# arhik/GaussianSplat

Measured on AMD Instinct MI355X. Metric: fwd+bwd Msplats/sec at 1M Gaussians, 1920x1080, SH deg 3, higher is better.
Workload: dtype f32; 1 GPU; C3: 1000000 gaussians, 1920x1080, SH3, ONE camera view per step, fwd+bwd; the steps cycle over the cameras [0, 4] (view k: eye rotated about +y by 45k degrees; one view slot per camera); synthetic scene of SURVEY 8d with the quaternions NORMALISED (8d leaves N(0,1)^4 raw: the reference never normalises q and |q| scales every footprint by |q|^4; un-normalised q is parity-tested, tests/test_gpu_size; views_per_rank=1, nranks=1, settle_steps=24, rank_mode=1, binning_rounds=1, schedule=3, view_slots=True, order=depth_desc, tile=16, instances=30150056, coarse_instances=2175944, walked_fwd=8350144, alpha_cull=True, list_cap=0, tile_parts=1, lists_capped=False

## Files before the change

### gaussiansplat_amd/backend.py

```python
from __future__ import annotations

import ctypes as C
import os

import numpy as np

_HERE = os.path.dirname(os.path.abspath(__file__))
LIB_PATH = os.environ.get("GSPLAT_HIP_LIB") or os.path.join(_HERE, "lib", "libgsplat_hip.so")

GS_MEM_HOST, GS_MEM_DEVICE = 0, 1
ORDER_INDEX, ORDER_DEPTH_DESC, ORDER_DEPTH_ASC = 0, 1, 2

(ARR_TS, ARR_TPS, ARR_MU, ARR_COV3D, ARR_COV2D, ARR_INVCOV, ARR_BBS, ARR_RGB, ARR_SIG, ARR_DEPTH_KEY,
 ARR_TILE_RECT, ARR_SORT_IDXS, ARR_TILE_RANGES, ARR_SORTED_IDS, ARR_SORTED_KEYS, ARR_GRAD2D) = range(16)

STAGES = ("preprocess", "depth_sort", "count_scan", "emit", "tile_sort", "ranges", "composite_fwd",
          "composite_bwd", "preprocess_bwd")

SYMBOLS = ("gs_default_config", "gs_abi_version", "gs_create", "gs_destroy", "gs_last_error", "gs_set_stream",
           "gs_synchronize", "gs_set_model", "gs_set_model_2d", "gs_set_image_size", "gs_set_camera", "gs_preprocess", "gs_bin", "gs_bind_outputs", "gs_forward", "gs_backward_sgd",
           "gs_backward", "gs_backward_ex", "gs_reset_grads", "gs_loss_l1_dssim", "gs_sgd_step", "gs_comm_unique_id",
           "gs_comm_init", "gs_allreduce_grads", "gs_comm_destroy", "gs_color_grads_pack", "gs_sh_grads_from_views", "gs_grads_alloc", "gs_grads_read", "gs_num_gaussians", "gs_num_instances", "gs_get_array",
           "gs_get_stage_times", "gs_get_stage_stats", "gs_get_work_counters", "gs_get_work_counters_ex", "gs_debug_time_composite",
           "gs_debug_tile_clock", "gs_debug_clock_mhz", "gs_rank_probe_result", "gs_num_rounds", "gs_set_view_slot", "gs_num_coarse_instances",
           "gs_get_list_stats", "gs_get_tile_parts", "gs_get_bin_path", "gs_debug_set_window", "gs_debug_tile_clock_rows")

GS_ABI_VERSION = 3
GS_DEBUG_WIDE_CURSORS = 1
GS_DEBUG_ALWAYS_ORDER = 2
GS_DEBUG_SUPER16 = 8
GS_DEBUG_SUPER8 = 16
GS_DEBUG_TINY_CAPS = 4
GS_MAX_VIEW_SLOTS = 4096


class GsConfig(C.Structure):
    _fields_ = [("struct_size", C.c_int32), ("abi_version", C.c_int32), ("tile_size", C.c_int32), ("order", C.c_int32), ("t_min", C.c_float),
                ("deterministic", C.c_int32), ("export_debug", C.c_int32), ("profile_stages", C.c_int32),
                ("bin_path", C.c_int32), ("rank_mode", C.c_int32), ("alpha_cull", C.c_int32), ("schedule", C.c_int32),
                ("slab_mode", C.c_int32), ("slab_max_ratio", C.c_float), ("slab_fractions", C.c_float * 3), ("debug_flags", C.c_int32),
                ("depth_sort", C.c_int32), ("list_cap", C.c_int32), ("tile_parts", C.c_int32), ("reserved", C.c_int32 * 3)]


class GsGrads(C.Structure):
    _fields_ = [("d_means", C.c_void_p), ("d_scales", C.c_void_p), ("d_quats", C.c_void_p),
                ("d_opacities", C.c_void_p), ("d_shs", C.c_void_p)]


class GsError(RuntimeError):
    def __init__(self, code: int, msg: str):
        super().__init__(f"libgsplat_hip error {code}: {msg}")
        self.code = code


_lib = None


def load():
    global _lib
    if _lib is not None:
        return _lib
    try:
        import torch
    except ImportError:
        pass
    if not os.path.exists(LIB_PATH):
        raise FileNotFoundError(f"{LIB_PATH} not found: build it with `python -m gaussiansplat_amd.build` "
                                "(there is no CPU fallback)")
    L = C.CDLL(LIB_PATH)
    vp, fp = C.c_void_p, C.POINTER(C.c_float)
    L.gs_default_config.argtypes = [C.POINTER(GsConfig)]; L.gs_default_config.restype = None
    L.gs_abi_version.restype = C.c_int
    L.gs_create.argtypes = [C.POINTER(vp), C.c_int, C.POINTER(GsConfig)]
    L.gs_destroy.argtypes = [vp]
    L.gs_last_error.argtypes = [vp]; L.gs_last_error.restype = C.c_char_p
    L.gs_set_stream.argtypes = [vp, vp]
    L.gs_synchronize.argtypes = [vp]
    L.gs_set_model.argtypes = [vp, C.c_int64, C.c_int, vp, vp, vp, vp, vp, C.c_int]
    L.gs_set_camera.argtypes = [vp, fp, fp, C.c_float, C.c_float, C.c_float, C.c_float, fp, fp, C.c_int32, C.c_int32]
    L.gs_preprocess.argtypes = [vp]
    L.gs_bin.argtypes = [vp, C.c_int32, C.c_int32]
    L.gs_bind_outputs.argtypes = [vp, vp, vp]
    L.gs_backward_sgd.argtypes = [vp, vp, C.c_int, C.c_float]
    L.gs_forward.argtypes = [vp, vp, vp, C.c_int]
    L.gs_backward.argtypes = [vp, vp, C.c_int, C.POINTER(GsGrads)]
    L.gs_backward_ex.argtypes = [vp, vp, C.c_int, C.POINTER(GsGrads), C.c_int]
    L.gs_reset_grads.argtypes = [vp, C.POINTER(GsGrads)]
    L.gs_loss_l1_dssim.argtypes = [vp, vp, vp, C.c_int32, C.c_int32, C.c_int32, C.c_float, vp, C.POINTER(C.c_double), C.c_int]
    L.gs_sgd_step.argtypes = [vp, C.c_float, C.POINTER(GsGrads)]
    L.gs_comm_unique_id.argtypes = [vp]
    L.gs_comm_init.argtypes = [vp, C.c_int, C.c_int, vp]
    L.gs_allreduce_grads.argtypes = [vp, C.POINTER(GsGrads)]
    L.gs_comm_destroy.argtypes = [vp]
    L.gs_grads_alloc.argtypes = [vp, C.POINTER(GsGrads)]
    L.gs_grads_read.argtypes = [vp, C.POINTER(GsGrads), vp, vp, vp, vp, vp]
    L.gs_num_gaussians.argtypes = [vp]; L.gs_num_gaussians.restype = C.c_int64
    L.gs_num_instances.argtypes = [vp]; L.gs_num_instances.restype = C.c_int64
    L.gs_get_array.argtypes = [vp, C.c_int, vp, C.c_int64]
    L.gs_get_stage_times.argtypes = [vp, fp]
    L.gs_get_stage_stats.argtypes = [vp, C.POINTER(C.c_double), C.POINTER(C.c_int64), C.c_int]
    L.gs_get_work_counters.argtypes = [vp, C.POINTER(C.c_int64), C.POINTER(C.c_int64)]
    L.gs_set_model_2d.argtypes = [vp, C.c_int64, vp, vp, vp, vp, vp, C.c_int]
    L.gs_set_image_size.argtypes = [vp, C.c_int32, C.c_int32]
    L.gs_color_grads_pack.argtypes = [vp, vp]
    L.gs_sh_grads_from_views.argtypes = [vp, C.c_int32, vp, vp, vp, C.c_int]
    L.gs_get_work_counters_ex.argtypes = [vp, C.POINTER(C.c_int64)]
    L.gs_debug_time_composite.argtypes = [vp, C.c_int, C.c_int, C.c_int, C.POINTER(C.c_float)]
    L.gs_debug_tile_clock.argtypes = [vp, C.c_int, C.c_int, vp]
    L.gs_debug_clock_mhz.argtypes = [vp, C.POINTER(C.c_float)]
    L.gs_rank_probe_result.argtypes = [vp]
    L.gs_num_rounds.argtypes = [vp]
    L.gs_set_view_slot.argtypes = [vp, C.c_int32]
    L.gs_num_coarse_instances.argtypes = [vp]; L.gs_num_coarse_instances.restype = C.c_int64
    L.gs_get_list_stats.argtypes = [vp, C.POINTER(C.c_int64)]
    L.gs_get_tile_parts.argtypes = [vp]
    L.gs_get_bin_path.argtypes = [vp]
    L.gs_debug_set_window.argtypes = [vp, C.c_int32, C.c_int32]
    L.gs_debug_tile_clock_rows.argtypes = [vp]
    if L.gs_abi_version() != GS_ABI_VERSION:
        raise RuntimeError(f"{LIB_PATH} has ABI version {L.gs_abi_version()}, this binding is written for {GS_ABI_VERSION}: "
                           "rebuild with `python -m gaussiansplat_amd.build --force`")
    _lib = L
    return L


def default_config() -> GsConfig:
    cfg = GsConfig()
    load().gs_default_config(C.byref(cfg))
    return cfg


class Context:

    def __init__(self, device: int = 0, order: int = ORDER_DEPTH_DESC, t_min: float = 1e-5, export_debug: bool = False,
                 profile_stages: bool = False, deterministic: bool = False, bin_path: int = 0, rank_mode: int = 1,
                 alpha_cull: bool = True, schedule: int = 0, slab_mode: int = 1, slab_fractions=(), slab_max_ratio: float = 0.0,
                 debug_flags: int = 0, depth_sort: int = 0, list_cap: int = 0, tile_parts: "int | None" = None,
                 cfg: "GsConfig | None" = None):
        self.L = load()
        if cfg is not None:
            twin = GsConfig()
            C.memmove(C.byref(twin), C.byref(cfg), C.sizeof(GsConfig))
            self.cfg = twin
            self.h = C.c_void_p()
            rc = self.L.gs_create(C.byref(self.h), device, C.byref(twin))
            if rc != 0:
                raise GsError(rc, (self.L.gs_last_error(None) or b"").decode())
            self._keep = []
            return
        cfg = default_config()
        assert cfg.struct_size == C.sizeof(GsConfig) and cfg.abi_version == GS_ABI_VERSION
        cfg.schedule = int(schedule)
        cfg.slab_mode = int(slab_mode)
        cfg.slab_max_ratio = float(slab_max_ratio)
        for i, f in enumerate(tuple(slab_fractions)[:3]):
            cfg.slab_fractions[i] = float(f)
        cfg.debug_flags = int(debug_flags)
        cfg.depth_sort = int(depth_sort)
        cfg.list_cap = int(list_cap)
        cfg.tile_parts = int(os.environ.get("GSPLAT_TILE_PARTS", "0")) if tile_parts is None else int(tile_parts)
        cfg.order, cfg.t_min = int(order), float(t_min)
        cfg.export_debug, cfg.profile_stages, cfg.deterministic = int(export_debug), int(profile_stages), int(deterministic)
        cfg.bin_path, cfg.rank_mode, cfg.alpha_cull = int(bin_path), int(rank_mode), int(alpha_cull)
        self.cfg = cfg
        self.h = C.c_void_p()
        rc = self.L.gs_create(C.byref(self.h), device, C.byref(cfg))
        if rc != 0:
            raise GsError(rc, (self.L.gs_last_error(None) or b"").decode())
        self._keep = []

    def _chk(self, rc: int):
        if rc != 0:
            raise GsError(rc, (self.L.gs_last_error(self.h) or b"").decode())

    def close(self):
        if getattr(self, "h", None) and self.h.value:
            self.L.gs_destroy(self.h)
            self.h = C.c_void_p()

    def __del__(self):
        try:
            self.close()
        except Exception:
            pass

    def set_stream(self, hip_stream: int | None):
        self._chk(self.L.gs_set_stream(self.h, C.c_void_p(hip_stream or 0)))

    def synchronize(self):
        self._chk(self.L.gs_synchronize(self.h))

    def set_model_host(self, means, scales, quats, opacities, shs, sh_degree: int):
        arrs = [np.ascontiguousarray(a, np.float32) for a in (means, scales, quats, opacities, shs)]
        n = arrs[0].shape[0]
        self._chk(self.L.gs_set_model(self.h, n, sh_degree, *(C.c_void_p(a.ctypes.data) for a in arrs), GS_MEM_HOST))

    def set_model_device(self, n: int, sh_degree: int, ptrs):
        self._chk(self.L.gs_set_model(self.h, n, sh_degree, *(C.c_void_p(int(p)) for p in ptrs), GS_MEM_DEVICE))

    def set_model_2d_host(self, means, scales, rots, opacities, colors):
        arrs = [np.ascontiguousarray(a, np.float32) for a in (means, scales, rots, opacities, colors)]
        n = arrs[0].shape[0]
        self._chk(self.L.gs_set_model_2d(self.h, n, *(C.c_void_p(a.ctypes.data) for a in arrs), GS_MEM_HOST))

    def set_model_2d_device(self, n: int, ptrs):
        self._chk(self.L.gs_set_model_2d(self.h, n, *(C.c_void_p(int(p)) for p in ptrs), GS_MEM_DEVICE))

    def set_image_size(self, W: int, H: int):
        self._chk(self.L.gs_set_image_size(self.h, int(W), int(H)))
        self.W, self.H = int(W), int(H)

    def set_camera(self, T, P, fx, fy, near, far, eye, lookAt, W, H):
        fp = C.POINTER(C.c_float)
        a = [np.ascontiguousarray(v, np.float32).reshape(-1) for v in (T, P, eye, lookAt)]
        self._chk(self.L.gs_set_camera(self.h, a[0].ctypes.data_as(fp), a[1].ctypes.data_as(fp), fx, fy, near, far,
                                       a[2].ctypes.data_as(fp), a[3].ctypes.data_as(fp), int(W), int(H)))
        self.W, self.H = int(W), int(H)

    def camera_record(self, T, P, fx, fy, near, far, eye, lookAt, W, H):
        f16, f3 = C.c_float * 16, C.c_float * 3
        a = [np.ascontiguousarray(v, np.float32).reshape(-1) for v in (T, P, eye, lookAt)]
        return (f16(*a[0]), f16(*a[1]), float(fx), float(fy), float(near), float(far), f3(*a[2]), f3(*a[3]), int(W), int(H))

    def set_camera_record(self, rec):
        self._chk(self.L.gs_set_camera(self.h, *rec))
        self.W, self.H = rec[8], rec[9]

    def set_view_slot(self, slot: int):
        self._chk(self.L.gs_set_view_slot(self.h, int(slot)))

    def preprocess(self):
        self._chk(self.L.gs_preprocess(self.h))

    def bin(self, gx: int = 0, gy: int = 0):
        self._chk(self.L.gs_bin(self.h, gx, gy))

    def forward_host(self):
        img = np.empty((3, self.H, self.W), np.float32)
        tr = np.empty((self.H, self.W), np.float32)
        self._chk(self.L.gs_forward(self.h, C.c_void_p(img.ctypes.data), C.c_void_p(tr.ctypes.data), GS_MEM_HOST))
        return img, tr

    def bind_outputs(self, image_ptr: int = 0, trans_ptr: int = 0):
        self._chk(self.L.gs_bind_outputs(self.h, C.c_void_p(image_ptr), C.c_void_p(trans_ptr)))

    def forward_device(self, image_ptr: int = 0, trans_ptr: int = 0):
        self._chk(self.L.gs_forward(self.h, C.c_void_p(image_ptr), C.c_void_p(trans_ptr), GS_MEM_DEVICE))

    def backward(self, dC_ptr_or_array, grads: GsGrads, overwrite: bool = False, phase: str = "all"):
        flags = (1 if overwrite else 0) | {"all": 0, "composite": 2, "params": 4, "params_sh": 4 | 8, "params_geom": 4 | 16}[phase]
        if isinstance(dC_ptr_or_array, np.ndarray):
            a = np.ascontiguousarray(dC_ptr_or_array, np.float32)
            self._chk(self.L.gs_backward_ex(self.h, C.c_void_p(a.ctypes.data), GS_MEM_HOST, C.byref(grads), flags))
        else:
            self._chk(self.L.gs_backward_ex(self.h, C.c_void_p(int(dC_ptr_or_array)), GS_MEM_DEVICE, C.byref(grads), flags))

    def color_grads_pack(self, drgb_ptr: int):
        self._chk(self.L.gs_color_grads_pack(self.h, C.c_void_p(int(drgb_ptr))))

    def sh_grads_from_views(self, cam_records: np.ndarray, drgb_ptr: int, d_shs_ptr: int, overwrite: bool = True):
        cr = np.ascontiguousarray(cam_records, np.float32)
        assert cr.ndim == 2 and cr.shape[1] == 38
        self._chk(self.L.gs_sh_grads_from_views(self.h, cr.shape[0], C.c_void_p(cr.ctypes.data), C.c_void_p(int(drgb_ptr)),
                                                C.c_void_p(int(d_shs_ptr)), 1 if overwrite else 0))

    def backward_sgd(self, dC_ptr: int, lr: float):
        self._chk(self.L.gs_backward_sgd(self.h, C.c_void_p(dC_ptr), GS_MEM_DEVICE, C.c_float(lr)))

    def grads_alloc(self) -> GsGrads:
        g = GsGrads()
        self._chk(self.L.gs_grads_alloc(self.h, C.byref(g)))
        return g

    def grads_read(self, grads: GsGrads, sh_degree: int) -> dict:
        n, k3 = self.num_gaussians, 3 * (sh_degree + 1) ** 2
        out = dict(means=np.empty((n, 3), np.float32), scales=np.empty((n, 3), np.float32), quats=np.empty((n, 4), np.float32),
                   opacities=np.empty((n,), np.float32), shs=np.empty((n, k3), np.float32))
        self._chk(self.L.gs_grads_read(self.h, C.byref(grads), *(C.c_void_p(out[k].ctypes.data) for k in
                                                                   ("means", "scales", "quats", "opacities", "shs"))))
        return out

    def grads_read_2d(self, grads: GsGrads) -> dict:
        n = self.num_gaussians
        out = dict(means=np.empty((n, 2), np.float32), scales=np.empty((n, 2), np.float32), rots=np.empty((n,), np.float32),
                   opacities=np.empty((n,), np.float32), colors=np.empty((n, 3), np.float32))
        self._chk(self.L.gs_grads_read(self.h, C.byref(grads), *(C.c_void_p(out[k].ctypes.data) for k in
                                                                   ("means", "scales", "rots", "opacities", "colors"))))
        return out

    def loss_host(self, img: np.ndarray, gt: np.ndarray, lam: float = 0.1):
        img = np.ascontiguousarray(img, np.float32); gt = np.ascontiguousarray(gt, np.float32)
        dC = np.empty_like(img)
        out = C.c_double()
        Cn, H, W = img.shape
        self._chk(self.L.gs_loss_l1_dssim(self.h, C.c_void_p(img.ctypes.data), C.c_void_p(gt.ctypes.data), W, H, Cn, lam,
                                          C.c_void_p(dC.ctypes.data), C.byref(out), GS_MEM_HOST))
        return float(out.value), dC

    def loss_device(self, img_ptr: int, gt_ptr: int, dC_ptr: int, W: int, H: int, Cn: int, lam: float = 0.1, want_loss: bool = True):
        out = C.c_double()
        self._chk(self.L.gs_loss_l1_dssim(self.h, C.c_void_p(img_ptr), C.c_void_p(gt_ptr), W, H, Cn, lam, C.c_void_p(dC_ptr),
                                          C.byref(out) if want_loss else None, GS_MEM_DEVICE))
        return float(out.value) if want_loss else None

    @staticmethod
    def comm_unique_id() -> bytes:
        buf = C.create_string_buffer(128)
        rc = load().gs_comm_unique_id(buf)
        if rc != 0:
            raise GsError(rc, (load().gs_last_error(None) or b"").decode())
        return buf.raw

    def comm_init(self, rank: int, nranks: int, unique_id: bytes):
        self._chk(self.L.gs_comm_init(self.h, rank, nranks, C.c_char_p(unique_id)))

    def allreduce_grads(self, grads: GsGrads):
        self._chk(self.L.gs_allreduce_grads(self.h, C.byref(grads)))

    def sgd_step(self, lr: float, grads: GsGrads):
        self._chk(self.L.gs_sgd_step(self.h, lr, C.byref(grads)))

    def reset_grads(self, grads: GsGrads):
        self._chk(self.L.gs_reset_grads(self.h, C.byref(grads)))

    @property
    def num_gaussians(self) -> int:
        return int(self.L.gs_num_gaussians(self.h))

    @property
    def num_instances(self) -> int:
        return int(self.L.gs_num_instances(self.h))

    @property
    def num_coarse_instances(self) -> int:
        return int(self.L.gs_num_coarse_instances(self.h))

    @property
    def num_rounds(self) -> int:
        return int(self.L.gs_num_rounds(self.h))

    def get_array(self, which: int, gx: int | None = None, gy: int | None = None) -> np.ndarray:
        n, ni = self.num_gaussians, self.num_instances
        spec = {ARR_TS: ((n, 4), np.float32), ARR_TPS: ((n, 4), np.float32), ARR_MU: ((n, 2), np.float32),
                ARR_COV3D: ((n, 9), np.float32), ARR_COV2D: ((n, 4), np.float32), ARR_INVCOV: ((n, 4), np.float32),
                ARR_BBS: ((n, 4), np.float32), ARR_RGB: ((n, 3), np.float32), ARR_SIG: ((n,), np.float32),
                ARR_DEPTH_KEY: ((n,), np.uint32), ARR_TILE_RECT: ((n, 4), np.uint16), ARR_SORT_IDXS: ((n,), np.uint32),
                ARR_SORTED_IDS: ((ni,), np.uint32), ARR_SORTED_KEYS: ((ni,), np.uint64), ARR_GRAD2D: ((n, 10), np.float32)}
        if which == ARR_TILE_RANGES:
            ntiles = ((self.W + 15) // 16) * ((self.H + 15) // 16)
            shape, dt = (ntiles, 2), np.uint32
        else:
            shape, dt = spec[which]
        out = np.empty(shape, dt)
        self._chk(self.L.gs_get_array(self.h, which, C.c_void_p(out.ctypes.data), out.nbytes))
        return out

    def stage_stats(self, reset: bool = False) -> dict:
        sm = (C.c_double * len(STAGES))()
        ct = (C.c_int64 * len(STAGES))()
        self._chk(self.L.gs_get_stage_stats(self.h, sm, ct, int(reset)))
        return {k: (float(sm[i]), int(ct[i])) for i, k in enumerate(STAGES)}

    def work_counters(self):
        a, b = C.c_int64(), C.c_int64()
        self._chk(self.L.gs_get_work_counters(self.h, C.byref(a), C.byref(b)))
        return int(a.value), int(b.value)

    def work_counters_ex(self) -> dict:
        o = (C.c_int64 * 4)()
        self._chk(self.L.gs_get_work_counters_ex(self.h, o))
        return dict(walked_fwd=int(o[0]), walked_bwd=int(o[1]), evaluated_fwd=int(o[2]), evaluated_bwd=int(o[3]))

    def list_stats(self) -> dict:
        o = (C.c_int64 * 3)()
        self._chk(self.L.gs_get_list_stats(self.h, o))
        return dict(listed=int(o[0]), extended_segments=int(o[1]), capped=bool(o[2]))

    def tile_parts_of_frame(self) -> int:
        rc = self.L.gs_get_tile_parts(self.h)
        if rc < 0:
            self._chk(rc)
        return int(rc)

    def bin_path_of_frame(self) -> int:
        rc = self.L.gs_get_bin_path(self.h)
        if rc < 0:
            self._chk(rc)
        return int(rc)

    def time_composite(self, which: int, variant: int, reps: int = 10) -> float:
        ms = C.c_float()
        self._chk(self.L.gs_debug_time_composite(self.h, which, variant, reps, C.byref(ms)))
        return float(ms.value)

    def tile_clock(self, which: int, variant: int = 0) -> np.ndarray:
        ntiles = ((self.W + 15) // 16) * ((self.H + 15) // 16)
        rows = ntiles
        if variant < 0:
            rows = int(self.L.gs_debug_tile_clock_rows(self.h))
            if rows <= 0:
                raise GsError(-1, "tile_clock: records by workgroup need a frame with a launch order")
        out = np.zeros((rows, 15), np.uint64)
        self._chk(self.L.gs_debug_tile_clock(self.h, which, variant, C.c_void_p(out.ctypes.data)))
        return out

    def set_debug_window(self, start: int = 0, length: int = 0):
        self._chk(self.L.gs_debug_set_window(self.h, start, length))

    def clock_mhz(self) -> float:
        mhz = C.c_float()
        self._chk(self.L.gs_debug_clock_mhz(self.h, C.byref(mhz)))
        return float(mhz.value)

    @property
    def rank_probe_result(self) -> int:
        return int(self.L.gs_rank_probe_result(self.h))

    def stage_times(self) -> dict:
        ms = (C.c_float * len(STAGES))()
        self._chk(self.L.gs_get_stage_times(self.h, ms))
        return {k: float(ms[i]) for i, k in enumerate(STAGES)}
```

### gaussiansplat_amd/csrc/gs_api_composite.hip

```cpp
#include "gs_ctx.h"

const uint32_t *forward_order(gs_ctx *c) {
    const int64_t ntiles = (int64_t)c->gx * c->gy;
    if (!lpt_schedule(c) || ntiles <= 0 || ntiles > GS_LPT_MAX_TILES) return nullptr;
    const int k = order_index(c);
    if (k == GS_MAX_VIEW_SLOTS && c->cfg.schedule != 4) return nullptr;
    if (c->slots[k].tiles != (((int64_t)c->gx << 32) | (int64_t)c->gy)) return nullptr;
    if (c->order_pending) {
        if (hipStreamWaitEvent(c->stream, c->ev_order, 0) != hipSuccess) return nullptr;
        c->order_pending = false;
    }
    c->frame_order_split = c->pinned_split ? c->pinned_split + 2 * k + c->slots[k].sel : nullptr;
    return c->slots[k].order[c->slots[k].sel].as<uint32_t>();
}

int build_frame_order(gs_ctx *c, const uint32_t *used) {
    const int64_t ntiles = (int64_t)c->gx * c->gy;
    c->frame_order = used;
    if (!lpt_schedule(c) || ntiles <= 0 || ntiles > GS_LPT_MAX_TILES) return GS_OK;
    const int k = order_index(c);
    const int dst = used ? 1 - c->slots[k].sel : c->slots[k].sel;
    DevBuf &ob = c->slots[k].order[dst];
    HIPCHK(c, ob.ensure(sizeof(uint32_t) * ((size_t)lpt_order_entries(c) + GS_SEG_SLOTS + 16)));
    const uint32_t *walked = lpt_front(c) > 0 ? c->last_walked : nullptr;
    uint32_t *rearm = nullptr, *nsplit = c->pinned_split ? c->pinned_split + 2 * k + dst : nullptr;
    if (nsplit) *nsplit = 0xFFFFFFFFu;
    if (lpt_front(c) > 0) {
        if (!c->snap_walked.p) {
            HIPCHK(c, c->snap_walked.ensure(sizeof(uint32_t) * 2 * GS_SEG_SLOTS));
            HIPCHK(c, hipMemsetAsync(c->snap_walked.p, 0, sizeof(uint32_t) * 2 * GS_SEG_SLOTS, c->stream));
        }
        rearm = c->snap_walked.as<uint32_t>() + (size_t)(c->snap_parity ^ 1) * GS_SEG_SLOTS;
    }
    if (used && use_side_stream(c)) {
        if (c->order_pending) HIPCHK(c, hipStreamWaitEvent(c->stream, c->ev_order, 0));
        HIPCHK(c, hipEventRecord(c->ev_main, c->stream));
        HIPCHK(c, hipStreamWaitEvent(c->side, c->ev_main, 0));
        HIPCHK(c, gs_launch_tile_lpt_order(c->tile_work.as<uint32_t>(), 0, c->gx, c->gy, ob.as<uint32_t>(), c->side, nullptr, 0, lpt_front(c), lpt_split_div(c), walked, rearm, nsplit));
        HIPCHK(c, hipEventRecord(c->ev_order, c->side));
        c->order_pending = true;
        c->slots[k].sel = dst;
    } else {
        HIPCHK(c, gs_launch_tile_lpt_order(c->tile_work.as<uint32_t>(), 0, c->gx, c->gy, ob.as<uint32_t>(), c->stream, nullptr, 0, lpt_front(c), lpt_split_div(c), walked, rearm, nsplit));
        c->frame_order = ob.as<uint32_t>();
        c->frame_order_split = nsplit;
    }
    c->slots[k].tiles = ((int64_t)c->gx << 32) | (int64_t)c->gy;
    return GS_OK;
}

extern "C" {

int gs_bind_outputs(gs_ctx *c, float *image, float *transmittance) {
    if (!c) return GS_ERR_INVALID;
    if ((image == nullptr) != (transmittance == nullptr)) return fail(c, GS_ERR_INVALID, "gs_bind_outputs: bind both buffers or neither");
    c->bound_image = image; c->bound_trans = transmittance;
    c->did_fwd = c->did_bwd = false;
    return GS_OK;
}

int gs_set_view_slot(gs_ctx *c, int32_t slot) {
    if (!c) return GS_ERR_INVALID;
    if (slot >= GS_MAX_VIEW_SLOTS) return fail(c, GS_ERR_INVALID, "gs_set_view_slot: slot must be below GS_MAX_VIEW_SLOTS (or negative: none)");
    c->view_slot = slot < 0 ? -1 : (int)slot;
    return GS_OK;
}

static int composite_parts(const gs_ctx *c) {
    const int want = c->cfg.tile_parts;
    if (want == 1 || !(c->cfg.t_min > 0.0f) || c->n_rounds > 1 || c->frame_capped) return 1;
    if (want == 2 || want == 4) return want;
    const long long ntiles = (long long)c->gx * c->gy, slots = c->wave_slots;
    return 4 * ntiles <= slots ? 4 : 2 * ntiles <= slots ? 2 : 1;
}

static int enqueue_forward_round(gs_ctx *c, int r, const uint32_t *order) {
    const int R = c->n_rounds;
    GsCompositeArgs a{};
    a.W = c->cam.W; a.H = c->cam.H; a.gx = c->gx; a.gy = c->gy; a.t_min = c->cfg.t_min;
    a.ranges = r == 0 ? c->ranges.as<uint32_t>() : c->ranges_r[r].as<uint32_t>();
    a.ids = c->ids.as<uint32_t>() + c->round_ids_off[r]; a.payload = c->payload.as<GsPayload>();
    a.image = c->img(); a.trans = c->tr();
    a.walked = nullptr;
    a.cull = c->cfg.alpha_cull != 0;
    a.resume = r > 0; a.final_round = r == R - 1;
    a.tile_work = c->tile_work.as<uint32_t>(); a.tile_walked = const_cast<uint32_t *>(c->last_walked);
    a.tile_order = order; a.order_len = order ? lpt_order_entries(c) : 0;
    a.parts = c->frame_parts;
    a.split_ok = order && lpt_front(c) > 0 && c->frame_parts == 1 && !c->frame_capped && R == 1;
    c->snap_order = nullptr;
    if (c->frame_seg_n && R == 1) {
        const size_t nt = (size_t)c->gx * c->gy;
        HIPCHK(c, c->snap.ensure(sizeof(float) * nt * (size_t)(c->frame_seg_n - 1) * 4 * 256));
        HIPCHK(c, c->tile_walked_b.ensure(sizeof(uint32_t) * (nt ? nt : 1)));
        HIPCHK(c, c->tile_work_b.ensure(sizeof(uint32_t) * (nt ? nt : 1)));
        a.snap = c->snap.as<float>(); a.seg_hist = c->seg_hist; a.seg_n = c->frame_seg_n;
        a.bw_walked = c->tile_walked_b.as<uint32_t>(); a.bw_work = c->tile_work_b.as<uint32_t>();
    }
    const bool may_split = !c->frame_order_split || *c->frame_order_split != 0u;
    if (a.split_ok && c->snap_walked.p && may_split) {
        HIPCHK(c, c->snap.ensure(sizeof(float) * (size_t)GS_SEG_SLOTS * GS_SEG_SNAP_FLOATS));
        const size_t nt = (size_t)c->gx * c->gy;
        HIPCHK(c, c->tile_walked_b.ensure(sizeof(uint32_t) * (nt ? nt : 1)));
        HIPCHK(c, c->tile_work_b.ensure(sizeof(uint32_t) * (nt ? nt : 1)));
        a.snap = c->snap.as<float>(); a.seg_len = order_seg_len(c, order); a.front = lpt_front(c);
        a.snap_walked = c->snap_walked.as<uint32_t>() + (size_t)c->snap_parity * GS_SEG_SLOTS;
        a.bw_walked = c->tile_walked_b.as<uint32_t>(); a.bw_work = c->tile_work_b.as<uint32_t>();
        c->snap_order = order;
    }
    if (c->frame_capped && R == 1) {
        a.tile_ext = c->tile_ext.as<uint2>(); a.cranges = c->cranges.as<uint32_t>(); a.cids = c->cids.as<uint32_t>(); a.clr = c->clr.as<uint16_t>();
        a.ids_w = c->ids.as<uint32_t>(); a.sgx = c->sgx; a.sbs = c->sbs; a.ext_count = c->ext_count();
    }
    if (R > 1) { a.tile_pos = c->tile_pos.as<uint32_t>(); a.tile_done = c->tile_done.as<uint8_t>(); a.tile_dead = c->tile_dead.as<unsigned long long>(); }
    StageTimer t(c, GS_STAGE_COMPOSITE_FWD);
    HIPCHK(c, gs_launch_composite_fwd(a, c->stream));
    return GS_OK;
}

int gs_forward(gs_ctx *c, float *image, float *transmittance, int mem) {
    if (!c) return GS_ERR_INVALID;
    if (!c->did_bin) return fail(c, GS_ERR_INVALID, "gs_forward: gs_bin first");
    if (mem != GS_MEM_HOST && mem != GS_MEM_DEVICE) return fail(c, GS_ERR_INVALID, "gs_forward: bad mem");
    if (bind_device(c)) return GS_ERR_HIP;
    const size_t px = (size_t)c->cam.W * c->cam.H;
    const size_t ntiles = (size_t)c->gx * c->gy;
    if (!c->bound_image) {
        HIPCHK(c, c->image.ensure(sizeof(float) * 3 * px));
        HIPCHK(c, c->trans.ensure(sizeof(float) * px));
    }
    HIPCHK(c, c->counters.ensure(GS_COUNTER_BYTES));
    HIPCHK(c, c->tile_work.ensure(sizeof(uint32_t) * (ntiles ? ntiles : 1)));
    c->counters_grid = ((int64_t)c->gx << 32) | (int64_t)c->gy;
    c->frame_seg_n = 0; c->seg_hist = nullptr;
    int flip_slot = -1;
    {
        const int k = order_index(c);
        if (k < GS_MAX_VIEW_SLOTS || c->cfg.schedule == 4) {
            gs_ctx::ViewSlot &vs = c->slots[k];
            DevBuf &wb = vs.walkbuf[vs.wsel ^ 1];
            HIPCHK(c, wb.ensure(sizeof(uint32_t) * (ntiles ? ntiles : 1)));
            const bool hist = vs.walked_grid == c->counters_grid && vs.walked().p;
            if (hist && c->cfg.tile_parts == 0 && c->cfg.t_min > 0.0f && c->n_rounds == 1 && !c->frame_capped && !lpt_schedule(c) && c->kind == 0 &&
                2 * (int64_t)ntiles <= c->wave_slots && ntiles > 0) {
                c->frame_seg_n = 2;
                c->seg_hist = vs.walked().as<uint32_t>();
            }
            c->last_walked = wb.as<uint32_t>();
            flip_slot = k;
        } else {
            HIPCHK(c, c->tile_walked.ensure(sizeof(uint32_t) * (ntiles ? ntiles : 1)));
            c->last_walked = c->tile_walked.as<uint32_t>();
        }
    }
    const int R = c->n_rounds;
    if (R > 1) {
        HIPCHK(c, c->tile_pos.ensure(sizeof(uint32_t) * (ntiles ? ntiles : 1)));
        HIPCHK(c, c->tile_done.ensure(ntiles ? ntiles : 1));
        HIPCHK(c, c->tile_dead.ensure(sizeof(unsigned long long) * 4 * (ntiles ? ntiles : 1)));
        HIPCHK(c, hipMemsetAsync(c->tile_pos.p, 0, sizeof(uint32_t) * ntiles, c->stream));
    }
    c->frame_parts = composite_parts(c);
    c->snap_parity ^= 1;
    const uint32_t *order = forward_order(c);
    if (c->order_pending) { HIPCHK(c, hipStreamWaitEvent(c->stream, c->ev_order, 0)); c->order_pending = false; }
    for (int r = 0; r < R; ++r) {
        if (r > 0) { if (int rc = bin_round(c, r)) return rc; }
        if (int rc = enqueue_forward_round(c, r, order)) return rc;
        if (r == 0) {
            bool redo = false;
            if (int rc = settle_totals(c, &redo, true)) return rc;
            if (redo) {
                if (int rc = enqueue_forward_round(c, 0, order)) return rc;
            }
        }
    }
    if (flip_slot >= 0) { c->slots[flip_slot].wsel ^= 1; c->slots[flip_slot].walked_grid = c->counters_grid; }
    if (int rc = build_frame_order(c, order)) return rc;
    const hipMemcpyKind kind = mem == GS_MEM_HOST ? hipMemcpyDeviceToHost : hipMemcpyDeviceToDevice;
    if (image && image != c->img()) HIPCHK(c, hipMemcpyAsync(image, c->img(), sizeof(float) * 3 * px, kind, c->stream));
    if (transmittance && transmittance != c->tr()) HIPCHK(c, hipMemcpyAsync(transmittance, c->tr(), sizeof(float) * px, kind, c->stream));
    if (mem == GS_MEM_HOST && (image || transmittance)) HIPCHK(c, hipStreamSynchronize(c->stream));
    c->did_fwd = true; c->did_bwd = false; c->did_bwd_composite = false;
    c->prev_counters_valid = true; c->prev_n_inst = c->n_inst;
    return GS_OK;
}

int gs_backward(gs_ctx *c, const float *dC, int mem, const gs_grads *grads) { return gs_backward_ex(c, dC, mem, grads, 0); }

static int backward_impl(gs_ctx *c, const float *dC, int mem, const gs_grads *grads, int flags, float sgd_scale);
int gs_backward_ex(gs_ctx *c, const float *dC, int mem, const gs_grads *grads, int flags) { return backward_impl(c, dC, mem, grads, flags, 0.0f); }

int gs_backward_sgd(gs_ctx *c, const float *dC, int mem, float lr) {
    if (!c) return GS_ERR_INVALID;
    if (c->kind != 0) return fail(c, GS_ERR_UNSUPPORTED, "gs_backward_sgd: 3-D renderer only");
    if (!(lr != 0.0f)) return fail(c, GS_ERR_INVALID, "gs_backward_sgd: lr must be non-zero");
    gs_grads g{const_cast<float *>(c->means), const_cast<float *>(c->scales), const_cast<float *>(c->quats),
               const_cast<float *>(c->opac), const_cast<float *>(c->shs)};
    const int rc = backward_impl(c, dC, mem, &g, 0, -lr);
    if (rc == GS_OK) c->did_pre = c->did_bin = c->did_fwd = c->did_bwd = false;
    return rc;
}

static int backward_impl(gs_ctx *c, const float *dC, int mem, const gs_grads *grads, int flags, float sgd_scale) {
    if (!c) return GS_ERR_INVALID;
    if (!c->did_fwd) return fail(c, GS_ERR_INVALID, "gs_backward: gs_forward first");
    const bool params_only = (flags & GS_BWD_PARAMS_ONLY) != 0, composite_only = (flags & GS_BWD_COMPOSITE_ONLY) != 0;
    if (params_only && composite_only) return fail(c, GS_ERR_INVALID, "gs_backward: COMPOSITE_ONLY and PARAMS_ONLY exclude each other");
    const int chain = (flags & (GS_BWD_PARAMS_SH | GS_BWD_PARAMS_GEOM)) >> 3;
    if (chain && !params_only) return fail(c, GS_ERR_INVALID, "gs_backward: GS_BWD_PARAMS_SH / _GEOM need GS_BWD_PARAMS_ONLY");
    if (chain && c->kind != 0) return fail(c, GS_ERR_UNSUPPORTED, "gs_backward: GS_BWD_PARAMS_SH / _GEOM: 3-D renderer only");
    if (params_only && !c->did_bwd_composite) return fail(c, GS_ERR_INVALID, "gs_backward: GS_BWD_PARAMS_ONLY needs a GS_BWD_COMPOSITE_ONLY call on this frame");
    if ((!dC && !params_only) || (!grads && !composite_only)) return fail(c, GS_ERR_INVALID, "gs_backward: NULL argument");
    if (mem != GS_MEM_HOST && mem != GS_MEM_DEVICE) return fail(c, GS_ERR_INVALID, "gs_backward: bad mem");
    if (bind_device(c)) return GS_ERR_HIP;
    const size_t px = (size_t)c->cam.W * c->cam.H, n1 = c->n ? (size_t)c->n : 1;
    const float *dC_dev = dC;
    if (mem == GS_MEM_HOST && !params_only) {
        HIPCHK(c, c->stage_in.ensure(sizeof(float) * 3 * px));
        HIPCHK(c, hipMemcpyAsync(c->stage_in.p, dC, sizeof(float) * 3 * px, hipMemcpyHostToDevice, c->stream));
        dC_dev = c->stage_in.as<float>();
    }
    const bool det = c->cfg.deterministic != 0;
    HIPCHK(c, c->g2d.ensure((det ? sizeof(long long) : sizeof(float)) * GS_G2D_STRIDE * n1));
    GsCompositeArgs a{};
    a.W = c->cam.W; a.H = c->cam.H; a.gx = c->gx; a.gy = c->gy; a.t_min = c->cfg.t_min;
    a.ranges = c->ranges.as<uint32_t>(); a.ids = c->ids.as<uint32_t>(); a.payload = c->payload.as<GsPayload>();
    a.image = c->img(); a.trans = c->tr();
    a.nseg = 0;
    for (int r = 0; r < c->n_rounds; ++r) {
        if (r > 0 && c->round_gen[r] == 0) continue;
        a.seg_ranges[a.nseg] = r == 0 ? c->ranges.as<uint32_t>() : c->ranges_r[r].as<uint32_t>();
        a.seg_ids[a.nseg] = c->ids.as<uint32_t>() + c->round_ids_off[r];
        ++a.nseg;
    }
    a.dC = dC_dev; a.g2d = det ? nullptr : c->g2d.as<float>(); a.g2d_fixed = det ? c->g2d.as<long long>() : nullptr;
    {
        const size_t nt = (size_t)c->gx * c->gy;
        HIPCHK(c, c->tile_walked_b.ensure(sizeof(uint32_t) * (nt ? nt : 1)));
        HIPCHK(c, c->tile_work_b.ensure(sizeof(uint32_t) * (nt ? nt : 1)));
    }
    a.walked = nullptr; a.tile_walked = c->tile_walked_b.as<uint32_t>(); a.tile_work = c->tile_work_b.as<uint32_t>();
    if (c->frame_capped && c->n_rounds == 1) a.tile_ext = c->tile_ext.as<uint2>();
    a.cull = c->cfg.alpha_cull != 0;
    a.parts = c->frame_parts;
    if (c->frame_seg_n && c->n_rounds == 1 && !c->frame_capped) {
        const long long nt = (long long)c->gx * c->gy;
        a.snap = c->snap.as<float>(); a.seg_hist = c->seg_hist; a.seg_n = c->frame_seg_n;
        a.parts = 4 * a.seg_n * nt <= c->wave_slots ? 4 : 2 * a.seg_n * nt <= c->wave_slots ? 2 : 1;
    }
    if (!params_only) {
        c->last_dC = dC_dev;
        if (!c->g2d_clean) HIPCHK(c, hipMemsetAsync(c->g2d.p, 0, (det ? sizeof(long long) : sizeof(float)) * GS_G2D_STRIDE * n1, c->stream));
        c->g2d_clean = false;
        if (lpt_schedule(c)) { a.tile_order = c->frame_order; a.order_len = c->frame_order ? lpt_order_entries(c) : 0; }
        a.split_ok = a.tile_order && lpt_front(c) > 0 && c->frame_parts == 1 && !c->frame_capped && c->n_rounds == 1;
        if (a.split_ok && c->snap_order && c->snap_order == a.tile_order) {
            a.snap = c->snap.as<float>(); a.seg_len = order_seg_len(c, a.tile_order); a.front = lpt_front(c);
            a.snap_walked = c->snap_walked.as<uint32_t>() + (size_t)c->snap_parity * GS_SEG_SLOTS;
        }
        {
            StageTimer t(c, GS_STAGE_COMPOSITE_BWD);
            HIPCHK(c, gs_launch_composite_bwd(a, c->stream));
        }
        c->did_bwd_composite = true;
    }
    if (composite_only) {
        if (mem == GS_MEM_HOST) HIPCHK(c, hipStreamSynchronize(c->stream));
        c->did_bwd = true;
        return GS_OK;
    }
    if (c->kind == 1) {
        GsPreprocess2DBwdArgs b2{};
        b2.n = c->n; b2.W = c->cam.W; b2.H = c->cam.H;
        b2.scales = c->scales; b2.rots = c->quats; b2.opac = c->opac;
        b2.g2d = det ? nullptr : c->g2d.as<float>(); b2.g2d_fixed = det ? c->g2d.as<long long>() : nullptr;
        b2.overwrite = (flags & GS_BWD_OVERWRITE) ? 1 : 0;
        b2.d_means = grads->d_means; b2.d_scales = grads->d_scales; b2.d_rots = grads->d_quats;
        b2.d_opac = grads->d_opacities; b2.d_colors = grads->d_shs;
        {
            StageTimer t(c, GS_STAGE_PREPROCESS_BWD);
            HIPCHK(c, gs_launch_preprocess2d_bwd(b2, c->stream));
        }
        if (mem == GS_MEM_HOST) HIPCHK(c, hipStreamSynchronize(c->stream));
        c->did_bwd = true;
        return GS_OK;
    }
    GsPreprocessBwdArgs b{};
    b.n = c->n; b.sh_degree = c->sh_degree;
    b.means = c->means; b.scales = c->scales; b.quats = c->quats; b.opac = c->opac; b.shs = c->shs;
    b.g2d = det ? nullptr : c->g2d.as<float>(); b.g2d_fixed = det ? c->g2d.as<long long>() : nullptr;
    HIPCHK(c, c->dpc.ensure(sizeof(float) * 4 * n1));
    b.dpc = c->dpc.as<float>();
    b.overwrite = (flags & GS_BWD_OVERWRITE) ? 1 : 0;
    b.sgd_scale = sgd_scale;
    b.d_means = grads->d_means; b.d_scales = grads->d_scales; b.d_quats = grads->d_quats;
    b.d_opac = grads->d_opacities; b.d_shs = grads->d_shs;
    {
        StageTimer t(c, GS_STAGE_PREPROCESS_BWD);
        HIPCHK(c, gs_launch_preprocess_bwd(b, c->cam, c->stream, chain ? chain : 3));
    }
    if (mem == GS_MEM_HOST) HIPCHK(c, hipStreamSynchronize(c->stream));
    c->did_bwd = true;
    return GS_OK;
}

int gs_color_grads_pack(gs_ctx *c, float *drgb) {
    if (!c || !drgb) return GS_ERR_INVALID;
    if (c->kind != 0) return fail(c, GS_ERR_UNSUPPORTED, "gs_color_grads_pack: 3-D renderer only");
    if (!c->did_bwd) return fail(c, GS_ERR_INVALID, "gs_color_grads_pack: gs_backward first");
    if (bind_device(c)) return GS_ERR_HIP;
    const bool det = c->cfg.deterministic != 0;
    HIPCHK(c, gs_launch_pack_drgb(det ? nullptr : c->g2d.as<float>(), det ? c->g2d.as<long long>() : nullptr, drgb, c->n, c->stream));
    return GS_OK;
}

int gs_sh_grads_from_views(gs_ctx *c, int32_t nviews, const float *cams, const float *drgb, float *d_shs, int flags) {
    if (!c || !cams || !drgb || !d_shs || nviews <= 0) return GS_ERR_INVALID;
    if (c->kind != 0) return fail(c, GS_ERR_UNSUPPORTED, "gs_sh_grads_from_views: 3-D renderer only");
    if (bind_device(c)) return GS_ERR_HIP;
    const size_t bytes = sizeof(float) * GS_VIEW_RECORD_FLOATS * (size_t)nviews;
    HIPCHK(c, c->view_cams.ensure(bytes));
    HIPCHK(c, hipMemcpyAsync(c->view_cams.p, cams, bytes, hipMemcpyHostToDevice, c->stream));
    HIPCHK(c, gs_launch_sh_from_views(c->n, c->sh_degree, c->means, nviews, c->view_cams.as<float>(), drgb, d_shs,
                                      (flags & GS_BWD_OVERWRITE) ? 1 : 0, c->stream));
    return GS_OK;
}

}
```

### gaussiansplat_amd/csrc/gs_api_debug.hip

```cpp
#include "gs_ctx.h"

extern "C" {

int64_t gs_num_gaussians(const gs_ctx *c) { return c ? c->n : 0; }
int64_t gs_num_instances(gs_ctx *c) { if (!c) return 0; (void)settle_totals(c, nullptr, true); return c->n_inst; }
int64_t gs_num_coarse_instances(gs_ctx *c) { if (!c) return 0; (void)settle_totals(c, nullptr, true); return c->two_level ? c->n_coarse : 0; }
int gs_num_rounds(const gs_ctx *c) { return c ? c->n_rounds : 0; }

int gs_get_array(gs_ctx *c, int which, void *dst, int64_t bytes) {
    if (!c || !dst) return GS_ERR_INVALID;
    if (bind_device(c)) return GS_ERR_HIP;
    const size_t n = (size_t)c->n;
    const void *src = nullptr;
    size_t need = 0;
    auto need_dbg = [&](int i, size_t w) -> int {
        if (!c->cfg.export_debug) return fail(c, GS_ERR_INVALID, "gs_get_array: needs gs_config.export_debug = 1");
        src = c->dbg[i].p; need = sizeof(float) * w * n; return GS_OK;
    };
    if (which <= GS_ARR_TILE_RECT && !c->did_pre) return fail(c, GS_ERR_INVALID, "gs_get_array: gs_preprocess first");
    if (which >= GS_ARR_SORT_IDXS && which <= GS_ARR_SORTED_KEYS && !c->did_bin) return fail(c, GS_ERR_INVALID, "gs_get_array: gs_bin first");
    if (which >= GS_ARR_TILE_RANGES && which <= GS_ARR_SORTED_KEYS) { if (int rc = settle_totals(c, nullptr, true)) return rc; }
    if (which >= GS_ARR_TILE_RANGES && which <= GS_ARR_SORTED_KEYS && c->n_rounds > 1)
        return fail(c, GS_ERR_INVALID, "gs_get_array: this frame was binned in depth slabs (lists spread over rounds); use gs_config.slab_mode = 0");
    if ((which == GS_ARR_SORTED_IDS || which == GS_ARR_SORTED_KEYS) && c->frame_capped && c->have_l2) {
        GsBin3Args a = c->last_l2;
        a.cap_src = nullptr; a.tile_nopen = nullptr; a.smax = nullptr; a.tile_ext = nullptr;
        HIPCHK(c, gs_bin3_write_lists(a, c->stream));
        c->frame_capped = false;
    }
    switch (which) {
        case GS_ARR_TS: if (int r = need_dbg(0, 4)) return r; break;
        case GS_ARR_TPS: if (int r = need_dbg(1, 4)) return r; break;
        case GS_ARR_COV3D: if (int r = need_dbg(3, 9)) return r; break;
        case GS_ARR_COV2D: if (int r = need_dbg(4, 4)) return r; break;
        case GS_ARR_BBS: if (int r = need_dbg(6, 4)) return r; break;
        case GS_ARR_INVCOV: src = c->invcov.p; need = sizeof(float) * 4 * n; break;
        case GS_ARR_MU: case GS_ARR_RGB: case GS_ARR_SIG: {
            const size_t w = which == GS_ARR_MU ? 2 : which == GS_ARR_RGB ? 3 : 1;
            if ((size_t)bytes != sizeof(float) * w * n) return fail(c, GS_ERR_INVALID, "gs_get_array: size mismatch");
            std::vector<GsPayload> h(n ? n : 1);
            HIPCHK(c, hipMemcpyAsync(h.data(), c->payload.p, sizeof(GsPayload) * n, hipMemcpyDeviceToHost, c->stream));
            HIPCHK(c, hipStreamSynchronize(c->stream));
            float *o = static_cast<float *>(dst);
            for (size_t g = 0; g < n; ++g) {
                const GsPayload &p = h[g];
                if (which == GS_ARR_MU) { o[2 * g] = p.mx; o[2 * g + 1] = p.my; }
                else if (which == GS_ARR_RGB) { o[3 * g] = p.r; o[3 * g + 1] = p.g; o[3 * g + 2] = p.b; }
                else o[g] = p.sig;
            }
            return GS_OK;
        }
        case GS_ARR_DEPTH_KEY: src = c->depth_key.p; need = sizeof(uint32_t) * n; break;
        case GS_ARR_TILE_RECT: src = c->rect.p; need = sizeof(uint16_t) * 4 * n; break;
        case GS_ARR_SORT_IDXS: {
            if ((size_t)bytes != sizeof(uint32_t) * n) return fail(c, GS_ERR_INVALID, "gs_get_array: size mismatch");
            if (c->perm_pending) {
                uint32_t *perm = nullptr;
                if (int rc = depth_order(c, &perm)) return rc;
                c->perm_ptr = c->perm_all = perm; c->perm_pending = false;
            }
            if (c->perm_ptr) { src = c->perm_ptr; need = sizeof(uint32_t) * n; break; }
            uint32_t *o = static_cast<uint32_t *>(dst);
            for (size_t g = 0; g < n; ++g) o[g] = (uint32_t)g;
            return GS_OK;
        }
        case GS_ARR_TILE_RANGES: src = c->ranges.p; need = sizeof(uint32_t) * 2 * (size_t)c->gx * c->gy; break;
        case GS_ARR_SORTED_IDS: case GS_ARR_SORTED_KEYS: {
            const size_t ni = (size_t)c->n_inst, nt = (size_t)c->gx * c->gy;
            const size_t w = which == GS_ARR_SORTED_IDS ? sizeof(uint32_t) : sizeof(uint64_t);
            if ((size_t)bytes != w * ni) return fail(c, GS_ERR_INVALID, "gs_get_array: size mismatch");
            std::vector<uint32_t> h(ni ? ni : 1), dk(n ? n : 1), rg(2 * (nt ? nt : 1));
            HIPCHK(c, hipMemcpyAsync(h.data(), c->ids.p, sizeof(uint32_t) * ni, hipMemcpyDeviceToHost, c->stream));
            HIPCHK(c, hipMemcpyAsync(dk.data(), c->depth_key.p, sizeof(uint32_t) * n, hipMemcpyDeviceToHost, c->stream));
            HIPCHK(c, hipMemcpyAsync(rg.data(), c->ranges.p, sizeof(uint32_t) * 2 * nt, hipMemcpyDeviceToHost, c->stream));
            HIPCHK(c, hipStreamSynchronize(c->stream));
            if (which == GS_ARR_SORTED_IDS) {
                std::memcpy(dst, h.data(), sizeof(uint32_t) * ni);
            } else {
                uint64_t *o = static_cast<uint64_t *>(dst);
                const bool by_index = c->order() == GS_ORDER_INDEX;
                for (size_t t = 0; t < nt; ++t)
                    for (size_t p = rg[2 * t]; p < rg[2 * t + 1] && p < ni; ++p)
                        o[p] = ((uint64_t)t << 32) | (by_index ? h[p] : dk[h[p]]);
            }
            return GS_OK;
        }
        case GS_ARR_GRAD2D: {
            if (!c->did_bwd) return fail(c, GS_ERR_INVALID, "gs_get_array: gs_backward first");
            if ((size_t)bytes != sizeof(float) * 10 * n) return fail(c, GS_ERR_INVALID, "gs_get_array: size mismatch");
            float *o = static_cast<float *>(dst);
            if (c->cfg.deterministic) {
                std::vector<long long> fx((size_t)GS_G2D_STRIDE * (n ? n : 1));
                if (n) HIPCHK(c, hipMemcpyAsync(fx.data(), c->g2d.p, sizeof(long long) * GS_G2D_STRIDE * n, hipMemcpyDeviceToHost, c->stream));
                HIPCHK(c, hipStreamSynchronize(c->stream));
                for (size_t g = 0; g < n; ++g)
                    for (int i = 0; i < 10; ++i) o[10 * g + i] = (float)((double)fx[GS_G2D_STRIDE * g + i] * gs_fixed_inv(i));
            } else {
                std::vector<float> fl((size_t)GS_G2D_STRIDE * (n ? n : 1));
                if (n) HIPCHK(c, hipMemcpyAsync(fl.data(), c->g2d.p, sizeof(float) * GS_G2D_STRIDE * n, hipMemcpyDeviceToHost, c->stream));
                HIPCHK(c, hipStreamSynchronize(c->stream));
                for (size_t g = 0; g < n; ++g)
                    for (int i = 0; i < 10; ++i) o[10 * g + i] = fl[GS_G2D_STRIDE * g + i];
            }
            std::vector<GsPayload> pay(n ? n : 1);
            std::vector<float> ic(4 * (n ? n : 1));
            if (n) HIPCHK(c, hipMemcpyAsync(pay.data(), c->payload.p, sizeof(GsPayload) * n, hipMemcpyDeviceToHost, c->stream));
            if (n) HIPCHK(c, hipMemcpyAsync(ic.data(), c->invcov.p, sizeof(float) * 4 * n, hipMemcpyDeviceToHost, c->stream));
            HIPCHK(c, hipStreamSynchronize(c->stream));
            for (size_t g = 0; g < n; ++g) {
                float row[10];
                for (int i = 0; i < 10; ++i) row[i] = o[10 * g + i];
                gs_g2d_to_grads(row, pay[g].sig, ic[4 * g], 0.5f * (ic[4 * g + 1] + ic[4 * g + 2]), ic[4 * g + 3]);
                for (int i = 0; i < 10; ++i) o[10 * g + i] = row[i];
            }
            return GS_OK;
        }
        default: return fail(c, GS_ERR_INVALID, "gs_get_array: unknown array");
    }
    if ((size_t)bytes != need) return fail(c, GS_ERR_INVALID, "gs_get_array: size mismatch");
    if (need) HIPCHK(c, hipMemcpyAsync(dst, src, need, hipMemcpyDeviceToHost, c->stream));
    HIPCHK(c, hipStreamSynchronize(c->stream));
    return GS_OK;
}

int gs_get_stage_times(gs_ctx *c, float ms[GS_STAGE_COUNT]) {
    if (!c || !ms) return GS_ERR_INVALID;
    if (!c->cfg.profile_stages) return fail(c, GS_ERR_INVALID, "gs_get_stage_times: needs gs_config.profile_stages = 1");
    if (bind_device(c)) return GS_ERR_HIP;
    HIPCHK(c, hipStreamSynchronize(c->stream));
    for (int s = 0; s < GS_STAGE_COUNT; ++s) {
        ms[s] = 0.0f;
        if (c->ev_valid[s]) HIPCHK(c, hipEventElapsedTime(&ms[s], c->ev[s][0], c->ev[s][1]));
    }
    return GS_OK;
}

int gs_get_stage_stats(gs_ctx *c, double sum_ms[GS_STAGE_COUNT], int64_t count[GS_STAGE_COUNT], int reset) {
    if (!c || !sum_ms || !count) return GS_ERR_INVALID;
    if (!c->cfg.profile_stages) return fail(c, GS_ERR_INVALID, "gs_get_stage_stats: needs gs_config.profile_stages = 1");
    if (bind_device(c)) return GS_ERR_HIP;
    HIPCHK(c, hipStreamSynchronize(c->stream));
    harvest_events(c);
    for (int s = 0; s < GS_STAGE_COUNT; ++s) {
        sum_ms[s] = c->ev_sum[s]; count[s] = c->ev_cnt[s];
        if (reset) { c->ev_sum[s] = 0.0; c->ev_cnt[s] = 0; }
    }
    return GS_OK;
}

static int debug_composite_args(gs_ctx *c, int which, int variant, GsCompositeArgs &a) {
    a.W = c->cam.W; a.H = c->cam.H; a.gx = c->gx; a.gy = c->gy; a.t_min = c->cfg.t_min;
    a.ranges = c->ranges.as<uint32_t>(); a.ids = c->ids.as<uint32_t>(); a.payload = c->payload.as<GsPayload>();
    a.image = c->img(); a.trans = c->tr();
    a.dC = c->last_dC; a.walked = nullptr;
    if (variant >= 10000) {
        variant -= 10000;
        a.walked = reinterpret_cast<unsigned long long *>(static_cast<char *>(c->counters.p) + 160);
    }
    a.final_round = 1;
    a.nseg = 0;
    for (int r = 0; r < c->n_rounds; ++r) {
        if (r > 0 && c->round_gen[r] == 0) continue;
        a.seg_ranges[a.nseg] = r == 0 ? c->ranges.as<uint32_t>() : c->ranges_r[r].as<uint32_t>();
        a.seg_ids[a.nseg] = c->ids.as<uint32_t>() + c->round_ids_off[r];
        ++a.nseg;
    }
    a.g2d = c->cfg.deterministic ? nullptr : c->g2d.as<float>(); a.g2d_fixed = c->cfg.deterministic ? c->g2d.as<long long>() : nullptr;
    c->g2d_clean = false;
    if (c->frame_capped && c->n_rounds == 1) {
        a.tile_ext = c->tile_ext.as<uint2>(); a.cranges = c->cranges.as<uint32_t>(); a.cids = c->cids.as<uint32_t>(); a.clr = c->clr.as<uint16_t>();
        a.ids_w = c->ids.as<uint32_t>(); a.sgx = c->sgx; a.sbs = c->sbs; a.ext_count = c->ext_count();
    }
    a.variant = variant % 100;
    a.cull = (c->cfg.alpha_cull != 0) != (variant >= 1000);
    a.tile_order = lpt_schedule(c) ? c->frame_order : nullptr;
    a.order_len = a.tile_order ? lpt_order_entries(c) : 0;
    a.split_ok = a.tile_order && lpt_front(c) > 0 && c->frame_parts == 1 && !c->frame_capped && c->n_rounds == 1;
    if (which == 1 && a.split_ok && c->snap_order && c->snap_order == a.tile_order) {
        a.snap = c->snap.as<float>(); a.seg_len = order_seg_len(c, a.tile_order); a.front = lpt_front(c);
        a.snap_walked = c->snap_walked.as<uint32_t>() + (size_t)c->snap_parity * GS_SEG_SLOTS;
    }
    a.parts = c->frame_parts;
    if (which == 1 && c->frame_seg_n && c->n_rounds == 1 && !c->frame_capped && !a.tile_order) {
        const long long nt = (long long)c->gx * c->gy;
        a.snap = c->snap.as<float>(); a.seg_hist = c->seg_hist; a.seg_n = c->frame_seg_n;
        a.parts = 4 * a.seg_n * nt <= c->wave_slots ? 4 : 2 * a.seg_n * nt <= c->wave_slots ? 2 : 1;
    }
    if (c->dbg_win_len > 0) {
        if (!a.tile_order || a.parts > 1) return fail(c, GS_ERR_INVALID, "gs_debug_set_window: the frame has no launch order (or several waves per tile)");
        if (c->dbg_win_start + c->dbg_win_len > a.order_len) return fail(c, GS_ERR_INVALID, "gs_debug_set_window: beyond the launch order");
        a.tile_order += c->dbg_win_start; a.order_len = c->dbg_win_len;
    }
    return GS_OK;
}

int gs_debug_set_window(gs_ctx *c, int32_t start, int32_t len) {
    if (!c) return GS_ERR_INVALID;
    if (start < 0 || len < 0 || (start & 7) || (len & 7)) return fail(c, GS_ERR_INVALID, "gs_debug_set_window: start and len must be non-negative multiples of 8");
    c->dbg_win_start = start; c->dbg_win_len = len;
    return GS_OK;
}

int gs_debug_time_composite(gs_ctx *c, int which, int variant, int reps, float *mean_ms) {
    if (!c || !mean_ms || reps == 0) return GS_ERR_INVALID;
    const bool cold = reps < 0;
    if (cold) reps = -reps;
    if (!c->did_fwd) return fail(c, GS_ERR_INVALID, "gs_debug_time_composite: gs_forward first");
    if (which == 1 && !c->did_bwd) return fail(c, GS_ERR_INVALID, "gs_debug_time_composite: gs_backward first");
    if (bind_device(c)) return GS_ERR_HIP;
    GsCompositeArgs a{};
    if (int rc = debug_composite_args(c, which, variant, a)) return rc;
    hipEvent_t e0, e1;
    HIPCHK(c, hipEventCreate(&e0)); HIPCHK(c, hipEventCreate(&e1));
    auto launch = [&]() -> hipError_t { return which == 0 ? gs_launch_composite_fwd(a, c->stream) : gs_launch_composite_bwd(a, c->stream); };
    if (!cold) HIPCHK(c, launch());
    HIPCHK(c, hipEventRecord(e0, c->stream));
    for (int i = 0; i < reps; ++i) HIPCHK(c, launch());
    HIPCHK(c, hipEventRecord(e1, c->stream));
    HIPCHK(c, hipEventSynchronize(e1));
    float ms = 0.0f;
    HIPCHK(c, hipEventElapsedTime(&ms, e0, e1));
    *mean_ms = ms / reps;
    (void)hipEventDestroy(e0); (void)hipEventDestroy(e1);
    return GS_OK;
}

int gs_debug_tile_clock(gs_ctx *c, int which, int variant, uint64_t *out) {
    if (!c || !out) return GS_ERR_INVALID;
    if (!c->did_fwd) return fail(c, GS_ERR_INVALID, "gs_debug_tile_clock: gs_forward first");
    if (which == 1 && !c->did_bwd) return fail(c, GS_ERR_INVALID, "gs_debug_tile_clock: gs_backward first");
    if (bind_device(c)) return GS_ERR_HIP;
    const size_t ntiles = (size_t)c->gx * c->gy;
    GsCompositeArgs a{};
    const bool by_block = variant < 0;
    if (by_block) variant = -variant;
    if (int rc = debug_composite_args(c, which, variant, a)) return rc;
    if (by_block) {
        if ((!a.tile_order && a.parts <= 1 && !a.seg_hist) || (a.variant / 10) % 10 == 1)
            return fail(c, GS_ERR_INVALID, "gs_debug_tile_clock: records by workgroup need the frame's launch order (or a small grid's tile parts)");
        a.clock_by_block = 1;
    } else { a.split_ok = 0; a.snap = nullptr; }
    const size_t rows = !a.clock_by_block ? ntiles : a.tile_order ? (size_t)(lpt_order_entries(c) + gs_seg_units(lpt_front(c))) : (size_t)gs_debug_tile_clock_rows(c);
    if (a.clock_by_block && (size_t)gs_composite_grid_blocks(a, which) > rows) return fail(c, GS_ERR_INVALID, "gs_debug_tile_clock: launch larger than its record");
    HIPCHK(c, c->tile_clock.ensure(sizeof(uint64_t) * GS_TILE_CLOCK_WORDS * (rows ? rows : 1)));
    HIPCHK(c, hipMemsetAsync(c->tile_clock.p, 0, sizeof(uint64_t) * GS_TILE_CLOCK_WORDS * rows, c->stream));
    a.tile_clock = c->tile_clock.as<unsigned long long>();
    for (int rep = 0; rep < 2; ++rep) {
        HIPCHK(c, which == 0 ? gs_launch_composite_fwd(a, c->stream) : gs_launch_composite_bwd(a, c->stream));
    }
    HIPCHK(c, hipMemcpyAsync(out, c->tile_clock.p, sizeof(uint64_t) * GS_TILE_CLOCK_WORDS * rows, hipMemcpyDeviceToHost, c->stream));
    HIPCHK(c, hipStreamSynchronize(c->stream));
    return GS_OK;
}

int gs_debug_tile_clock_rows(gs_ctx *c) {
    if (!c) return GS_ERR_INVALID;
    if (lpt_schedule(c)) return lpt_order_entries(c) + gs_seg_units(lpt_front(c));
    const int len = ((c->gx * c->gy + 7) / 8) * 8;
    const int units = std::max(c->frame_parts, 1) * (c->frame_seg_n ? 4 * c->frame_seg_n : 1);
    return units > 1 ? len * units : 0;
}

int gs_debug_clock_mhz(gs_ctx *c, float *mhz) {
    if (!c || !mhz) return GS_ERR_INVALID;
    if (bind_device(c)) return GS_ERR_HIP;
    HIPCHK(c, c->counters.ensure(GS_COUNTER_BYTES));
    unsigned long long *d = reinterpret_cast<unsigned long long *>(static_cast<char *>(c->counters.p) + 160), h[2] = {0, 1};
    HIPCHK(c, gs_launch_clock_probe(d, c->stream));
    HIPCHK(c, hipMemcpyAsync(h, d, sizeof(h), hipMemcpyDeviceToHost, c->stream));
    HIPCHK(c, hipStreamSynchronize(c->stream));
    *mhz = h[1] ? (float)((double)h[0] / (double)h[1] * 100.0) : 0.0f;
    return GS_OK;
}

int gs_rank_probe_result(const gs_ctx *c) { return c ? c->rank_probe : -1; }

static int sum_work_counters(gs_ctx *c) {
    unsigned long long *w = c->counters.as<unsigned long long>();
    const int nt = c->gx * c->gy;
    HIPCHK(c, gs_launch_sum_tiles(c->last_walked, c->tile_work.as<uint32_t>(), nt, w, c->stream));
    if (c->did_bwd_composite && c->tile_walked_b.p && c->tile_work_b.p)
        HIPCHK(c, gs_launch_sum_tiles(c->tile_walked_b.as<uint32_t>(), c->tile_work_b.as<uint32_t>(), nt, w + 2, c->stream));
    else HIPCHK(c, hipMemsetAsync(w + 2, 0, 16, c->stream));
    return GS_OK;
}

int gs_get_work_counters(gs_ctx *c, int64_t *walked_fwd, int64_t *walked_bwd) {
    if (!c) return GS_ERR_INVALID;
    if (!c->did_fwd) return fail(c, GS_ERR_INVALID, "gs_get_work_counters: gs_forward first");
    if (bind_device(c)) return GS_ERR_HIP;
    unsigned long long h[4] = {0, 0, 0, 0};
    if (int rc = sum_work_counters(c)) return rc;
    HIPCHK(c, hipMemcpyAsync(h, c->counters.p, 32, hipMemcpyDeviceToHost, c->stream));
    HIPCHK(c, hipStreamSynchronize(c->stream));
    if (walked_fwd) *walked_fwd = (int64_t)h[0];
    if (walked_bwd) *walked_bwd = (int64_t)h[2];
    return GS_OK;
}

int gs_get_list_stats(gs_ctx *c, int64_t out[3]) {
    if (!c || !out) return GS_ERR_INVALID;
    if (!c->did_fwd) return fail(c, GS_ERR_INVALID, "gs_get_list_stats: gs_forward first");
    if (bind_device(c)) return GS_ERR_HIP;
    if (int rc = settle_totals(c, nullptr, true)) return rc;
    out[0] = c->n_inst; out[1] = 0; out[2] = 0;
    if (!c->frame_capped || c->n_rounds != 1) return GS_OK;
    unsigned long long *d = reinterpret_cast<unsigned long long *>(static_cast<char *>(c->counters.p) + 160), h = 0;
    uint32_t e = 0;
    HIPCHK(c, gs_launch_sum_listed(c->tile_ext.as<uint2>(), c->gx * c->gy, d, c->stream));
    HIPCHK(c, hipMemcpyAsync(&h, d, sizeof(h), hipMemcpyDeviceToHost, c->stream));
    HIPCHK(c, hipMemcpyAsync(&e, c->ext_count(), sizeof(e), hipMemcpyDeviceToHost, c->stream));
    HIPCHK(c, hipStreamSynchronize(c->stream));
    out[0] = (int64_t)h; out[1] = (int64_t)e; out[2] = 1;
    return GS_OK;
}

int gs_get_tile_parts(gs_ctx *c) {
    if (!c) return GS_ERR_INVALID;
    if (!c->did_fwd) return fail(c, GS_ERR_INVALID, "gs_get_tile_parts: gs_forward first");
    return c->frame_parts;
}

int gs_get_bin_path(gs_ctx *c) {
    if (!c) return GS_ERR_INVALID;
    if (!c->did_bin) return fail(c, GS_ERR_INVALID, "gs_get_bin_path: gs_bin first");
    return c->small_bin ? 3 : c->two_level ? 0 : c->fast_bin ? 2 : 1;
}

int gs_get_work_counters_ex(gs_ctx *c, int64_t out[4]) {
    if (!c || !out) return GS_ERR_INVALID;
    if (!c->did_fwd) return fail(c, GS_ERR_INVALID, "gs_get_work_counters_ex: gs_forward first");
    if (bind_device(c)) return GS_ERR_HIP;
    unsigned long long h[4] = {0, 0, 0, 0};
    if (int rc = sum_work_counters(c)) return rc;
    HIPCHK(c, hipMemcpyAsync(h, c->counters.p, 32, hipMemcpyDeviceToHost, c->stream));
    HIPCHK(c, hipStreamSynchronize(c->stream));
    out[0] = (int64_t)h[0]; out[1] = (int64_t)h[2]; out[2] = (int64_t)h[1]; out[3] = (int64_t)h[3];
    return GS_OK;
}

}
```

### gaussiansplat_amd/csrc/gs_common.h

```cpp
#pragma once
#include <hip/hip_runtime.h>
#include <stdint.h>

#define GS_TILE 16
#define GS_WAVE 64

#define GS_PAYLOAD_QUADS 4
#define GS_BIG 1.0e30f
struct __attribute__((aligned(16))) GsPayload {
    float mx, my;
    float l2s;
    float xlo;
    float ka, kb, kc;
    float xhi;
    float r, g, b;
    float ylo;
    float yhi;
    float sig;
    uint32_t bbx;
    uint32_t bby;
};
static_assert(sizeof(GsPayload) == 16 * GS_PAYLOAD_QUADS, "payload row size");
__host__ __device__ inline void gs_payload_box_edges(GsPayload &p) {
    const int xmin = (int)(short)(p.bbx & 0xFFFFu), xmax = (int)(short)(p.bbx >> 16);
    const int ymin = (int)(short)(p.bby & 0xFFFFu), ymax = (int)(short)(p.bby >> 16);
    const bool empty = xmax < xmin || ymax < ymin;
    p.xlo = empty ? GS_BIG : ((float)xmin - p.mx) - 0.25f; p.xhi = empty ? GS_BIG : ((float)xmax - p.mx) + 0.25f;
    p.ylo = empty ? GS_BIG : ((float)ymin - p.my) - 0.25f; p.yhi = empty ? GS_BIG : ((float)ymax - p.my) + 0.25f;
}
#define GS_NEG_HALF_LOG2E (-0.72134752044448170368f)
#define GS_L2S_CAP (-2.6e-7f)

struct GsCamera {
    float T[16], P[16];
    float fx, fy, near_, far_;
    float eye[3], lookAt[3];
    int32_t W, H;
};

struct GsDebugArrays {
    float *ts, *tps, *mu, *cov3d, *cov2d, *invcov, *bbs;
};

struct GsPreprocessArgs {
    int64_t n;
    int sh_degree;
    int order;
    int gx, gy;
    const float *means, *scales, *quats, *opac, *shs;
    GsPayload *payload;
    float *invcov;
    uint32_t *depth_key;
    uint16_t *rect;
    GsDebugArrays dbg;
    uint32_t *key_range;
};
#define GS_KEY_RANGE_SLOTS 64
#define GS_KEY_RANGE_STRIDE 64
hipError_t gs_launch_preprocess(const GsPreprocessArgs &a, const GsCamera &cam, hipStream_t stream);

struct GsPreprocess2DArgs {
    int64_t n;
    int W, H, gx, gy;
    const float *means, *scales, *rots, *opac, *colors;
    GsPayload *payload;
    float *invcov;
    uint32_t *depth_key;
    uint16_t *rect;
    GsDebugArrays dbg;
};
struct GsPreprocess2DBwdArgs {
    int64_t n;
    int W, H;
    const float *scales, *rots, *opac;
    const float *g2d;
    const long long *g2d_fixed;
    float *d_means, *d_scales, *d_rots, *d_opac, *d_colors;
    int overwrite;
};
hipError_t gs_launch_preprocess2d(const GsPreprocess2DArgs &a, hipStream_t stream);
hipError_t gs_launch_preprocess2d_bwd(const GsPreprocess2DBwdArgs &a, hipStream_t stream);

struct GsSortScratch {
    uint32_t *block_hist;
    uint32_t *digit_total;
};
size_t gs_sort_table_entries(int64_t n_max);
hipError_t gs_radix_sort_u64(uint64_t *a, uint64_t *b, int64_t n, int bit_lo, int bit_hi,
                             uint32_t *block_hist, uint32_t *digit_total, int *result_in_b,
                             hipStream_t stream, bool ballot_ranks = false, uint32_t *final_low32 = nullptr,
                             const uint32_t *keys32 = nullptr);

size_t gs_depth_range_words();
size_t gs_depth_range_parity_words();
int64_t gs_depth_buckets_max_n();
hipError_t gs_depth_range_reset(uint32_t *acc, hipStream_t s, int nparity = 2);
hipError_t gs_depth_sort_buckets(const uint32_t *keys32, uint64_t *pairs_a, uint64_t *pairs_b, int64_t n, uint32_t *block_hist,
                                 uint32_t *digit_total, uint32_t *perm, const uint32_t *range_acc, uint32_t *reset_acc,
                                 uint32_t *host_stat, hipStream_t stream, bool ballot_ranks);

hipError_t gs_probe_lds_atomic_order(hipStream_t s, int *mismatches);
hipError_t gs_launch_depth_pairs(const uint32_t *depth_key, uint64_t *pairs, int64_t n, hipStream_t s);
hipError_t gs_launch_unpack_perm(const uint64_t *pairs, uint32_t *perm, int64_t n, hipStream_t s);
hipError_t gs_launch_count_scan(const uint16_t *rect, const uint32_t *perm, uint32_t *offsets,
                                uint32_t *block_sums, int64_t n, hipStream_t s);
hipError_t gs_launch_live_prefix(const uint8_t *done, int gx, int gy, uint32_t *live2d, uint32_t *rowp_scratch, hipStream_t s);
hipError_t gs_launch_count_scan_live(const uint16_t *rect, const uint32_t *perm, const uint32_t *live2d, int gx, uint16_t *rect_out,
                                     uint32_t *offsets, uint32_t *block_sums, int64_t n, hipStream_t s);
hipError_t gs_launch_emit(const uint16_t *rect, const uint32_t *perm, const uint32_t *offsets,
                          uint64_t *inst, int64_t n, int gx, hipStream_t s);
hipError_t gs_launch_ranges(const uint64_t *inst, int64_t n_inst, uint32_t *ranges, int64_t n_tiles,
                            hipStream_t s);
hipError_t gs_launch_split_ids(const uint64_t *inst, uint32_t *ids, int64_t n_inst, hipStream_t s);
hipError_t gs_launch_radix_scan(uint32_t *block_hist, int nblocks, uint32_t *digit_total, hipStream_t s);

size_t gs_tile_ranges_scratch_ints(int gx, int gy);
bool gs_tile_ranges_supported(int gx, int gy);
hipError_t gs_launch_tile_ranges(const uint16_t *rect, const uint32_t *perm, int64_t n, int *scratch, int gx, int gy, uint32_t *ranges,
                                 const uint8_t *done, hipStream_t s);
struct GsBin2Args {
    int64_t n, n_inst;
    int gx;
    int lo_bits, hi_bits, gid_bits;
    const uint32_t *offsets, *perm;
    const uint16_t *rect;
    uint32_t *cs;
    uint32_t *block_hist, *digit_total;
    uint32_t *buf_a;
    uint32_t *ids_out;
    bool ballot_ranks;
    const uint8_t *done;
    uint32_t *live_total;
};
hipError_t gs_bin2_build_lists(const GsBin2Args &b, hipStream_t s);

struct GsBin3L1 {
    const uint16_t *rect;
    const uint32_t *perm;
    const uint8_t *sdone;
    int64_t n, n_slab;
    int sgx, ns;
    int sbs;
    uint32_t *rect_sorted;
    uint32_t *table;
    uint32_t *row_total;
    uint32_t *partials;
    uint32_t *totals;
    uint32_t *cranges;
    uint32_t *cids;
    uint16_t *clr;
    uint32_t *tilecnt;
    int ntiles;
    uint32_t *zero_words;
    uint32_t cap_coarse, cap_fine;
    uint32_t *host_totals, *host_walked;
    const uint32_t *walked_src;
    const uint32_t *tile_walked;
    int n_tile_walked;
};
struct GsBin3Args {
    const uint32_t *cranges;
    const uint32_t *cids;
    const uint16_t *clr;
    uint32_t *ranges;
    uint32_t *tilecnt;
    const uint8_t *done;
    uint32_t *segcnt;
    uint32_t *ids_out;
    int gx, gy, sgx, ns;
    int sbs;
    int max_work;
    int wide;
    const uint32_t *totals;
    uint32_t cap_coarse, cap_fine;
    const uint32_t *cap_src;
    uint32_t *tile_nopen;
    uint32_t *smax;
    uint2 *tile_ext;
    uint32_t *ext_count;
};
#define GS_CONT_NONE 0xFFFFFFFFu
__host__ __device__ inline uint32_t gs_list_cap(uint32_t w) { const uint32_t c = w + (w >> 2) + 128u; return c < w ? 0xFFFFFFFFu : c; }
int gs_bin3_seg();
int gs_bin3_sb_shift(int gx, int gy, int force);
bool gs_bin3_supported(int ns);
int64_t gs_bin3_max_work(int64_t coarse_instances, int ns);
size_t gs_bin3_table_words(int64_t n_slab, int ns);
size_t gs_bin3_partial_words(int64_t n, int ns);
hipError_t gs_bin3_l1_count(const GsBin3L1 &b, hipStream_t s);
hipError_t gs_bin3_l1_scatter(const GsBin3L1 &b, hipStream_t s);
hipError_t gs_bin3_build_lists(const GsBin3Args &a, hipStream_t s);
hipError_t gs_bin3_write_lists(const GsBin3Args &a, hipStream_t s);
hipError_t gs_launch_super_done(const uint8_t *done, int gx, int gy, int sgx, int sgy, int sbs, uint8_t *sdone, hipStream_t s);

#define GS_BIN_SMALL_MAX_N 16384
#define GS_BIN_SMALL_MAX_TILES 1024
#define GS_BIN_SMALL_MAX_PAIRS (4ll << 20)
struct GsBinSmallArgs {
    const uint32_t *depth_key;
    const uint2 *rect;
    int n, gx, gy, ntiles;
    uint32_t *ranges;
    uint32_t *ids;
    uint32_t *totals;
    uint32_t *host_totals, *host_walked;
    const uint32_t *walked_src, *tile_walked;
    int n_tile_walked;
    uint4 *zero; size_t zero_words16;
};
bool gs_bin_small_supported(int64_t n, int gx, int gy);
hipError_t gs_bin_small(const GsBinSmallArgs &a, hipStream_t s);

#define GS_TILE_CLOCK_WORDS 15
#define GS_MAX_ROUNDS 4
#define GS_G2D_STRIDE 16
struct GsCompositeArgs {
    int W, H, gx, gy;
    float t_min;
    const uint32_t *ranges;
    const uint32_t *ids;
    const GsPayload *payload;
    float *image;
    float *trans;
    const float *dC;
    float *g2d;
    long long *g2d_fixed;
    unsigned long long *walked;
    uint32_t *tile_walked;
    int cull;
    int variant;
    const uint32_t *tile_order;
    int order_len;
    uint32_t *tile_work;
    unsigned long long *zero_words;
    unsigned long long *tile_clock;
    int nseg;
    const uint32_t *seg_ranges[GS_MAX_ROUNDS];
    const uint32_t *seg_ids[GS_MAX_ROUNDS];
    uint32_t *tile_pos;
    uint8_t *tile_done;
    unsigned long long *tile_dead;
    int resume;
    int final_round;
    uint2 *tile_ext;
    const uint32_t *cranges, *cids;
    const uint16_t *clr;
    uint32_t *ids_w;
    int sgx, sbs;
    uint32_t *ext_count;
    int parts;
    int split_ok;
    float *snap;
    const uint32_t *seg_len;
    uint32_t *snap_walked;
    int front;
    uint32_t *bw_walked, *bw_work;
    const uint32_t *seg_hist;
    int seg_n;
    int clock_by_block;
};
hipError_t gs_launch_sum_listed(const uint2 *ext, int n, unsigned long long *out, hipStream_t s);
#define GS_LPT_MAX_TILES 35000
int gs_lpt_order_len(int gx, int gy);
hipError_t gs_launch_clock_probe(unsigned long long *out, hipStream_t s);
hipError_t gs_launch_sum_tiles(const uint32_t *a, const uint32_t *b, int n, unsigned long long *out, hipStream_t s);
#define GS_LPT_FRONT 2304
#define GS_SEG_MAX 8
#define GS_SEG_MIN_LEN 1024
#define GS_SEG_ALL_MIN_LEN 128
#define GS_SEG_SLOTS (GS_LPT_FRONT / 3)
#define GS_SEG_SNAP_FLOATS ((GS_SEG_MAX - 1) * 4 * 256)
hipError_t gs_launch_tile_lpt_order(const uint32_t *work_or_ranges, int ranges_mode, int gx, int gy, uint32_t *order, hipStream_t s,
                                    unsigned long long *zero14 = nullptr, int buckets = 0, int front = 0, int split_div = 1,
                                    const uint32_t *walked = nullptr, uint32_t *zero_words = nullptr, uint32_t *host_nsplit = nullptr);
#ifndef GS_SEG_ALL_NUM
#define GS_SEG_ALL_NUM 5
#define GS_SEG_ALL_DEN 8
#endif
#ifndef GS_SEG_ALL_SHORT
#define GS_SEG_ALL_SHORT 1
#endif
__host__ __device__ inline uint32_t gs_seg_len_all(uint32_t w, int seg_n) {
    if (GS_SEG_ALL_SHORT && w >= 80u && w <= (seg_n == 2 ? 192u : 64u * (uint32_t)seg_n + 64u)) return 64u;
    const uint32_t per = seg_n == 2 ? (w * GS_SEG_ALL_NUM + GS_SEG_ALL_DEN - 1u) / GS_SEG_ALL_DEN : (w + (uint32_t)seg_n - 1u) / (uint32_t)seg_n, sl = ((per + 63u) & ~63u) < (uint32_t)GS_SEG_ALL_MIN_LEN ? (uint32_t)GS_SEG_ALL_MIN_LEN : ((per + 63u) & ~63u);
    return w > sl ? sl : 0u;
}
int gs_seg_units(int front);
int gs_composite_grid_blocks(const GsCompositeArgs &a, int bwd);
hipError_t gs_launch_composite_fwd(const GsCompositeArgs &a, hipStream_t s);
hipError_t gs_launch_composite_bwd(const GsCompositeArgs &a, hipStream_t s);

struct GsPreprocessBwdArgs {
    int64_t n;
    int sh_degree;
    const float *means, *scales, *quats, *opac, *shs;
    const float *g2d;
    const long long *g2d_fixed;
    float *d_means, *d_scales, *d_quats, *d_opac, *d_shs;
    float *dpc;
    int overwrite;
    float sgd_scale;
};
hipError_t gs_launch_preprocess_bwd(const GsPreprocessBwdArgs &a, const GsCamera &cam, hipStream_t s, int phases = 3);

hipError_t gs_launch_pack_drgb(const float *g2d, const long long *g2d_fixed, float *out, int64_t n, hipStream_t s);
hipError_t gs_launch_sh_from_views(int64_t n, int sh_degree, const float *means, int nviews, const float *cams, const float *drgb,
                                   float *d_shs, int overwrite, hipStream_t s);

template <typename R>
__host__ __device__ inline void gs_g2d_to_grads(R (&g2)[10], R sig, R i0, R mc, R i3) {
#pragma clang fp contract(off)
    const R S0 = g2[3], Sx = g2[4], Sy = g2[5], Sxx = g2[6], Sxy = g2[7], Syy = g2[9];
    g2[3] = sig > R(0) ? -S0 / sig : R(0);
    g2[4] = -(i0 * Sx + mc * Sy);
    g2[5] = -(mc * Sx + i3 * Sy);
    g2[6] = R(0.5) * Sxx; g2[7] = R(0.5) * Sxy; g2[8] = R(0.5) * Sxy; g2[9] = R(0.5) * Syy;
}

#define GS_FIXED_SCALE 1099511627776.0f
#define GS_FIXED_INV (1.0 / 1099511627776.0)
#define GS_FIXED_SCALE2 268435456.0f
#define GS_FIXED_INV2 (1.0 / 268435456.0)
__host__ __device__ inline double gs_fixed_inv(int comp) { return comp >= 6 ? GS_FIXED_INV2 : GS_FIXED_INV; }

#define GS_LOSS_SLOTS 64
#define GS_LOSS_SLOT_STRIDE 8
hipError_t gs_loss_run(int W, int H, int C, const float *img, const float *gt, float *maps, double *acc, float *dC, float lam,
                       const float *win121, hipStream_t s);
hipError_t gs_launch_sgd(float *p, const float *g, float lr, size_t n, hipStream_t s);
```

### gaussiansplat_amd/csrc/gs_composite.hip

```cpp
#include "gs_common.h"

#pragma clang fp contract(off)

#ifndef GS_BWD_MINW
#define GS_BWD_MINW 6
#endif
#ifndef GS_FWD_MINW
#define GS_FWD_MINW 5
#endif
#ifndef GS_LIVE_RECT
#define GS_LIVE_RECT 1
#endif
#ifndef GS_FWD_PACK
#define GS_FWD_PACK 1
#endif
#ifndef GS_FWD_NO_PREFETCH
#define GS_FWD_NO_PREFETCH 0
#endif
#ifndef GS_BWD_PAIR
#define GS_BWD_PAIR 1
#endif
#ifndef GS_FWD_UNROLL
#define GS_FWD_UNROLL 2
#endif
constexpr int kFwdUnroll = GS_FWD_UNROLL;
#define CB 64
#ifndef L2_SEG
#define L2_SEG 2048
#endif
__device__ __forceinline__ int gs_bin3_seg_const() { return L2_SEG; }
#define NEG_HALF_LOG2E (-0.72134752044448170368f)

__device__ __forceinline__ float fast_exp2(float x) { return __builtin_amdgcn_exp2f(x); }
__device__ __forceinline__ float vgpr_const(float x) { float r; asm volatile("v_mov_b32 %0, %1" : "=v"(r) : "s"(x)); return r; }
__device__ __forceinline__ float fast_rcp(float x) { return __builtin_amdgcn_rcpf(x); }

#define GS_ORDER_TILE_MASK 0x0FFFFFFFu
__device__ __forceinline__ int tile_of_block(const GsCompositeArgs &a, int ntiles, int &part, int &nparts, int first_block = 0) {
    const int len = (a.tile_order && a.order_len > 0) ? a.order_len : ((ntiles + 7) / 8) * 8;
    int b = (int)blockIdx.x - first_block;
    part = 0; nparts = a.parts > 1 ? a.parts : 1;
    if (a.parts > 1) { part = b / len; b -= part * len; if (part >= a.parts) return -1; }
    if (a.tile_order) {
        if (b >= (a.order_len > 0 ? a.order_len : ntiles)) return -1;
        uint32_t t = a.tile_order[b];
        if (t == 0xFFFFFFFFu) return -1;
        if (a.parts <= 1 && (t >> 28)) {
            part = (int)((t >> 28) & 3u); nparts = 1 << (t >> 30);
            if (!a.split_ok) { if (part) return -1; nparts = 1; }
        }
        t &= GS_ORDER_TILE_MASK;
        return t < (uint32_t)ntiles ? (int)t : -1;
    }
    return b < ntiles ? b : -1;
}
__device__ __forceinline__ uint32_t strips_of_part(int nparts, int part) {
    return nparts == 4 ? (1u << part) : nparts == 2 ? (3u << (2 * part)) : 0xFu;
}

__device__ __forceinline__ unsigned long long wave_hw_id() {
    const uint32_t hw = (uint32_t)__builtin_amdgcn_s_getreg((4) | (0 << 6) | (31 << 11));
    const uint32_t xcc = (uint32_t)__builtin_amdgcn_s_getreg((20) | (0 << 6) | (3 << 11));
    return (unsigned long long)hw | ((unsigned long long)xcc << 32);
}

#define GS_ALPHA_CULL_LOG2 (-27.0f)
__device__ __forceinline__ bool rect_can_contribute(float A, float B, float C, float hBrA, float hBrC, bool concave, float l2s,
                                                    float rx0, float rx1, float ry0, float ry1) {
    const float cx = __builtin_amdgcn_fmed3f(0.0f, rx0, rx1), cy = __builtin_amdgcn_fmed3f(0.0f, ry0, ry1);
    const float dy1 = __builtin_amdgcn_fmed3f(-(hBrC * cx), ry0, ry1);
    const float dx2 = __builtin_amdgcn_fmed3f(-(hBrA * cy), rx0, rx1);
    const float f1 = fmaf(A * cx, cx, dy1 * fmaf(B, cx, C * dy1));
    const float f2 = fmaf(C * cy, cy, dx2 * fmaf(B, cy, A * dx2));
    const float fm = (cx != 0.0f && cy != 0.0f) ? fmaxf(f1, f2) : (cx != 0.0f ? f1 : f2);
    const bool nopix = rx0 > rx1 || ry0 > ry1;
    return !(nopix || (concave && fm + l2s < GS_ALPHA_CULL_LOG2));
}

template <bool STRIPS>
__device__ __forceinline__ void stage_record(const float4 &n0, const float4 &n1, const float4 &n3, const int qx0, const int qx1, const int qy0, const int qy1,
                                             const int ty0, bool &keep, uint32_t &strips) {
    const uint32_t bbx = __float_as_uint(n3.z), bby = __float_as_uint(n3.w);
    const int xmin = (int)(short)(bbx & 0xFFFFu), xmax = (int)(short)(bbx >> 16);
    const int ymin = (int)(short)(bby & 0xFFFFu), ymax = (int)(short)(bby >> 16);
    const bool empty = xmax < xmin || ymax < ymin;
    const float l2s = n0.z;
    const float A = n1.x, B = n1.y, C = n1.z;
    const bool concave = A < 0.0f && C < 0.0f && 4.0f * A * C - B * B > 0.0f;
    const float rx0 = (float)max(qx0, xmin) - n0.x, rx1 = (float)min(qx1, xmax) - n0.x;
    const float ry0 = (float)max(qy0, ymin) - n0.y, ry1 = (float)min(qy1, ymax) - n0.y;
    const float hBrA = 0.5f * B * fast_rcp(A), hBrC = 0.5f * B * fast_rcp(C);
    keep = !empty && rect_can_contribute(A, B, C, hBrA, hBrC, concave, l2s, rx0, rx1, ry0, ry1);
    strips = 0xFu;
    if (STRIPS) {
        strips = 0;
#pragma unroll
        for (int p = 0; p < 4; ++p) {
            const float sy0 = (float)max(max(ty0 + 4 * p, qy0), ymin) - n0.y, sy1 = (float)min(min(ty0 + 4 * p + 3, qy1), ymax) - n0.y;
            if (keep && rect_can_contribute(A, B, C, hBrA, hBrC, concave, l2s, rx0, rx1, sy0, sy1)) strips |= 1u << p;
        }
    }
}

__device__ __forceinline__ void first_use_here(float4 &a, float4 &b, float4 &c, float4 &d) {
    asm volatile("" : "+v"(a.x), "+v"(a.y), "+v"(a.z), "+v"(a.w), "+v"(b.x), "+v"(b.y), "+v"(b.z), "+v"(b.w),
                      "+v"(c.x), "+v"(c.y), "+v"(c.z), "+v"(c.w), "+v"(d.x), "+v"(d.y), "+v"(d.z), "+v"(d.w));
}

__device__ __forceinline__ int wave_min_i32(int v) {
#pragma unroll
    for (int d = 32; d > 0; d >>= 1) v = min(v, __shfl_xor(v, d));
    return __builtin_amdgcn_readfirstlane(v);
}
__device__ __forceinline__ int wave_max_i32(int v) {
#pragma unroll
    for (int d = 32; d > 0; d >>= 1) v = max(v, __shfl_xor(v, d));
    return __builtin_amdgcn_readfirstlane(v);
}

#ifndef GS_RECT_FROM_MASKS
#define GS_RECT_FROM_MASKS 1
#endif
struct LiveRectAcc {
    uint64_t any = 0; uint32_t rows = 0;
    __device__ __forceinline__ void slot(const int p, const uint64_t m) {
        any |= m;
        uint64_t t = m | (m >> 8); t |= t >> 4; t |= t >> 2; t |= t >> 1;
        t &= 0x0001000100010001ull;
        rows |= (uint32_t)((t | (t >> 15) | (t >> 30) | (t >> 45)) & 0xFull) << (4 * p);
    }
    __device__ __forceinline__ void rect(const int tx0, const int ty0, int &qx0, int &qx1, int &qy0, int &qy1) const {
        const uint32_t cols = (uint32_t)((any | (any >> 16) | (any >> 32) | (any >> 48)) & 0xFFFFull);
        if (cols == 0u) { qx0 = 1 << 20; qx1 = -1; qy0 = 1 << 20; qy1 = -1; return; }
        qx0 = tx0 + (int)__builtin_ctz(cols); qx1 = tx0 + 31 - (int)__builtin_clz(cols);
        qy0 = ty0 + (int)__builtin_ctz(rows); qy1 = ty0 + 31 - (int)__builtin_clz(rows);
    }
};

__device__ __forceinline__ int slot_of(uint64_t m) {
    return (int)__builtin_amdgcn_mbcnt_hi((uint32_t)(m >> 32), __builtin_amdgcn_mbcnt_lo((uint32_t)m, 0u));
}

struct Entry { float4 q0, q1, q2; float yhi; };
__device__ __forceinline__ Entry load_entry(const float4 *sp, const float *syhi, int k) {
    Entry e;
    e.q0 = sp[3 * k]; e.q1 = sp[3 * k + 1]; e.q2 = sp[3 * k + 2]; e.yhi = syhi[k];
    return e;
}

__device__ __forceinline__ uint32_t extend_tile_list(const GsCompositeArgs &a, const int tile, uint32_t &cont, uint32_t s1) {
    const int lane = threadIdx.x;
    const int tx = tile % a.gx, ty = tile / a.gx;
    const int sbs = a.sbs;
    const uint32_t sm = (1u << sbs) - 1u;
    const int S = (ty >> sbs) * a.sgx + (tx >> sbs);
    const uint32_t lx = (uint32_t)tx & sm, ly = (uint32_t)ty & sm;
    const uint32_t c1 = a.cranges[2 * S + 1];
    const uint32_t seg = (uint32_t)gs_bin3_seg_const();
    const uint32_t e_end = min(cont + seg, c1);
    for (uint32_t e0 = cont; e0 < e_end; e0 += GS_WAVE) {
        const uint32_t e = e0 + (uint32_t)lane;
        bool hit = false;
        uint32_t id = 0;
        if (e < e_end) {
            const uint32_t lr = a.clr[e];
            hit = (lr & sm) <= lx && lx <= ((lr >> sbs) & sm) && ((lr >> (2 * sbs)) & sm) <= ly && ly <= ((lr >> (3 * sbs)) & sm);
            id = a.cids[e];
        }
        const uint64_t bal = __ballot(hit);
        if (hit) a.ids_w[s1 + (uint32_t)slot_of(bal)] = id;
        s1 += (uint32_t)__popcll(bal);
    }
    cont = e_end < c1 ? e_end : GS_CONT_NONE;
    if (lane == 0 && a.ext_count) atomicAdd(a.ext_count, 1u);
    __threadfence();
    return s1;
}

template <bool EARLY, bool CULL, bool CLK, bool SLAB, bool SNAP = false>
__device__ __forceinline__ void forward_tile(const GsCompositeArgs &a, const int tile, const int part, const int nparts, float4 *sp, float *syhi, const float nbig,
                                             const int snap_slot = -1, const uint32_t seg_len = 0) {
    const int lane = threadIdx.x;
    const int px = (tile % a.gx) * GS_TILE + (lane & 15) + 1;
    const int py0 = (tile / a.gx) * GS_TILE + (lane >> 4) + 1;
    const float fx = (float)px;
    const uint32_t s0 = a.ranges[2 * tile];
    uint32_t s1 = a.ranges[2 * tile + 1];
    uint32_t cont = GS_CONT_NONE;
    const bool capped = !SLAB && EARLY && a.tile_ext != nullptr;
    if (capped) { const uint2 ex = a.tile_ext[tile]; s1 = s0 + ex.x; cont = ex.y; }
    const int ty0 = py0 - (lane >> 4);
    unsigned long long clk0 = 0;
    if (CLK) clk0 = __builtin_amdgcn_s_memrealtime();

    if (SLAB && a.resume && a.tile_done[tile]) return;
    const uint32_t gp0 = SLAB && a.tile_pos ? a.tile_pos[tile] : 0u;
    const uint32_t plane = (uint32_t)a.W * (uint32_t)a.H;
    float Cr[4], Cg[4], Cb[4], T[4], fy[4];
    bool dead[4];
    uint32_t walked = 0, evaluated = 0;
    constexpr bool PACK = GS_FWD_PACK && EARLY && !SLAB;
    const uint32_t own = (EARLY && !SLAB) ? strips_of_part(nparts, part) : 0xFu;
    bool first_pack = PACK && nparts > 1;
    int K = 4;
    uint32_t next_snap = (SNAP && snap_slot >= 0) ? seg_len : 0xFFFFFFFFu;
#pragma unroll
    for (int p = 0; p < 4; ++p) {
        Cr[p] = Cg[p] = Cb[p] = 0.0f;
        fy[p] = (float)(py0 + 4 * p);
        const bool in = (px <= a.W && py0 + 4 * p <= a.H) && ((own >> p) & 1u);
        T[p] = in ? 1.0f : 0.0f;
        dead[p] = !in;
        if (SLAB && a.resume && in) {
            const uint32_t o = (uint32_t)(px - 1) + (uint32_t)a.W * (uint32_t)(py0 + 4 * p - 1);
            Cr[p] = a.image[o]; Cg[p] = a.image[o + plane]; Cb[p] = a.image[o + 2u * plane];
            dead[p] = ((a.tile_dead[4 * (size_t)tile + p] >> lane) & 1ull) != 0ull;
            T[p] = dead[p] ? 0.0f : a.trans[o];
        }
    }
    int qx0, qx1, qy0, qy1;
    auto live_rect = [&]() {
        int lx0 = 1 << 20, lx1 = -1, ly0 = 1 << 20, ly1 = -1;
#pragma unroll
        for (int p = 0; p < 4; ++p) {
            if (!dead[p]) {
                const int x = (int)((!PACK || K == 4) ? fx : fy[2 + (p & 1)]), y = (int)fy[p];
                lx0 = min(lx0, x); lx1 = max(lx1, x); ly0 = min(ly0, y); ly1 = max(ly1, y);
            }
        }
        qx0 = wave_min_i32(lx0); qx1 = wave_max_i32(lx1); qy0 = wave_min_i32(ly0); qy1 = wave_max_i32(ly1);
        if (!GS_LIVE_RECT) { qx0 = (tile % a.gx) * GS_TILE + 1; qx1 = qx0 + GS_TILE - 1; qy0 = ty0; qy1 = ty0 + GS_TILE - 1; }
    };
    {
        qx0 = (tile % a.gx) * GS_TILE + 1; qx1 = min(qx0 + GS_TILE - 1, a.W);
        qy0 = ty0 + 4 * (int)__builtin_ctz(own); qy1 = min(ty0 + 4 * (31 - (int)__builtin_clz(own)) + 3, a.H);
        if (SLAB && a.resume) live_rect();
    }
    const float4 *pay4 = reinterpret_cast<const float4 *>(a.payload);
    float4 n0 = make_float4(0.f, 0.f, 0.f, 0.f), n1 = n0, n2 = n0, n3 = n0;
    uint32_t pos = s0 + lane;
    uint32_t id2 = 0;
    uint32_t gp = gp0;
    uint32_t base = s0;
    unsigned long long t_loop = 0, t_stage = 0, t_mark = 0;
    unsigned long long clk_exec = 0, clk_ideal = 0, clk_alive = 0, clk_pix = 0;
    uint32_t clk_live = 0, clk_strips = 0;
    uint32_t clk_hist[3][4] = {{0, 0, 0, 0}, {0, 0, 0, 0}, {0, 0, 0, 0}};
    int clk_k[3] = {4, 4, 4};
    uint32_t clk_bbkeep = 0;
    if (CLK) t_mark = __builtin_amdgcn_s_memtime();
    for (;;) {
    bool stopped = false;
    {
        const uint32_t pos2 = pos + min((uint32_t)CB - (gp & (CB - 1)), s1 - base);
        if (pos < s1) { const size_t g = a.ids[pos]; n0 = pay4[4 * g]; n1 = pay4[4 * g + 1]; n2 = pay4[4 * g + 2]; n3 = pay4[4 * g + 3]; }
        if (pos2 < s1) id2 = a.ids[pos2];
    }
    for (; base < s1;) {
        const uint32_t phase = gp & (CB - 1);
        const int cnt = (int)min((uint32_t)CB - phase, s1 - base);
        if (EARLY && phase == 0) {
            bool live = false, froze = false;
#pragma unroll
            for (int p = 0; p < 4; ++p) {
                if (!dead[p] && T[p] < a.t_min) {
                    const float x = (!PACK || K == 4) ? fx : fy[2 + (p & 1)];
                    if (a.trans) a.trans[(uint32_t)((int)x - 1) + (uint32_t)a.W * (uint32_t)((int)fy[p] - 1)] = T[p];
                    if (SNAP && snap_slot >= 0) {
                        const int nsn = a.seg_hist ? a.seg_n - 1 : GS_SEG_MAX - 1;
                        float *st = a.snap + (size_t)snap_slot * (size_t)(nsn * 4 * 256) + 768 + ((int)fy[p] - ty0) * GS_TILE + ((int)x - (px - (lane & 15)));
                        for (int kk = (int)(next_snap / seg_len) - 1; kk < nsn; ++kk) st[kk * (4 * 256)] = __int_as_float(0x7FC00000);
                    }
                    dead[p] = true; T[p] = 0.0f; froze = true;
                }
                live = live || !dead[p];
            }
            if (__ballot(live) == 0ull) { stopped = true; break; }
            const bool anyfroze = __ballot(froze) != 0ull;
            if (anyfroze) live_rect();
            if (PACK && K > 1 && (anyfroze || first_pack)) {
                first_pack = false;
                uint64_t lm[4];
                uint32_t nlive = 0;
#pragma unroll
                for (int p = 0; p < 4; ++p) { lm[p] = __ballot(!dead[p]); nlive += (uint32_t)__popcll(lm[p]); }
                const int Kn = (int)((nlive + 63u) >> 6);
                if (Kn <= 2 && Kn < K) {
#pragma unroll
                    for (int p = 0; p < 4; ++p) {
                        const float x = K == 4 ? fx : fy[2 + (p & 1)];
                        const bool mine = K == 4 ? (px <= a.W && py0 + 4 * p <= a.H && ((own >> p) & 1u)) : (p < 2 && x > 0.5f);
                        if (mine && dead[p] && a.image) {
                            const uint32_t o = (uint32_t)((int)x - 1) + (uint32_t)a.W * (uint32_t)((int)fy[p] - 1);
                            a.image[o] = Cr[p]; a.image[o + plane] = Cg[p]; a.image[o + 2u * plane] = Cb[p];
                        }

                    }
                    float *buf = reinterpret_cast<float *>(sp);
                    __syncthreads();
                    uint32_t rb = 0;
#pragma unroll
                    for (int p = 0; p < 4; ++p) {
                        if (!dead[p]) {
                            const uint32_t r = rb + (uint32_t)slot_of(lm[p]);
                            buf[r] = K == 4 ? fx : fy[2 + (p & 1)]; buf[128 + r] = fy[p];
                            buf[256 + r] = Cr[p]; buf[384 + r] = Cg[p]; buf[512 + r] = Cb[p]; buf[640 + r] = T[p];
                        }
                        rb += (uint32_t)__popcll(lm[p]);
                    }
                    __syncthreads();
#pragma unroll
                    for (int q = 0; q < 2; ++q) {
                        const uint32_t idx = (uint32_t)(q * 64 + lane);
                        const bool has = idx < nlive;
                        fy[2 + q] = has ? buf[idx] : 0.0f;
                        fy[q] = has ? buf[128 + idx] : 0.0f;
                        Cr[q] = has ? buf[256 + idx] : 0.0f; Cg[q] = has ? buf[384 + idx] : 0.0f; Cb[q] = has ? buf[512 + idx] : 0.0f;
                        T[q] = has ? buf[640 + idx] : 0.0f;
                        dead[q] = !has; dead[2 + q] = true;
                        T[2 + q] = 0.0f;
                    }
                    K = Kn;
                }
            }
        }
        if (SNAP && EARLY && !SLAB && gp == next_snap) {
            const int ksnap = (int)(next_snap / seg_len) - 1;
            const int nsn = a.seg_hist ? a.seg_n - 1 : GS_SEG_MAX - 1;
            if (ksnap < nsn) {
                float *sn = a.snap + (size_t)snap_slot * (size_t)(nsn * 4 * 256) + ksnap * (4 * 256);
#pragma unroll
                for (int p = 0; p < 4; ++p) {
                    if (!dead[p]) {
                        const float x = (!PACK || K == 4) ? fx : fy[2 + (p & 1)];
                        const int idx = ((int)fy[p] - ty0) * GS_TILE + ((int)x - (px - (lane & 15)));
                        sn[idx] = Cr[p]; sn[256 + idx] = Cg[p]; sn[512 + idx] = Cb[p]; sn[768 + idx] = T[p];
                    }
                }
            }
            next_snap += seg_len;
        }
        if (CLK && (phase == 0 || base == s0)) {
            clk_live = 0; clk_strips = 0;
            uint32_t rows = 0, colcnt[16];
            for (int cidx = 0; cidx < 16; ++cidx) colcnt[cidx] = 0;
#pragma unroll
            for (int p = 0; p < 4; ++p) {
                const uint64_t m = __ballot(!dead[p]); clk_live += (uint32_t)__popcll(m); clk_strips += m ? 1u : 0u;
                for (int r4 = 0; r4 < 4; ++r4) rows += ((m >> (16 * r4)) & 0xFFFFull) ? 1u : 0u;
                for (int cidx = 0; cidx < 16; ++cidx) colcnt[cidx] += (uint32_t)__popcll(m & (0x0001000100010001ull << cidx));
            }
            uint32_t cmax = 0;
            for (int cidx = 0; cidx < 16; ++cidx) cmax = max(cmax, colcnt[cidx]);
            clk_k[0] = (int)((clk_live + 63u) >> 6); clk_k[1] = (int)((rows + 3u) >> 2); clk_k[2] = (int)((cmax + 3u) >> 2);
        }
#if GS_FWD_NO_PREFETCH
        if (base > s0 && pos < s1) {
            const size_t g = a.ids[pos]; n0 = pay4[4 * g]; n1 = pay4[4 * g + 1]; n2 = pay4[4 * g + 2]; n3 = pay4[4 * g + 3];
        }
#endif
        uint32_t strips;
        bool keep;
        stage_record<false>(n0, n1, n3, qx0, qx1, qy0, qy1, ty0, keep, strips);
        int slot = lane, nk = cnt;
        if (!CULL) keep = true;
        if (CULL) {
            keep = keep && lane < cnt;
            const uint64_t m = __ballot(keep);
            slot = slot_of(m); nk = __popcll(m);
        }
        if (CLK && CULL) {
            bool k2; uint32_t st2;
            stage_record<false>(n0, n1, n3, px - (lane & 15), px - (lane & 15) + GS_TILE - 1, ty0, ty0 + GS_TILE - 1, ty0, k2, st2);
            clk_bbkeep += (uint32_t)__popcll(__ballot(k2 && lane < cnt));
        }
        __syncthreads();
        if (keep) {
            sp[3 * slot] = n0; sp[3 * slot + 1] = n1; sp[3 * slot + 2] = n2;
            syhi[slot] = n3.x;
        }
        __syncthreads();
        base += (uint32_t)cnt; gp += (uint32_t)cnt;
        pos = base + lane;
#if !GS_FWD_NO_PREFETCH
        {
            if (pos < s1) { const size_t g = id2; n0 = pay4[4 * g]; n1 = pay4[4 * g + 1]; n2 = pay4[4 * g + 2]; n3 = pay4[4 * g + 3]; }
            const uint32_t pos2 = pos + min((uint32_t)CB, s1 - base);
            if (base < s1 && pos2 < s1) id2 = a.ids[pos2];
        }
#endif
        if (CLK) { const unsigned long long t = __builtin_amdgcn_s_memtime(); t_stage += t - t_mark; t_mark = t; }
#define GS_FWD_PIXEL(e, A0, B0, p) do {                                               \
            const float dY = fy[p] - (e).q0.y;                                              \
            const float ey = dY - __builtin_amdgcn_fmed3f(dY, (e).q2.w, (e).yhi);           \
            const float pw = fmaf(dY, fmaf((e).q1.z, dY, (B0)), (A0));                      \
            const float w = fast_exp2(fmaf(nbig, fabsf(ey), pw)) * T[p];                    \
            Cr[p] = fmaf((e).q2.x, w, Cr[p]);                                               \
            Cg[p] = fmaf((e).q2.y, w, Cg[p]);                                               \
            Cb[p] = fmaf((e).q2.z, w, Cb[p]);                                               \
            T[p] = T[p] - w;                                                                \
        } while (0)
#define GS_FWD_COLUMN(e, XCOL, A0, B0)                                                        \
            const float dX##A0 = (XCOL) - (e).q0.x;                                           \
            const float ex##A0 = dX##A0 - __builtin_amdgcn_fmed3f(dX##A0, (e).q0.w, (e).q1.w);    \
            const float A0 = fmaf(nbig, fabsf(ex##A0), fmaf((e).q1.x * dX##A0, dX##A0, (e).q0.z));  \
            const float B0 = (e).q1.y * dX##A0
        if (!PACK || K == 4) {
#pragma clang loop unroll_count(kFwdUnroll)
            for (int k = 0; k < nk; ++k) {
                const Entry e = load_entry(sp, syhi, k);
                GS_FWD_COLUMN(e, fx, A0, B0);
                GS_FWD_PIXEL(e, A0, B0, 0); GS_FWD_PIXEL(e, A0, B0, 1); GS_FWD_PIXEL(e, A0, B0, 2); GS_FWD_PIXEL(e, A0, B0, 3);
            }
        } else if (K == 2) {
#pragma clang loop unroll_count(kFwdUnroll)
            for (int k = 0; k < nk; ++k) {
                const Entry e = load_entry(sp, syhi, k);
                GS_FWD_COLUMN(e, fy[2], A0, B0);
                GS_FWD_COLUMN(e, fy[3], A1, B1);
                GS_FWD_PIXEL(e, A0, B0, 0); GS_FWD_PIXEL(e, A1, B1, 1);
            }
        } else {
#pragma clang loop unroll_count(4)
            for (int k = 0; k < nk; ++k) {
                const Entry e = load_entry(sp, syhi, k);
                GS_FWD_COLUMN(e, fy[2], A0, B0);
                GS_FWD_PIXEL(e, A0, B0, 0);
            }
        }
#undef GS_FWD_PIXEL
#undef GS_FWD_COLUMN
        walked += (uint32_t)cnt; evaluated += (uint32_t)nk;
        first_use_here(n0, n1, n2, n3);
        if (CLK) {
            const unsigned long long t = __builtin_amdgcn_s_memtime(); t_loop += t - t_mark; t_mark = t;
            clk_exec += (unsigned long long)K * (uint32_t)nk; clk_ideal += (unsigned long long)nk * ((clk_live + 63u) >> 6);
            clk_alive += (unsigned long long)nk * clk_strips; clk_pix += (unsigned long long)nk * clk_live;
            for (int w = 0; w < 3; ++w) if (clk_k[w] >= 1 && clk_k[w] <= 4) clk_hist[w][clk_k[w] - 1] += (uint32_t)nk;
        }
    }
    if (!capped || stopped || cont == GS_CONT_NONE) break;
    s1 = extend_tile_list(a, tile, cont, s1);
    pos = base + lane;
    }
    if (capped && lane == 0) a.tile_ext[tile] = make_uint2(s1 - s0, cont);
    bool anylive = false;
#pragma unroll
    for (int p = 0; p < 4; ++p) anylive = anylive || !dead[p];
    const bool all_dead = __ballot(anylive) == 0ull;
    if (SLAB && a.tile_dead && !a.final_round) {
#pragma unroll
        for (int p = 0; p < 4; ++p) {
            const unsigned long long m = __ballot(dead[p]);
            if (lane == 0) a.tile_dead[4 * (size_t)tile + p] = m;
        }
    }
    if (SNAP && snap_slot >= 0 && lane == 0) {
        if (a.snap_walked) atomicMax(a.snap_walked + snap_slot, gp0 + walked);
        if (part == 0) { if (a.bw_walked) a.bw_walked[tile] = 0u; if (a.bw_work) a.bw_work[tile] = 0u; }
    }
    if (lane == 0 && part == 0) {
        if (a.tile_work) a.tile_work[tile] = SLAB && a.resume ? a.tile_work[tile] + evaluated : evaluated;
        if (a.tile_walked) a.tile_walked[tile] = SLAB && a.resume ? a.tile_walked[tile] + walked : walked;
        if (SLAB && a.tile_done) a.tile_done[tile] = all_dead ? 1 : 0;
        if (SLAB && a.tile_pos) a.tile_pos[tile] = gp0 + (s1 - s0);
    }
    if (PACK && K < 4) {
#pragma unroll
        for (int q = 0; q < 2; ++q) {
            if (fy[2 + q] > 0.5f) {
                const uint32_t o = (uint32_t)((int)fy[2 + q] - 1) + (uint32_t)a.W * (uint32_t)((int)fy[q] - 1);
                if (a.image) { a.image[o] = Cr[q]; a.image[o + plane] = Cg[q]; a.image[o + 2u * plane] = Cb[q]; }
                if (a.trans && !dead[q]) a.trans[o] = T[q];
            }
        }
    } else if (px <= a.W) {
#pragma unroll
        for (int p = 0; p < 4; ++p) {
            const int py = py0 + 4 * p;
            if (py <= a.H && ((own >> p) & 1u)) {
                const uint32_t o = (uint32_t)(px - 1) + (uint32_t)a.W * (uint32_t)(py - 1);
                if (a.image) { a.image[o] = Cr[p]; a.image[o + plane] = Cg[p]; a.image[o + 2u * plane] = Cb[p]; }
                if (a.trans && !(EARLY && dead[p])) a.trans[o] = T[p];
            }
        }
    }
    if (CLK && a.tile_clock && lane == 0) {
        unsigned long long *c = a.tile_clock + GS_TILE_CLOCK_WORDS * (size_t)(a.clock_by_block ? (int)blockIdx.x : tile);
        c[0] = clk0; c[1] = __builtin_amdgcn_s_memrealtime(); c[2] = wave_hw_id();
        c[3] = ((unsigned long long)walked << 32) | evaluated;
        c[4] = t_loop; c[5] = t_stage;
        c[6] = (clk_exec << 32) | (clk_ideal & 0xFFFFFFFFull); c[7] = (clk_alive << 32) | (clk_pix & 0xFFFFFFFFull);
        c[14] = clk_bbkeep;
        for (int w = 0; w < 3; ++w) {
            c[8 + 2 * w] = ((unsigned long long)clk_hist[w][0] << 32) | clk_hist[w][1];
            c[9 + 2 * w] = ((unsigned long long)clk_hist[w][2] << 32) | clk_hist[w][3];
        }
    }
}

template <bool EARLY, int MINW, bool CULL, bool CLK = false, bool SLAB = false, bool SNAP = false>
__global__ __launch_bounds__(64, MINW) void composite_fwd_kernel(GsCompositeArgs a) {
    __shared__ float4 sp[CB * 3];
    __shared__ float syhi[CB];
    const int ntiles = a.gx * a.gy;
    const float nbig = vgpr_const(-GS_BIG);
    int part, nparts;
    const int tile = tile_of_block(a, ntiles, part, nparts);
    if (tile < 0) return;
    int snap_slot = -1;
    uint32_t sl = 0;
    if (SNAP && EARLY && !SLAB && a.snap && a.seg_hist) {
        sl = gs_seg_len_all(a.seg_hist[tile], a.seg_n);
        if (sl) snap_slot = tile;
    } else if (SNAP && EARLY && !SLAB && a.snap && nparts > 1 && a.parts <= 1) {
        const int b = (int)blockIdx.x, slot = (b < a.front ? ((b >> 3) / 3) : ((b - a.front) >> 3)) * 8 + (b & 7);
        sl = a.seg_len[slot];
        if (sl) snap_slot = slot;
    }
    forward_tile<EARLY, CULL, CLK, SLAB, SNAP>(a, tile, part, nparts, sp, syhi, nbig, snap_slot, sl);
}

#define RS 68
#define RED_FLOATS (9 * RS)

template <bool DET>
__device__ __forceinline__ void add_to_row(const GsCompositeArgs &a, uint32_t gid, int ocomp, float v) {
    if (DET) {
        const float sc = fminf(fmaxf(v * (ocomp >= 6 ? GS_FIXED_SCALE2 : GS_FIXED_SCALE), -9.0e18f), 9.0e18f);
        char *rowp = reinterpret_cast<char *>(a.g2d_fixed) + (size_t)gid * (8 * GS_G2D_STRIDE);
        atomicAdd(reinterpret_cast<unsigned long long *>(rowp + 8u * (uint32_t)ocomp), (unsigned long long)__float2ll_rn(sc));
    } else {
        char *rowp = reinterpret_cast<char *>(a.g2d) + (size_t)gid * (4 * GS_G2D_STRIDE);
        atomicAdd(reinterpret_cast<float *>(rowp + 4u * (uint32_t)ocomp), v);
    }
}

__device__ __forceinline__ float dpp_xor1(float v) { return __int_as_float(__builtin_amdgcn_update_dpp(0, __float_as_int(v), 0xB1, 0xF, 0xF, true)); }
__device__ __forceinline__ float dpp_xor2(float v) { return __int_as_float(__builtin_amdgcn_update_dpp(0, __float_as_int(v), 0x4E, 0xF, 0xF, true)); }


__device__ __forceinline__ void backward_entry(const Entry &e, const float fx, const float (&fy)[4], const float nbig,
                                               const float (&dCr)[4], const float (&dCg)[4], const float (&dCb)[4],
                                               float (&T)[4], float (&S)[4], float (&v)[9], bool &any, const uint32_t live) {
    const float dX = fx - e.q0.x;
    const float ex = dX - __builtin_amdgcn_fmed3f(dX, e.q0.w, e.q1.w);
    const float A0 = fmaf(nbig, fabsf(ex), fmaf(e.q1.x * dX, dX, e.q0.z));
    const float B0 = e.q1.y * dX;
    float ar = 0.0f, ag = 0.0f, ab = 0.0f, q0s = 0.0f, q1s = 0.0f, q2s = 0.0f, asum = 0.0f;
#pragma unroll
    for (int p = 0; p < 4; ++p) {
        if (!((live >> p) & 1u)) continue;
        const float dY = fy[p] - e.q0.y;
        const float ey = dY - __builtin_amdgcn_fmed3f(dY, e.q2.w, e.yhi);
        const float xp = fmaf(nbig, fabsf(ey), fmaf(dY, fmaf(e.q1.z, dY, B0), A0));
        const float al = fast_exp2(xp);
        asum += al;
        const float w = al * T[p];
        const float cdot = fmaf(e.q2.x, dCr[p], fmaf(e.q2.y, dCg[p], e.q2.z * dCb[p]));
        S[p] = fmaf(-cdot, w, S[p]);
        const float inv = fast_rcp(1.0f - al);
        const float dalpha = fmaf(T[p], cdot, -(S[p] * inv));
        const float dd = -(al * dalpha);
        const float ddy = dd * dY;
        ar = fmaf(w, dCr[p], ar); ag = fmaf(w, dCg[p], ag); ab = fmaf(w, dCb[p], ab);
        q0s += dd; q1s += ddy; q2s = fmaf(ddy, dY, q2s);
        T[p] = T[p] - w;
    }
    any = asum != 0.0f;
    const float qx = dX * q0s;
    v[0] = ar; v[1] = ag; v[2] = ab; v[3] = q0s;
    v[4] = qx; v[5] = q1s;
    v[6] = dX * qx; v[7] = dX * q1s; v[8] = q2s;
}

template <bool EARLY, bool DET, bool CULL, bool CLK, bool PAIR = false>
__device__ __forceinline__ void backward_tile(const GsCompositeArgs &a, const int tile, const int part, const int nparts, float4 *sp, float *syhi, uint32_t *sid,
                                              uint32_t *sstrip, float *red, const float nbig, const float *snap_in = nullptr, const uint32_t seg_start = 0,
                                              const uint32_t seg_end = 0xFFFFFFFFu, const bool seg_tile = false) {
    const int lane = threadIdx.x;
    const int px = (tile % a.gx) * GS_TILE + (lane & 15) + 1;
    const int py0 = (tile / a.gx) * GS_TILE + (lane >> 4) + 1;
    const float fx = (float)px;
    const size_t plane = (size_t)a.W * a.H;
    const int ty0 = py0 - (lane >> 4);
    unsigned long long clk0 = 0;
    if (CLK) clk0 = __builtin_amdgcn_s_memrealtime();
    const int rl = lane < 36 ? lane : lane - 36;
    const float *rrow = red + (rl >> 2) * RS + (rl & 3) * 16;
    float *wrow = red + lane;
    const int ocomp_t = (lane < 36 && (lane & 3) == 0) ? ((lane >> 2) < 8 ? (lane >> 2) : 9) : -1;

    float dCr[4], dCg[4], dCb[4], T[4], S[4], fy[4];
    bool dead[4];
    uint32_t walked = 0, evaluated = 0;
    const uint32_t own = EARLY ? strips_of_part(nparts, part) : 0xFu;
#pragma unroll
    for (int p = 0; p < 4; ++p) {
        const int py = py0 + 4 * p;
        const bool in = (px <= a.W && py <= a.H) && ((own >> p) & 1u);
        const size_t o = in ? (size_t)(px - 1) + (size_t)a.W * (py - 1) : 0;
        fy[p] = (float)py;
        dCr[p] = in ? a.dC[o] : 0.0f;
        dCg[p] = in ? a.dC[o + plane] : 0.0f;
        dCb[p] = in ? a.dC[o + 2 * plane] : 0.0f;
        T[p] = in ? 1.0f : 0.0f;
        S[p] = in ? (a.image[o] * dCr[p] + a.image[o + plane] * dCg[p] + a.image[o + 2 * plane] * dCb[p]) : 0.0f;
        dead[p] = !in;
        if (snap_in && in) {
            const int idx = (lane >> 4) * GS_TILE + 64 * p + (lane & 15);
            const float tin = snap_in[768 + idx];
            if (tin != tin) { T[p] = 0.0f; S[p] = 0.0f; dead[p] = true; }
            else {
                T[p] = tin;
                S[p] = (a.image[o] - snap_in[idx]) * dCr[p] + (a.image[o + plane] - snap_in[256 + idx]) * dCg[p] + (a.image[o + 2 * plane] - snap_in[512 + idx]) * dCb[p];
            }
        }
    }
    int qx0, qx1, qy0, qy1;
    auto live_rect = [&]() {
        if (GS_RECT_FROM_MASKS && GS_LIVE_RECT) {
            LiveRectAcc acc;
#pragma unroll
            for (int p = 0; p < 4; ++p) acc.slot(p, __ballot(!dead[p]));
            acc.rect(px - (lane & 15), ty0, qx0, qx1, qy0, qy1);
            return;
        }
        int lx0 = 1 << 20, lx1 = -1, ly0 = 1 << 20, ly1 = -1;
#pragma unroll
        for (int p = 0; p < 4; ++p) {
            if (!dead[p]) { const int x = (int)fx, y = (int)fy[p]; lx0 = min(lx0, x); lx1 = max(lx1, x); ly0 = min(ly0, y); ly1 = max(ly1, y); }
        }
        qx0 = wave_min_i32(lx0); qx1 = wave_max_i32(lx1); qy0 = wave_min_i32(ly0); qy1 = wave_max_i32(ly1);
        if (!GS_LIVE_RECT) { qx0 = (tile % a.gx) * GS_TILE + 1; qx1 = qx0 + GS_TILE - 1; qy0 = ty0; qy1 = ty0 + GS_TILE - 1; }
    };
    qx0 = (tile % a.gx) * GS_TILE + 1; qx1 = min(qx0 + GS_TILE - 1, a.W);
    qy0 = ty0 + 4 * (int)__builtin_ctz(own); qy1 = min(ty0 + 4 * (31 - (int)__builtin_clz(own)) + 3, a.H);
    if (snap_in) live_rect();
    const float4 *pay4 = reinterpret_cast<const float4 *>(a.payload);
    float4 n0 = make_float4(0.f, 0.f, 0.f, 0.f), n1 = n0, n2 = n0, n3 = n0;
    uint32_t nid = 0;
    float4 r0 = make_float4(0.f, 0.f, 0.f, 0.f), r1 = r0, r2 = r0, r3 = r0;
    uint32_t pend_gid = 0;
    auto finish = [&]() {
        float s = ((r0.x + r0.y) + (r0.z + r0.w)) + ((r1.x + r1.y) + (r1.z + r1.w));
        s += ((r2.x + r2.y) + (r2.z + r2.w)) + ((r3.x + r3.y) + (r3.z + r3.w));
        s += dpp_xor1(s);
        s += dpp_xor2(s);
        if (ocomp_t >= 0) add_to_row<DET>(a, pend_gid, ocomp_t, s);
    };
    uint32_t gp = seg_start;
    uint32_t alive = own;
    bool stop = false;
    unsigned long long t_loop = 0, t_stage = 0, t_mark = 0;
    unsigned long long clk_exec = 0, clk_ideal = 0, clk_alive = 0, clk_pix = 0;
    uint32_t clk_live = 0, clk_strips = 0;
    if (CLK) t_mark = __builtin_amdgcn_s_memtime();
    for (int sg = 0; sg < a.nseg && !stop; ++sg) {
    const uint32_t *ids = a.seg_ids[sg];
    const uint32_t r0s = a.seg_ranges[sg][2 * tile];
    const uint32_t r1s = a.tile_ext ? r0s + a.tile_ext[tile].x : a.seg_ranges[sg][2 * tile + 1];
    const uint32_t s0 = min(r1s, r0s + seg_start), s1 = seg_end < r1s - r0s ? r0s + seg_end : r1s;
    uint32_t pos = s0 + lane;
    uint32_t id2 = 0;
    {
        const uint32_t pos2 = pos + min((uint32_t)CB - (gp & (CB - 1)), s1 - s0);
        if (pos < s1) { nid = ids[pos]; n0 = pay4[4 * (size_t)nid]; n1 = pay4[4 * (size_t)nid + 1]; n2 = pay4[4 * (size_t)nid + 2]; n3 = pay4[4 * (size_t)nid + 3]; }
        if (pos2 < s1) id2 = ids[pos2];
    }
    for (uint32_t base = s0; base < s1;) {
        const uint32_t phase = gp & (CB - 1);
        const int cnt = (int)min((uint32_t)CB - phase, s1 - base);
        if (EARLY && phase == 0) {
            bool live = false, froze = false;
            alive = 0;
#pragma unroll
            for (int p = 0; p < 4; ++p) {
                if (!dead[p] && T[p] < a.t_min) { dead[p] = true; T[p] = 0.0f; S[p] = 0.0f; froze = true; }
                live = live || !dead[p];
                if (__ballot(!dead[p]) != 0ull) alive |= 1u << p;
            }
            if (alive == 0u) { stop = true; break; }
            if (__ballot(froze) != 0ull) live_rect();
        }
        if (CLK && (phase == 0 || gp == 0)) {
            clk_live = 0; clk_strips = 0;
#pragma unroll
            for (int p = 0; p < 4; ++p) { const uint64_t m = __ballot(!dead[p]); clk_live += (uint32_t)__popcll(m); clk_strips += m ? 1u : 0u; }
        }
        uint32_t strips;
        bool keep;
        stage_record<CULL>(n0, n1, n3, qx0, qx1, qy0, qy1, ty0, keep, strips);
        if (CULL && EARLY) strips &= alive;
        int slot = lane, nk = cnt;
        if (!CULL) keep = true;
        uint64_t mq[4] = {~0ull, ~0ull, ~0ull, ~0ull};
        if (CULL) {
            keep = keep && lane < cnt;
            const uint64_t m = __ballot(keep);
            slot = slot_of(m); nk = __popcll(m);
        }
        __syncthreads();
        if (keep) {
            sp[3 * slot] = n0; sp[3 * slot + 1] = n1; sp[3 * slot + 2] = n2;
            syhi[slot] = n3.x;
            sid[slot] = nid;
            if (CULL) sstrip[slot] = strips;
        }
        __syncthreads();
        if (CULL) {
            const uint32_t mine = lane < nk ? sstrip[lane] : 0u;
#pragma unroll
            for (int p = 0; p < 4; ++p) mq[p] = __ballot((mine >> p) & 1u);
        }
        auto live_of = [&](int k) -> uint32_t {
            return (uint32_t)((mq[0] >> k) & 1ull) | ((uint32_t)((mq[1] >> k) & 1ull) << 1) | ((uint32_t)((mq[2] >> k) & 1ull) << 2)
                   | ((uint32_t)((mq[3] >> k) & 1ull) << 3);
        };
        base += (uint32_t)cnt; gp += (uint32_t)cnt;
        pos = base + lane;
        if (pos < s1) { nid = id2; n0 = pay4[4 * (size_t)nid]; n1 = pay4[4 * (size_t)nid + 1]; n2 = pay4[4 * (size_t)nid + 2]; n3 = pay4[4 * (size_t)nid + 3]; }
        {
            const uint32_t pos2 = pos + min((uint32_t)CB, s1 - base);
            if (base < s1 && pos2 < s1) id2 = ids[pos2];
        }
        if (CLK) { const unsigned long long t = __builtin_amdgcn_s_memtime(); t_stage += t - t_mark; t_mark = t; }
        int k = 0;
        if (PAIR) {
            float *wrow2 = wrow + RED_FLOATS;
            const float4 *rr = reinterpret_cast<const float4 *>(rrow), *rr2 = reinterpret_cast<const float4 *>(rrow + RED_FLOATS);
            for (; k + 1 < nk; k += 2) {
                const Entry ea = load_entry(sp, syhi, k), eb = load_entry(sp, syhi, k + 1);
                const uint32_t gida = (uint32_t)__builtin_amdgcn_readfirstlane((int)sid[k]), gidb = (uint32_t)__builtin_amdgcn_readfirstlane((int)sid[k + 1]);
                float va[9], vb[9];
                bool anya = true, anyb = true;
                backward_entry(ea, fx, fy, nbig, dCr, dCg, dCb, T, S, va, anya, live_of(k));
                backward_entry(eb, fx, fy, nbig, dCr, dCg, dCb, T, S, vb, anyb, live_of(k + 1));
#pragma unroll
                for (int c = 0; c < 9; ++c) { wrow[c * RS] = va[c]; wrow2[c * RS] = vb[c]; }
                const float4 a0 = rr[0], a1 = rr[1], a2 = rr[2], a3 = rr[3], b0 = rr2[0], b1 = rr2[1], b2 = rr2[2], b3 = rr2[3];
                r0 = a0; r1 = a1; r2 = a2; r3 = a3; pend_gid = gida; finish();
                r0 = b0; r1 = b1; r2 = b2; r3 = b3; pend_gid = gidb; finish();
            }
        }
        for (; k < nk; ++k) {
            const Entry e = load_entry(sp, syhi, k);
            const uint32_t gid = (uint32_t)__builtin_amdgcn_readfirstlane((int)sid[k]);
            float v[9];
            bool any = true;
            backward_entry(e, fx, fy, nbig, dCr, dCg, dCb, T, S, v, any, live_of(k));
            if (!CULL && __ballot(any) == 0ull) continue;
#pragma unroll
            for (int c = 0; c < 9; ++c) wrow[c * RS] = v[c];
            const float4 *rr = reinterpret_cast<const float4 *>(rrow);
            r0 = rr[0]; r1 = rr[1]; r2 = rr[2]; r3 = rr[3];
            pend_gid = gid;
            finish();
        }
        walked += (uint32_t)cnt; evaluated += (uint32_t)nk;
        first_use_here(n0, n1, n2, n3);
        if (CLK) {
            const unsigned long long t = __builtin_amdgcn_s_memtime(); t_loop += t - t_mark; t_mark = t;
            const uint64_t below = nk >= 64 ? ~0ull : ((1ull << nk) - 1ull);
            clk_exec += CULL ? (unsigned long long)(__popcll(mq[0] & below) + __popcll(mq[1] & below) + __popcll(mq[2] & below) + __popcll(mq[3] & below)) : 4ull * (uint32_t)nk;
            clk_ideal += (unsigned long long)nk * ((clk_live + 63u) >> 6);
            clk_alive += (unsigned long long)nk * clk_strips; clk_pix += (unsigned long long)nk * clk_live;
        }
    }
    }
    if (lane == 0 && part == 0) {
        if (a.walked) { atomicAdd(a.walked, (unsigned long long)walked); atomicAdd(a.walked + 1, (unsigned long long)evaluated); }
        if (seg_tile) {
            if (a.tile_walked) atomicAdd(a.tile_walked + tile, walked);
            if (a.tile_work) atomicAdd(a.tile_work + tile, evaluated);
        } else {
            if (a.tile_walked) a.tile_walked[tile] = walked;
            if (a.tile_work) a.tile_work[tile] = evaluated;
        }
    }
    if (CLK && a.tile_clock && lane == 0) {
        unsigned long long *c = a.tile_clock + GS_TILE_CLOCK_WORDS * (size_t)(a.clock_by_block ? (int)blockIdx.x : tile);
        c[0] = clk0; c[1] = __builtin_amdgcn_s_memrealtime(); c[2] = wave_hw_id();
        c[3] = ((unsigned long long)walked << 32) | evaluated;
        c[4] = t_loop; c[5] = t_stage;
        c[6] = (clk_exec << 32) | (clk_ideal & 0xFFFFFFFFull); c[7] = (clk_alive << 32) | (clk_pix & 0xFFFFFFFFull);
    }
}

template <bool EARLY, int MINW, bool DET, bool CULL, bool CLK = false, bool PAIR = false>
__global__ __launch_bounds__(64, MINW) void composite_bwd_kernel(GsCompositeArgs a) {
    __shared__ float4 sp[CB * 3];
    __shared__ float syhi[CB];
    __shared__ uint32_t sid[CB];
    __shared__ uint32_t sstrip[CB];
    __shared__ __attribute__((aligned(16))) float red[PAIR ? 2 * RED_FLOATS : RED_FLOATS];
    const int ntiles = a.gx * a.gy;
    const float nbig = vgpr_const(-GS_BIG);
    int part = 0, nparts = 1, tile;
    const float *snap_in = nullptr;
    uint32_t seg_start = 0, seg_end = 0xFFFFFFFFu;
    bool seg_tile = false;
    const int segunits = (EARLY && a.snap && !a.seg_hist) ? 8 * (a.front / 24) * (GS_SEG_MAX - 1) : 0;
    if (EARLY && a.snap && a.seg_hist) {
        const int len = ((ntiles + 7) / 8) * 8, unit = (int)blockIdx.x / len;
        tile = (int)blockIdx.x - unit * len;
        nparts = a.parts > 1 ? a.parts : 1; part = unit % nparts;
        const int k = unit / nparts;
        if (tile >= ntiles || k >= a.seg_n) return;
        const uint32_t sl = gs_seg_len_all(a.seg_hist[tile], a.seg_n);
        if (k > 0) {
            if (sl == 0u) return;
            snap_in = a.snap + (size_t)tile * (size_t)((a.seg_n - 1) * 4 * 256) + (size_t)(k - 1) * (4 * 256);
            seg_start = (uint32_t)k * sl;
        }
        if (sl) { seg_end = k == a.seg_n - 1 ? 0xFFFFFFFFu : seg_start + sl; seg_tile = true; }
    } else if ((int)blockIdx.x < segunits) {
        const int b = (int)blockIdx.x, x = b & 7, q = b >> 3, pos = q / (GS_SEG_MAX - 1), k = q - pos * (GS_SEG_MAX - 1) + 1, slot = 8 * pos + x;
        const uint32_t sl = a.seg_len[slot], t = a.tile_order[a.front + 8 * pos + x];
        if (sl == 0u || t == 0xFFFFFFFFu || (t >> 30) == 0u) return;
        const uint32_t wk = a.snap_walked[slot];
        if ((uint32_t)k * sl >= wk) return;
        tile = (int)(t & GS_ORDER_TILE_MASK);
        if (tile >= ntiles) return;
        snap_in = a.snap + (size_t)slot * GS_SEG_SNAP_FLOATS + (size_t)(k - 1) * (4 * 256);
        seg_start = (uint32_t)k * sl; seg_end = k == GS_SEG_MAX - 1 ? 0xFFFFFFFFu : seg_start + sl; seg_tile = true;
    } else {
        tile = tile_of_block(a, ntiles, part, nparts, segunits);
        if (tile < 0) return;
        if (segunits && nparts > 1) {
            const int b = (int)blockIdx.x - segunits, slot = (b < a.front ? ((b >> 3) / 3) : ((b - a.front) >> 3)) * 8 + (b & 7);
            const uint32_t sl = a.seg_len[slot];
            if (sl) {
                if (part) return;
                nparts = 1; seg_end = sl; seg_tile = true;
            }
        }
    }
    backward_tile<EARLY, DET, CULL, CLK, PAIR>(a, tile, part, nparts, sp, syhi, sid, sstrip, red, nbig, snap_in, seg_start, seg_end, seg_tile);
}

#ifndef GS_LPT_BUCKETS
#define GS_LPT_BUCKETS 32
#endif
#define GS_LPT_NONE 0xFFFFFFFFu
static inline int lpt_groups(int gx, int gy, int gs) { return ((gx + gs - 1) / gs) * ((gy + gs - 1) / gs); }
static inline int lpt_group_side(int gx, int gy) {
    for (int gs = 8; gs > 1; gs >>= 1) if (lpt_groups(gx, gy, gs) >= 128) return gs;
    return 1;
}
int gs_lpt_order_len(int gx, int gy) { const int gs = lpt_group_side(gx, gy); return 8 * gs * gs * ((lpt_groups(gx, gy, gs) + 7) / 8); }

__global__ __launch_bounds__(1024) void tile_lpt_order_kernel(const uint32_t *__restrict__ src, int ranges_mode, int ntiles, int gx, int ng, int gs, int nb,
                                                               uint32_t *__restrict__ order, unsigned long long *__restrict__ zero14, int front, int split_div,
                                                               const uint32_t *__restrict__ walked, uint32_t *__restrict__ zero_words,
                                                               uint32_t *__restrict__ host_nsplit) {
    extern __shared__ uint32_t lds[];
    __shared__ uint32_t wmax, wtot, nsplit;
    __shared__ uint32_t rowtot[8 * 32], rowstart[8 * 32], xcount[8];
    const int tid = threadIdx.x, lane = tid & 63, wv = tid >> 6;
    const int GT = gs * gs;
    const int ordmax = (ng + 7) >> 3;
    const int per = ordmax * GT;
    const int W = (per + 31) >> 5;
    const int rows = 8 * nb;
    const int ngx = (gx + gs - 1) / gs;
    uint32_t *bm = lds;
    uint32_t *gsum = bm + rows * W;
    uint16_t *pre = reinterpret_cast<uint16_t *>(gsum + ng);
    uint16_t *ginfo = pre + rows * W;
    uint8_t *cls = reinterpret_cast<uint8_t *>(ginfo + ng + (ng & 1) + ((rows * W) & 1));
    for (int i = tid; i < rows * W + ng; i += 1024) bm[i] = 0;
    for (int i = tid; i < front; i += 1024) order[i] = GS_LPT_NONE;
    uint32_t *seg_len = order + front + 8 * per;
    if (front > 0) for (int i = tid; i < front / 3; i += 1024) { seg_len[i] = 0; if (zero_words) zero_words[i] = 0; }
    if (tid == 0) { wmax = 1; nsplit = 0; }
    if (zero14 && tid < 14) zero14[tid] = 0ull;
    __syncthreads();
    auto load8 = [&](int t0, uint32_t (&v)[8]) {
#pragma unroll
        for (int k = 0; k < 8; ++k) {
            const int t = t0 + k * 1024 + tid;
            v[k] = 0;
            if (t < ntiles) v[k] = ranges_mode ? src[2 * t + 1] - src[2 * t] : src[t];
        }
    };
    auto group_of = [&](int t, int &local) {
        const int ty = t / gx, tx = t - ty * gx;
        local = (ty & (gs - 1)) * gs + (tx & (gs - 1));
        return (ty / gs) * ngx + tx / gs;
    };
    uint32_t m = 0;
    for (int t0 = 0; t0 < ntiles; t0 += 8 * 1024) {
        uint32_t v[8];
        load8(t0, v);
#pragma unroll
        for (int k = 0; k < 8; ++k) {
            const int t = t0 + k * 1024 + tid;
            m = max(m, v[k]);
            if (t < ntiles && v[k]) { int local; atomicAdd(&gsum[group_of(t, local)], v[k]); }
        }
    }
#pragma unroll
    for (int d = 32; d > 0; d >>= 1) m = max(m, (uint32_t)__shfl_xor((int)m, d));
    if (lane == 0) atomicMax(&wmax, m);
    __syncthreads();
    if (wv == 0) {
        uint32_t sw = 0;
        for (int g = lane; g < ng; g += 64) sw += gsum[g];
#pragma unroll
        for (int d = 32; d > 0; d >>= 1) sw += (uint32_t)__shfl_xor((int)sw, d);
        if (lane == 0) wtot = sw;
    }
    for (int g = tid; g < ng; g += 1024) {
        const uint32_t mine = gsum[g];
        int rank = 0;
        for (int h = 0; h < ng; ++h) { const uint32_t o = gsum[h]; rank += (o > mine || (o == mine && h < g)) ? 1 : 0; }
        const int r = rank >> 3, x = (r & 1) ? 7 - (rank & 7) : (rank & 7);
        ginfo[g] = (uint16_t)(x | (r << 3));
    }
    __syncthreads();
    const float scale = (float)nb / (float)wmax;
    for (int t0 = 0; t0 < ntiles; t0 += 8 * 1024) {
        uint32_t v[8];
        load8(t0, v);
#pragma unroll
        for (int k = 0; k < 8; ++k) {
            const int t = t0 + k * 1024 + tid;
            if (t < ntiles) {
                const int c = min(nb - 1, max(0, nb - 1 - (int)((float)v[k] * scale)));
                cls[t] = (uint8_t)c;
                int local;
                const uint32_t gi = ginfo[group_of(t, local)];
                const int i = (int)(gi >> 3) * GT + local;
                atomicOr(&bm[((int)(gi & 7u) * nb + c) * W + (i >> 5)], 1u << (i & 31));
            }
        }
    }
    __syncthreads();
    for (int r = wv; r < rows; r += 16) {
        uint32_t carry = 0;
        for (int w0 = 0; w0 < W; w0 += 64) {
            const int w = w0 + lane;
            const uint32_t c = w < W ? (uint32_t)__popc(bm[r * W + w]) : 0u;
            uint32_t incl = c;
#pragma unroll
            for (int d = 1; d < 64; d <<= 1) { const uint32_t u = __shfl_up(incl, d); if (lane >= d) incl += u; }
            if (w < W) pre[r * W + w] = (uint16_t)(carry + incl - c);
            carry += (uint32_t)__shfl((int)incl, 63);
        }
        if (lane == 0) rowtot[r] = carry;
    }
    __syncthreads();
    if (tid < 8) {
        uint32_t run = 0;
        for (int c = 0; c < nb; ++c) { rowstart[tid * nb + c] = run; run += rowtot[tid * nb + c]; }
        xcount[tid] = run;
    }
    __syncthreads();
    uint32_t *main_order = order + front;
    for (int i = tid; i < 8 * per; i += 1024)
        if ((uint32_t)(i >> 3) >= xcount[i & 7]) main_order[i] = GS_LPT_NONE;
    const uint32_t thr = front > 0 ? max(wtot / (uint32_t)max(split_div, 1), 256u) : 0xFFFFFFFFu, eligible = (uint32_t)front / 24u;
    for (int t = tid; t < ntiles; t += 1024) {
        int local;
        const uint32_t gi = ginfo[group_of(t, local)];
        const int x = (int)(gi & 7u), r = x * nb + cls[t], i = (int)(gi >> 3) * GT + local;
        const uint32_t pos = rowstart[r] + pre[r * W + (i >> 5)] + (uint32_t)__popc(bm[r * W + (i >> 5)] & ((1u << (i & 31)) - 1u));
        uint32_t entry = (uint32_t)t;
        if (pos < eligible) {
            const uint32_t w = ranges_mode ? src[2 * t + 1] - src[2 * t] : src[t];
            if (w >= thr) {
                const uint32_t pc = w >= 2u * thr ? 2u : 1u, extra = (1u << pc) - 1u;
                for (uint32_t j = 0; j < extra; ++j) order[8u * (3u * pos + j) + (uint32_t)x] = (uint32_t)t | ((j + 1u) << 28) | (pc << 30);
                entry |= pc << 30;
                atomicAdd(&nsplit, 1u);
                if (walked) {
                    const uint32_t wk = walked[t], per_seg = (wk + GS_SEG_MAX - 1) / GS_SEG_MAX;
                    const uint32_t sl = max((per_seg + 63u) & ~63u, (uint32_t)GS_SEG_MIN_LEN);
                    seg_len[8u * pos + (uint32_t)x] = wk > sl ? sl : 0u;
                }
            }
        }
        main_order[8u * pos + (uint32_t)x] = entry;
    }
    if (host_nsplit) {
        __syncthreads();
        if (tid == 0) *host_nsplit = nsplit;
    }
}

hipError_t gs_launch_tile_lpt_order(const uint32_t *work_or_ranges, int ranges_mode, int gx, int gy, uint32_t *order, hipStream_t s,
                                    unsigned long long *zero14, int buckets, int front, int split_div, const uint32_t *walked, uint32_t *zero_words, uint32_t *host_nsplit) {
    const int ntiles = gx * gy;
    if (ntiles <= 0) return hipSuccess;
    if (ntiles > GS_LPT_MAX_TILES) return hipErrorInvalidValue;
    int nb = buckets > 0 && buckets <= 32 ? buckets : GS_LPT_BUCKETS;
    const int gs = lpt_group_side(gx, gy), ng = lpt_groups(gx, gy, gs), W = (gs_lpt_order_len(gx, gy) / 8 + 31) / 32;
    auto lds_of = [&](int b) { return (size_t)8 * b * W * 4 + (size_t)ng * 4 + ((size_t)8 * b * W + ng + 2) * 2 + (size_t)ntiles + 16; };
    while (nb > 2 && lds_of(nb) > 150 * 1024) nb >>= 1;
    const size_t lds = lds_of(nb);
    if (lds > 150 * 1024) return hipErrorInvalidValue;
    if (lds > 40 * 1024) {
        hipError_t e = hipFuncSetAttribute(reinterpret_cast<const void *>(tile_lpt_order_kernel), hipFuncAttributeMaxDynamicSharedMemorySize, (int)lds);
        if (e != hipSuccess) return e;
    }
    if (front < 0 || (front % 24) || ntiles > (int)GS_ORDER_TILE_MASK) return hipErrorInvalidValue;
    hipLaunchKernelGGL(tile_lpt_order_kernel, dim3(1), dim3(1024), lds, s, work_or_ranges, ranges_mode, ntiles, gx, ng, gs, nb, order, zero14, front, split_div, walked, zero_words, host_nsplit);
    return hipGetLastError();
}

__global__ __launch_bounds__(1024) void sum_tiles_kernel(const uint32_t *__restrict__ a, const uint32_t *__restrict__ b, int n,
                                                          unsigned long long *__restrict__ out) {
    __shared__ unsigned long long sm[2][16];
    unsigned long long sa = 0, sb = 0;
    for (int i = threadIdx.x; i < n; i += 1024) { if (a) sa += a[i]; if (b) sb += b[i]; }
#pragma unroll
    for (int d = 32; d > 0; d >>= 1) { sa += __shfl_down(sa, d); sb += __shfl_down(sb, d); }
    if ((threadIdx.x & 63) == 0) { sm[0][threadIdx.x >> 6] = sa; sm[1][threadIdx.x >> 6] = sb; }
    __syncthreads();
    if (threadIdx.x < 2) { unsigned long long t = 0; for (int k = 0; k < 16; ++k) t += sm[threadIdx.x][k]; out[threadIdx.x] = t; }
}
__global__ __launch_bounds__(1024) void sum_listed_kernel(const uint2 *__restrict__ ext, int n, unsigned long long *__restrict__ out) {
    __shared__ unsigned long long sm[16];
    unsigned long long sa = 0;
    for (int i = threadIdx.x; i < n; i += 1024) sa += ext[i].x;
#pragma unroll
    for (int d = 32; d > 0; d >>= 1) sa += __shfl_down(sa, d);
    if ((threadIdx.x & 63) == 0) sm[threadIdx.x >> 6] = sa;
    __syncthreads();
    if (threadIdx.x == 0) { unsigned long long t = 0; for (int k = 0; k < 16; ++k) t += sm[k]; out[0] = t; }
}
hipError_t gs_launch_sum_listed(const uint2 *ext, int n, unsigned long long *out, hipStream_t s) {
    hipLaunchKernelGGL(sum_listed_kernel, dim3(1), dim3(1024), 0, s, ext, n, out);
    return hipGetLastError();
}
hipError_t gs_launch_sum_tiles(const uint32_t *a, const uint32_t *b, int n, unsigned long long *out, hipStream_t s) {
    hipLaunchKernelGGL(sum_tiles_kernel, dim3(1), dim3(1024), 0, s, a, b, n, out);
    return hipGetLastError();
}

__global__ void clock_probe_kernel(unsigned long long *__restrict__ out) {
    const unsigned long long r0 = __builtin_amdgcn_s_memrealtime(), c0 = __builtin_amdgcn_s_memtime();
    unsigned long long r1 = r0;
    for (int i = 0; i < (1 << 20) && r1 - r0 < 2000ull; ++i) r1 = __builtin_amdgcn_s_memrealtime();
    const unsigned long long c1 = __builtin_amdgcn_s_memtime();
    if (threadIdx.x == 0) { out[0] = c1 - c0; out[1] = r1 - r0; }
}
hipError_t gs_launch_clock_probe(unsigned long long *out, hipStream_t s) {
    hipLaunchKernelGGL(clock_probe_kernel, dim3(1), dim3(64), 0, s, out);
    return hipGetLastError();
}

int gs_seg_units(int front) { return 8 * (front / 24) * (GS_SEG_MAX - 1); }
static dim3 composite_grid(const GsCompositeArgs &a, int ntiles, bool bwd = false) {
    const int len = (a.tile_order && a.order_len > 0) ? a.order_len : ((ntiles + 7) / 8) * 8;
    if (bwd && a.snap && a.seg_hist && a.t_min > 0.0f) return dim3((unsigned)(len * a.seg_n * (a.parts > 1 ? a.parts : 1)));
    return dim3((unsigned)(len * (a.parts > 1 ? a.parts : 1) + ((bwd && a.snap && a.t_min > 0.0f) ? gs_seg_units(a.front) : 0)));
}

int gs_composite_grid_blocks(const GsCompositeArgs &a, int bwd) { return (int)composite_grid(a, a.gx * a.gy, bwd != 0).x; }

static GsCompositeArgs apply_sched_variant(const GsCompositeArgs &a0) {
    GsCompositeArgs a = a0;
    if ((a.variant / 10) % 10 == 1) { a.tile_order = nullptr; a.order_len = 0; a.split_ok = 0; }
    return a;
}

hipError_t gs_launch_composite_fwd(const GsCompositeArgs &a0, hipStream_t s) {
    const GsCompositeArgs a = apply_sched_variant(a0);
    const int ntiles = a.gx * a.gy;
    if (ntiles <= 0) return hipSuccess;
    const dim3 grid = composite_grid(a, ntiles), block(64);
    const bool early = a.t_min > 0.0f;
    if (a.parts > 1 && ((a.parts != 2 && a.parts != 4) || !early || a.tile_ext || a.tile_pos || (a.tile_clock && !a.clock_by_block))) return hipErrorInvalidValue;
    if (a.split_ok && (!early || a.tile_ext || a.tile_pos || a.parts > 1)) return hipErrorInvalidValue;
    if (a.snap && !a.seg_hist && (!a.split_ok || !a.seg_len || !a.snap_walked || !a.tile_order || a.front <= 0)) return hipErrorInvalidValue;
    if (a.snap && a.seg_hist && (a.tile_order || a.seg_n < 2 || a.seg_n > GS_SEG_MAX || !early || a.tile_ext || a.tile_pos)) return hipErrorInvalidValue;
    if (a.tile_ext && (gs_bin3_seg() != L2_SEG || !early || !a.cranges || !a.cids || !a.clr || !a.ids_w || a.tile_pos)) return hipErrorInvalidValue;
    if (a.tile_pos) {
        if (!early || a.tile_clock) return hipErrorInvalidValue;
        if (a.cull) hipLaunchKernelGGL((composite_fwd_kernel<true, 4, true, false, true>), grid, block, 0, s, a);
        else hipLaunchKernelGGL((composite_fwd_kernel<true, 4, false, false, true>), grid, block, 0, s, a);
        return hipGetLastError();
    }
    if (a.tile_clock) {
        if (!a.cull) return hipErrorInvalidValue;
        if (early) hipLaunchKernelGGL((composite_fwd_kernel<true, GS_FWD_MINW, true, true>), grid, block, 0, s, a);
        else hipLaunchKernelGGL((composite_fwd_kernel<false, GS_FWD_MINW, true, true>), grid, block, 0, s, a);
        return hipGetLastError();
    }
    if (early && a.snap) {
        if (a.cull) hipLaunchKernelGGL((composite_fwd_kernel<true, GS_FWD_MINW, true, false, false, true>), grid, block, 0, s, a);
        else hipLaunchKernelGGL((composite_fwd_kernel<true, GS_FWD_MINW, false, false, false, true>), grid, block, 0, s, a);
    } else if (early) {
        if (a.cull) hipLaunchKernelGGL((composite_fwd_kernel<true, GS_FWD_MINW, true>), grid, block, 0, s, a);
        else hipLaunchKernelGGL((composite_fwd_kernel<true, GS_FWD_MINW, false>), grid, block, 0, s, a);
    } else {
        if (a.cull) hipLaunchKernelGGL((composite_fwd_kernel<false, GS_FWD_MINW, true>), grid, block, 0, s, a);
        else hipLaunchKernelGGL((composite_fwd_kernel<false, GS_FWD_MINW, false>), grid, block, 0, s, a);
    }
    return hipGetLastError();
}

hipError_t gs_launch_composite_bwd(const GsCompositeArgs &a0, hipStream_t s) {
    const GsCompositeArgs a = apply_sched_variant(a0);
    const int ntiles = a.gx * a.gy;
    if (ntiles <= 0) return hipSuccess;
    const bool early = a.t_min > 0.0f;
    const dim3 grid = composite_grid(a, ntiles, true), block(64);
    if (a.snap && !a.seg_hist && (!a.split_ok || !a.seg_len || !a.snap_walked || !a.tile_order || a.front <= 0)) return hipErrorInvalidValue;
    if (a.snap && a.seg_hist && (a.tile_order || a.seg_n < 2 || a.seg_n > GS_SEG_MAX || !early || a.tile_ext || a.nseg > 1)) return hipErrorInvalidValue;
    if (a.parts > 1 && ((a.parts != 2 && a.parts != 4) || !early || a.tile_ext || a.nseg > 1 || (a.tile_clock && !a.clock_by_block))) return hipErrorInvalidValue;
    if (a.split_ok && (!early || a.tile_ext || a.nseg > 1 || a.parts > 1)) return hipErrorInvalidValue;
#define GS_B2(E, D) do { if (a.cull) hipLaunchKernelGGL((composite_bwd_kernel<E, GS_BWD_MINW, D, true>), grid, block, 0, s, a); \
                         else hipLaunchKernelGGL((composite_bwd_kernel<E, GS_BWD_MINW, D, false>), grid, block, 0, s, a); } while (0)
#define GS_B(E) do { if (a.g2d_fixed) GS_B2(E, true); else GS_B2(E, false); } while (0)
    if (a.tile_clock) {
        if (!a.cull || a.g2d_fixed) return hipErrorInvalidValue;
        if (early) hipLaunchKernelGGL((composite_bwd_kernel<true, 5, false, true, true>), grid, block, 0, s, a);
        else hipLaunchKernelGGL((composite_bwd_kernel<false, 5, false, true, true>), grid, block, 0, s, a);
        return hipGetLastError();
    }
    if (GS_BWD_PAIR && early && a.cull && !a.tile_order && (a.parts > 1 || a.seg_hist)) {
        if (a.g2d_fixed) hipLaunchKernelGGL((composite_bwd_kernel<true, 2, true, true, false, true>), grid, block, 0, s, a);
        else hipLaunchKernelGGL((composite_bwd_kernel<true, 2, false, true, false, true>), grid, block, 0, s, a);
        return hipGetLastError();
    }
    if (early) GS_B(true); else GS_B(false);
#undef GS_B
#undef GS_B2
    return hipGetLastError();
}
```

### gaussiansplat_amd/csrc/gs_ctx.h

```cpp
#pragma once
#include "../../include/gsplat.h"
#include "gs_common.h"

#include <rccl/rccl.h>

#include <algorithm>
#include <cmath>
#include <cstdio>
#include <cstdlib>
#include <cstring>
#include <new>
#include <string>
#include <vector>

struct DevBuf {
    void *p = nullptr;
    size_t cap = 0;
    hipError_t ensure(size_t bytes) {
        if (bytes <= cap) return hipSuccess;
        if (p) { hipError_t e = hipFree(p); p = nullptr; cap = 0; if (e != hipSuccess) return e; }
        size_t want = bytes + bytes / 8 + 256;
        hipError_t e = hipMalloc(&p, want);
        if (e == hipSuccess) cap = want;
        return e;
    }
    void release() { if (p) (void)hipFree(p); p = nullptr; cap = 0; }
    template <typename T> T *as() const { return static_cast<T *>(p); }
};

extern std::string g_create_error;

#define GS_COUNTER_BYTES 192
struct gs_ctx {
    int device = 0;
    hipStream_t stream = nullptr;
    bool own_stream = false, borrowed_stream = false;
    gs_config cfg{};
    std::string err;

    int64_t n = 0;
    int sh_degree = 0;
    int kind = 0;
    size_t width[5] = {3, 3, 4, 1, 3};
    int order() const { return kind == 1 ? (int)GS_ORDER_INDEX : cfg.order; }
    const float *means = nullptr, *scales = nullptr, *quats = nullptr, *opac = nullptr, *shs = nullptr;
    DevBuf model[5];
    GsCamera cam{};
    bool have_cam = false, did_pre = false, did_bin = false, did_fwd = false, did_bwd = false, did_bwd_composite = false;
    int gx = 0, gy = 0;

    DevBuf invcov;
    DevBuf payload, depth_key, rect, pairs_a, pairs_b, perm, offsets, block_sums;
    DevBuf inst_a, inst_b, table, digit_total, ranges, image, trans, g2d, stage_in;
    DevBuf dbg[7];
    DevBuf ids, words, cs, diff;
    uint32_t *perm_ptr = nullptr;
    int64_t n_inst = 0;
    uint32_t *pinned = nullptr;
    const float *last_dC = nullptr;

    hipEvent_t ev_count = nullptr;
    hipEvent_t ev[GS_STAGE_COUNT][2] = {};
    bool ev_valid[GS_STAGE_COUNT] = {};
    bool ev_fresh[GS_STAGE_COUNT] = {};
    double ev_sum[GS_STAGE_COUNT] = {};
    int64_t ev_cnt[GS_STAGE_COUNT] = {};
    DevBuf counters;
    DevBuf tile_work, tile_clock;
    int view_slot = -1;
    struct ViewSlot {
        DevBuf order[2];
        int sel = 0;
        int64_t tiles = 0;
        DevBuf walkbuf[2];
        int wsel = 0;
        int64_t walked_grid = 0;
        DevBuf &walked() { return walkbuf[wsel]; }
    };
    std::vector<ViewSlot> slots;
    const uint32_t *last_walked = nullptr;
    bool frame_capped = false;
    int frame_parts = 1;
    int wave_slots = 5120;
    const uint32_t *cap_src = nullptr;
    DevBuf tile_nopen, smax, tile_ext, zero_tiles;
    GsBin3Args last_l2{};
    bool have_l2 = false;
    const uint32_t *frame_order = nullptr;
    DevBuf snap, snap_walked;
    const uint32_t *snap_order = nullptr;
    int frame_seg_n = 0;
    const uint32_t *seg_hist = nullptr;
    uint32_t *pinned_split = nullptr;
    const uint32_t *frame_order_split = nullptr;
    int snap_parity = 0;
    hipStream_t side = nullptr;
    hipEvent_t ev_main = nullptr, ev_order = nullptr;
    bool order_pending = false;
    bool pending_totals = false;
    bool spec_lists = false;
    size_t spec_cap_coarse = 0, spec_cap_fine = 0;
    int64_t n_coarse = 0;
    DevBuf tile_dead;
    int dbg_win_start = 0, dbg_win_len = 0;
    int rank_probe = -1;
    int n_rounds = 1;
    int64_t slab_lo[GS_MAX_ROUNDS + 1] = {};
    int64_t round_gen[GS_MAX_ROUNDS] = {};
    size_t round_ids_off[GS_MAX_ROUNDS] = {};
    DevBuf ranges_r[GS_MAX_ROUNDS];
    DevBuf tile_pos, tile_done, live2d, rect_r, offsets_r, live_total;
    uint32_t *perm_all = nullptr;
    bool two_level = false;
    int sgx = 0, sgy = 0, sbs = 3;
    int64_t coarse_listed = 0;
    DevBuf rect_sorted, l1_table, l1_rows, l1_partials, cids, clr, cranges, segcnt, sdone, tilecnt;
    uint32_t *bin_totals() { return counters.as<uint32_t>() + 32; }
    uint32_t *ext_count() { return counters.as<uint32_t>() + 36; }
    DevBuf tile_walked, tile_walked_b, tile_work_b;
    int64_t counters_grid = 0;
    DevBuf key_range;
    int range_parity = 0;
    bool range_valid = false;
    bool dsort_buckets_used = false;
    int64_t dsort_classic_until = 0;
    int dsort_stat_parity = 0;
    uint32_t *dsort_stat() { return pinned + 100 + (dsort_stat_parity & 1); }
    bool dsort_can_bucket() const {
        return cfg.depth_sort != 1 && (cfg.depth_sort == 2 || (n <= gs_depth_buckets_max_n() && frame_id > dsort_classic_until));
    }
    bool small_bin = false;
    bool perm_pending = false;
    bool g2d_clean = false;
    bool small_bin_possible() const {
        if (cfg.bin_path != 0 || cfg.depth_sort != 0 || cfg.list_cap == 2 || cfg.slab_fractions[0] > 0.0f) return false;
        if (cfg.debug_flags & (GS_DEBUG_WIDE_CURSORS | GS_DEBUG_SUPER8 | GS_DEBUG_SUPER16 | GS_DEBUG_TINY_CAPS)) return false;
        return gs_bin_small_supported(n, gx, gy);
    }
    float *bound_image = nullptr, *bound_trans = nullptr;
    float *img() { return bound_image ? bound_image : image.as<float>(); }
    float *tr() { return bound_trans ? bound_trans : trans.as<float>(); }
    int tile_bits = 0, gid_bits = 0, lo_bits = 0, hi_bits = 0;
    bool fast_bin = false;
    double walked_ratio = -1.0;
    int64_t prev_n_inst = 0;
    bool prev_counters_valid = false;
    int64_t frame_id = 0, ev_frame[GS_STAGE_COUNT] = {};
    int64_t ev_counted[GS_STAGE_COUNT] = {};
    DevBuf grads_flat;
    DevBuf dpc;
    DevBuf loss_maps, loss_acc, loss_in[2], loss_dc, view_cams;
    ncclComm_t comm = nullptr;
    int comm_ranks = 0;
};

inline int fail(gs_ctx *c, int code, const std::string &msg) {
    if (c) c->err = msg; else g_create_error = msg;
    return code;
}
inline int hipfail(gs_ctx *c, hipError_t e, const char *what) {
    std::string m = std::string(what) + ": " + hipGetErrorString(e);
    return fail(c, e == hipErrorOutOfMemory ? GS_ERR_OOM : GS_ERR_HIP, m);
}
#define HIPCHK(c, call)                                              \
    do {                                                             \
        hipError_t e__ = (call);                                     \
        if (e__ != hipSuccess) return hipfail((c), e__, #call);      \
    } while (0)

inline bool harvest_stage(gs_ctx *c, int s) {
    if (!c->ev_fresh[s]) return true;
    float ms = 0.0f;
    if (hipEventElapsedTime(&ms, c->ev[s][0], c->ev[s][1]) != hipSuccess) { (void)hipGetLastError(); return false; }
    c->ev_sum[s] += ms;
    if (c->ev_counted[s] != c->ev_frame[s]) { c->ev_counted[s] = c->ev_frame[s]; c->ev_cnt[s] += 1; }
    c->ev_fresh[s] = false;
    return true;
}
struct StageTimer {
    gs_ctx *c; int st; bool on;
    StageTimer(gs_ctx *c_, int st_) : c(c_), st(st_), on(c_->cfg.profile_stages == 1 || c_->cfg.profile_stages == 2 + st_) {
        if (on) {
            if (c->ev_fresh[st] && !harvest_stage(c, st)) {
                (void)hipEventSynchronize(c->ev[st][1]);
                (void)harvest_stage(c, st);
            }
            c->ev_frame[st] = c->frame_id;
            (void)hipEventRecord(c->ev[st][0], c->stream);
        }
    }
    ~StageTimer() {
        if (on) { (void)hipEventRecord(c->ev[st][1], c->stream); c->ev_valid[st] = true; c->ev_fresh[st] = true; }
    }
};

inline void harvest_events(gs_ctx *c, int skip_stage = -1) {
    if (!c->cfg.profile_stages) return;
    for (int s = 0; s < GS_STAGE_COUNT; ++s)
        if (s != skip_stage) (void)harvest_stage(c, s);
}

inline int bind_device(gs_ctx *c) {
    HIPCHK(c, hipSetDevice(c->device));
    return GS_OK;
}

inline bool lpt_schedule(const gs_ctx *c) {
    return (c->cfg.schedule == 3 || c->cfg.schedule == 4) && ((int64_t)c->gx * c->gy > c->wave_slots || (c->cfg.debug_flags & GS_DEBUG_ALWAYS_ORDER));
}
inline int lpt_front(const gs_ctx *c) {
    const int64_t ntiles = (int64_t)c->gx * c->gy;
    return (lpt_schedule(c) && c->cfg.tile_parts == 0 && c->cfg.t_min > 0.0f && 2 * ntiles > c->wave_slots && ntiles <= GS_LPT_MAX_TILES) ? GS_LPT_FRONT : 0;
}
inline const uint32_t *order_seg_len(const gs_ctx *c, const uint32_t *order) { return order + lpt_front(c) + gs_lpt_order_len(c->gx, c->gy); }
inline int lpt_order_entries(const gs_ctx *c) { return lpt_front(c) + gs_lpt_order_len(c->gx, c->gy); }
inline int lpt_split_div(const gs_ctx *c) { return c->wave_slots * 4 / 5; }
inline bool use_side_stream(const gs_ctx *c) { return c->n >= 262144 || (c->cfg.debug_flags & GS_DEBUG_ALWAYS_ORDER); }
inline int order_index(const gs_ctx *c) { return c->view_slot >= 0 ? c->view_slot : GS_MAX_VIEW_SLOTS; }

int settle_totals(gs_ctx *c, bool *redo, bool may_relist);
int bin_round(gs_ctx *c, int r);
int depth_order(gs_ctx *c, uint32_t **perm_out);
void comm_release(gs_ctx *c);
const uint32_t *forward_order(gs_ctx *c);
int build_frame_order(gs_ctx *c, const uint32_t *used);
```

### include/gsplat.h

```cpp
#ifndef GSPLAT_H
#define GSPLAT_H

#include <stdint.h>

#ifdef __cplusplus
extern "C" {
#endif

#define GS_ABI_VERSION 3

typedef enum {
    GS_OK = 0,
    GS_ERR_INVALID = -1,
    GS_ERR_NO_DEVICE = -2,
    GS_ERR_HIP = -3,
    GS_ERR_OOM = -4,
    GS_ERR_UNSUPPORTED = -5
} gs_status;

typedef enum { GS_MEM_HOST = 0, GS_MEM_DEVICE = 1 } gs_mem;

typedef enum { GS_ORDER_INDEX = 0, GS_ORDER_DEPTH_DESC = 1, GS_ORDER_DEPTH_ASC = 2 } gs_order;

typedef struct {
    int32_t struct_size;
    int32_t abi_version;
    int32_t tile_size;
    int32_t order;
    float   t_min;
    int32_t deterministic;
    int32_t export_debug;
    int32_t profile_stages;
    int32_t bin_path;
    int32_t rank_mode;
    int32_t alpha_cull;
    int32_t schedule;
    int32_t slab_mode;
    float   slab_max_ratio;
    float   slab_fractions[3];
    int32_t debug_flags;
    int32_t depth_sort;
    int32_t list_cap;
    int32_t tile_parts;
    int32_t reserved[3];
} gs_config;
#define GS_DEBUG_WIDE_CURSORS 1
#define GS_DEBUG_ALWAYS_ORDER 2
#define GS_DEBUG_SUPER16 8
#define GS_DEBUG_SUPER8 16
#define GS_DEBUG_TINY_CAPS 4

typedef struct gs_ctx gs_ctx;

void gs_default_config(gs_config *cfg);

int gs_abi_version(void);

int gs_create(gs_ctx **out, int device, const gs_config *cfg);
int gs_destroy(gs_ctx *ctx);
const char *gs_last_error(const gs_ctx *ctx);

#define GS_STREAM_LEGACY ((void *)1)
int gs_set_stream(gs_ctx *ctx, void *hip_stream);
int gs_synchronize(gs_ctx *ctx);

int gs_set_model(gs_ctx *ctx, int64_t n, int sh_degree,
                 const float *means, const float *scales, const float *quats,
                 const float *opacities, const float *shs, int mem);

int gs_set_model_2d(gs_ctx *ctx, int64_t n, const float *means, const float *scales, const float *rotations,
                    const float *opacities, const float *colors, int mem);
int gs_set_image_size(gs_ctx *ctx, int32_t W, int32_t H);

int gs_set_camera(gs_ctx *ctx, const float T[16], const float P[16], float fx, float fy,
                  float near_, float far_, const float eye[3], const float lookAt[3],
                  int32_t W, int32_t H);

#define GS_MAX_VIEW_SLOTS 4096
int gs_set_view_slot(gs_ctx *ctx, int32_t slot);

int gs_preprocess(gs_ctx *ctx);

int gs_bin(gs_ctx *ctx, int32_t gx, int32_t gy);

int gs_bind_outputs(gs_ctx *ctx, float *image_dev, float *transmittance_dev);

int gs_forward(gs_ctx *ctx, float *image, float *transmittance, int mem);

typedef struct {
    float *d_means;
    float *d_scales;
    float *d_quats;
    float *d_opacities;
    float *d_shs;
} gs_grads;

int gs_backward(gs_ctx *ctx, const float *dC, int mem, const gs_grads *grads);

#define GS_BWD_OVERWRITE 1
#define GS_BWD_COMPOSITE_ONLY 2
#define GS_BWD_PARAMS_ONLY 4
#define GS_BWD_PARAMS_SH 8
#define GS_BWD_PARAMS_GEOM 16
int gs_backward_ex(gs_ctx *ctx, const float *dC, int mem, const gs_grads *grads, int flags);
int gs_backward_sgd(gs_ctx *ctx, const float *dC, int mem, float lr);

int gs_reset_grads(gs_ctx *ctx, const gs_grads *grads);

int gs_grads_alloc(gs_ctx *ctx, gs_grads *out);
int gs_grads_read(gs_ctx *ctx, const gs_grads *grads, float *h_means, float *h_scales, float *h_quats,
                  float *h_opacities, float *h_shs);


#define GS_VIEW_RECORD_FLOATS 38
int gs_color_grads_pack(gs_ctx *ctx, float *drgb);
int gs_sh_grads_from_views(gs_ctx *ctx, int32_t nviews, const float *cams, const float *drgb, float *d_shs, int flags);

#define GS_COMM_ID_BYTES 128
int gs_comm_unique_id(void *id128);
int gs_comm_init(gs_ctx *ctx, int rank, int nranks, const void *id128);
int gs_allreduce_grads(gs_ctx *ctx, const gs_grads *grads);
int gs_comm_destroy(gs_ctx *ctx);


int gs_loss_l1_dssim(gs_ctx *ctx, const float *img, const float *gt, int32_t W, int32_t H, int32_t C, float lam,
                     float *dC, double *loss_out, int mem);

int gs_sgd_step(gs_ctx *ctx, float lr, const gs_grads *grads);


typedef enum {
    GS_ARR_TS = 0,
    GS_ARR_TPS = 1,
    GS_ARR_MU = 2,
    GS_ARR_COV3D = 3,
    GS_ARR_COV2D = 4,
    GS_ARR_INVCOV = 5,
    GS_ARR_BBS = 6,
    GS_ARR_RGB = 7,
    GS_ARR_SIG = 8,
    GS_ARR_DEPTH_KEY = 9,
    GS_ARR_TILE_RECT = 10,
    GS_ARR_SORT_IDXS = 11,
    GS_ARR_TILE_RANGES = 12,
    GS_ARR_SORTED_IDS = 13,
    GS_ARR_SORTED_KEYS = 14,
    GS_ARR_GRAD2D = 15
} gs_array;

int64_t gs_num_gaussians(const gs_ctx *ctx);
int64_t gs_num_instances(gs_ctx *ctx);
int64_t gs_num_coarse_instances(gs_ctx *ctx);
int gs_num_rounds(const gs_ctx *ctx);

int gs_get_array(gs_ctx *ctx, int which, void *host_dst, int64_t bytes);

typedef enum {
    GS_STAGE_PREPROCESS = 0, GS_STAGE_DEPTH_SORT, GS_STAGE_COUNT_SCAN, GS_STAGE_EMIT,
    GS_STAGE_TILE_SORT, GS_STAGE_RANGES, GS_STAGE_COMPOSITE_FWD, GS_STAGE_COMPOSITE_BWD,
    GS_STAGE_PREPROCESS_BWD, GS_STAGE_COUNT
} gs_stage;

int gs_get_stage_times(gs_ctx *ctx, float ms[GS_STAGE_COUNT]);

int gs_get_stage_stats(gs_ctx *ctx, double sum_ms[GS_STAGE_COUNT], int64_t count[GS_STAGE_COUNT], int reset);

int gs_get_work_counters(gs_ctx *ctx, int64_t *walked_fwd, int64_t *walked_bwd);

int gs_get_list_stats(gs_ctx *ctx, int64_t out[3]);

int gs_get_tile_parts(gs_ctx *ctx);

int gs_get_bin_path(gs_ctx *ctx);

int gs_get_work_counters_ex(gs_ctx *ctx, int64_t out[4]);

int gs_debug_time_composite(gs_ctx *ctx, int which, int variant, int reps, float *mean_ms);

int gs_debug_tile_clock(gs_ctx *ctx, int which, int variant, uint64_t *out);
int gs_debug_tile_clock_rows(gs_ctx *ctx);

int gs_debug_clock_mhz(gs_ctx *ctx, float *mhz);

int gs_debug_set_window(gs_ctx *ctx, int32_t start, int32_t len);

int gs_rank_probe_result(const gs_ctx *ctx);

#ifdef __cplusplus
}
#endif
#endif
```

Measured before the change: 817.8 Msplats/s.

## Split heavy LPT-ordered tiles in two for backward using forward transmittance snapshots

```diff
diff --git a/gaussiansplat_amd/backend.py b/gaussiansplat_amd/backend.py
--- a/gaussiansplat_amd/backend.py
+++ b/gaussiansplat_amd/backend.py
@@ -23,7 +23,8 @@
            "gs_comm_init", "gs_allreduce_grads", "gs_comm_destroy", "gs_color_grads_pack", "gs_sh_grads_from_views", "gs_grads_alloc", "gs_grads_read", "gs_num_gaussians", "gs_num_instances", "gs_get_array",
            "gs_get_stage_times", "gs_get_stage_stats", "gs_get_work_counters", "gs_get_work_counters_ex", "gs_debug_time_composite",
            "gs_debug_tile_clock", "gs_debug_clock_mhz", "gs_rank_probe_result", "gs_num_rounds", "gs_set_view_slot", "gs_num_coarse_instances",
-           "gs_get_list_stats", "gs_get_tile_parts", "gs_get_bin_path", "gs_debug_set_window", "gs_debug_tile_clock_rows")
+           "gs_get_list_stats", "gs_get_tile_parts", "gs_get_bin_path", "gs_debug_set_window", "gs_debug_tile_clock_rows",
+           "gs_debug_set_seg_fraction")
 
 GS_ABI_VERSION = 3
 GS_DEBUG_WIDE_CURSORS = 1
@@ -117,6 +118,7 @@
     L.gs_get_bin_path.argtypes = [vp]
     L.gs_debug_set_window.argtypes = [vp, C.c_int32, C.c_int32]
     L.gs_debug_tile_clock_rows.argtypes = [vp]
+    L.gs_debug_set_seg_fraction.argtypes = [vp, C.c_float]
     if L.gs_abi_version() != GS_ABI_VERSION:
         raise RuntimeError(f"{LIB_PATH} has ABI version {L.gs_abi_version()}, this binding is written for {GS_ABI_VERSION}: "
                            "rebuild with `python -m gaussiansplat_amd.build --force`")
@@ -407,6 +409,9 @@
     def set_debug_window(self, start: int = 0, length: int = 0):
         self._chk(self.L.gs_debug_set_window(self.h, start, length))
 
+    def set_seg_fraction(self, f: float = -1.0):
+        self._chk(self.L.gs_debug_set_seg_fraction(self.h, f))
+
     def clock_mhz(self) -> float:
         mhz = C.c_float()
         self._chk(self.L.gs_debug_clock_mhz(self.h, C.byref(mhz)))
diff --git a/gaussiansplat_amd/csrc/gs_api_composite.hip b/gaussiansplat_amd/csrc/gs_api_composite.hip
--- a/gaussiansplat_amd/csrc/gs_api_composite.hip
+++ b/gaussiansplat_amd/csrc/gs_api_composite.hip
@@ -21,7 +21,7 @@
     const int k = order_index(c);
     const int dst = used ? 1 - c->slots[k].sel : c->slots[k].sel;
     DevBuf &ob = c->slots[k].order[dst];
-    HIPCHK(c, ob.ensure(sizeof(uint32_t) * ((size_t)lpt_order_entries(c) + GS_SEG_SLOTS + 16)));
+    HIPCHK(c, ob.ensure(sizeof(uint32_t) * order_words(c)));
     const uint32_t *walked = lpt_front(c) > 0 ? c->last_walked : nullptr;
     uint32_t *rearm = nullptr, *nsplit = c->pinned_split ? c->pinned_split + 2 * k + dst : nullptr;
     if (nsplit) *nsplit = 0xFFFFFFFFu;
@@ -108,6 +108,17 @@
         a.bw_walked = c->tile_walked_b.as<uint32_t>(); a.bw_work = c->tile_work_b.as<uint32_t>();
         c->snap_order = order;
     }
+    c->snap_order_u = nullptr; c->frame_useg = 0;
+    const int useg = uniform_seg_entries(c);
+    if (a.split_ok && useg > 0) {
+        HIPCHK(c, c->snap_u.ensure(sizeof(float) * (size_t)useg * 4 * 256));
+        const size_t nt = (size_t)c->gx * c->gy;
+        HIPCHK(c, c->tile_walked_b.ensure(sizeof(uint32_t) * (nt ? nt : 1)));
+        HIPCHK(c, c->tile_work_b.ensure(sizeof(uint32_t) * (nt ? nt : 1)));
+        a.snap_u = c->snap_u.as<float>(); a.seg_len_u = order_seg_len_u(c, order); a.useg = useg; a.front = lpt_front(c);
+        a.bw_walked = c->tile_walked_b.as<uint32_t>(); a.bw_work = c->tile_work_b.as<uint32_t>();
+        c->snap_order_u = order; c->frame_useg = useg;
+    }
     if (c->frame_capped && R == 1) {
         a.tile_ext = c->tile_ext.as<uint2>(); a.cranges = c->cranges.as<uint32_t>(); a.cids = c->cids.as<uint32_t>(); a.clr = c->clr.as<uint16_t>();
         a.ids_w = c->ids.as<uint32_t>(); a.sgx = c->sgx; a.sbs = c->sbs; a.ext_count = c->ext_count();
@@ -141,7 +152,7 @@
             DevBuf &wb = vs.walkbuf[vs.wsel ^ 1];
             HIPCHK(c, wb.ensure(sizeof(uint32_t) * (ntiles ? ntiles : 1)));
             const bool hist = vs.walked_grid == c->counters_grid && vs.walked().p;
-            if (hist && c->cfg.tile_parts == 0 && c->cfg.t_min > 0.0f && c->n_rounds == 1 && !c->frame_capped && !lpt_schedule(c) && c->kind == 0 &&
+            if (hist && c->cfg.tile_parts == 0 && !c->cfg.deterministic && c->cfg.t_min > 0.0f && c->n_rounds == 1 && !c->frame_capped && !lpt_schedule(c) && c->kind == 0 &&
                 2 * (int64_t)ntiles <= c->wave_slots && ntiles > 0) {
                 c->frame_seg_n = 2;
                 c->seg_hist = vs.walked().as<uint32_t>();
@@ -259,6 +270,15 @@
             a.snap = c->snap.as<float>(); a.seg_len = order_seg_len(c, a.tile_order); a.front = lpt_front(c);
             a.snap_walked = c->snap_walked.as<uint32_t>() + (size_t)c->snap_parity * GS_SEG_SLOTS;
         }
+        if (a.split_ok && c->snap_order_u && c->snap_order_u == a.tile_order) {
+            a.snap_u = c->snap_u.as<float>(); a.seg_len_u = order_seg_len_u(c, a.tile_order); a.useg = c->frame_useg; a.front = lpt_front(c);
+            a.fwd_walked = c->last_walked;
+        }
+        if (c->did_bwd_composite && (a.snap || a.snap_u)) {
+            const size_t nt = (size_t)c->gx * c->gy;
+            HIPCHK(c, hipMemsetAsync(c->tile_walked_b.p, 0, sizeof(uint32_t) * nt, c->stream));
+            HIPCHK(c, hipMemsetAsync(c->tile_work_b.p, 0, sizeof(uint32_t) * nt, c->stream));
+        }
         {
             StageTimer t(c, GS_STAGE_COMPOSITE_BWD);
             HIPCHK(c, gs_launch_composite_bwd(a, c->stream));
diff --git a/gaussiansplat_amd/csrc/gs_api_debug.hip b/gaussiansplat_amd/csrc/gs_api_debug.hip
--- a/gaussiansplat_amd/csrc/gs_api_debug.hip
+++ b/gaussiansplat_amd/csrc/gs_api_debug.hip
@@ -180,6 +180,10 @@
         a.snap = c->snap.as<float>(); a.seg_len = order_seg_len(c, a.tile_order); a.front = lpt_front(c);
         a.snap_walked = c->snap_walked.as<uint32_t>() + (size_t)c->snap_parity * GS_SEG_SLOTS;
     }
+    if (which == 1 && a.split_ok && c->snap_order_u && c->snap_order_u == a.tile_order) {
+        a.snap_u = c->snap_u.as<float>(); a.seg_len_u = order_seg_len_u(c, a.tile_order); a.useg = c->frame_useg; a.front = lpt_front(c);
+        a.fwd_walked = c->last_walked;
+    }
     a.parts = c->frame_parts;
     if (which == 1 && c->frame_seg_n && c->n_rounds == 1 && !c->frame_capped && !a.tile_order) {
         const long long nt = (long long)c->gx * c->gy;
@@ -190,7 +194,15 @@
         if (!a.tile_order || a.parts > 1) return fail(c, GS_ERR_INVALID, "gs_debug_set_window: the frame has no launch order (or several waves per tile)");
         if (c->dbg_win_start + c->dbg_win_len > a.order_len) return fail(c, GS_ERR_INVALID, "gs_debug_set_window: beyond the launch order");
         a.tile_order += c->dbg_win_start; a.order_len = c->dbg_win_len;
-    }
+        a.snap_u = nullptr;
+    }
+    return GS_OK;
+}
+
+int gs_debug_set_seg_fraction(gs_ctx *c, float f) {
+    if (!c) return GS_ERR_INVALID;
+    if (!(f <= 1.0f)) return fail(c, GS_ERR_INVALID, "gs_debug_set_seg_fraction: f must be at most 1 (negative: the library's choice)");
+    c->seg_frac = f;
     return GS_OK;
 }
 
@@ -239,8 +251,8 @@
         if ((!a.tile_order && a.parts <= 1 && !a.seg_hist) || (a.variant / 10) % 10 == 1)
             return fail(c, GS_ERR_INVALID, "gs_debug_tile_clock: records by workgroup need the frame's launch order (or a small grid's tile parts)");
         a.clock_by_block = 1;
-    } else { a.split_ok = 0; a.snap = nullptr; }
-    const size_t rows = !a.clock_by_block ? ntiles : a.tile_order ? (size_t)(lpt_order_entries(c) + gs_seg_units(lpt_front(c))) : (size_t)gs_debug_tile_clock_rows(c);
+    } else { a.split_ok = 0; a.snap = nullptr; a.snap_u = nullptr; }
+    const size_t rows = !a.clock_by_block ? ntiles : (size_t)gs_debug_tile_clock_rows(c);
     if (a.clock_by_block && (size_t)gs_composite_grid_blocks(a, which) > rows) return fail(c, GS_ERR_INVALID, "gs_debug_tile_clock: launch larger than its record");
     HIPCHK(c, c->tile_clock.ensure(sizeof(uint64_t) * GS_TILE_CLOCK_WORDS * (rows ? rows : 1)));
     HIPCHK(c, hipMemsetAsync(c->tile_clock.p, 0, sizeof(uint64_t) * GS_TILE_CLOCK_WORDS * rows, c->stream));
@@ -255,7 +267,7 @@
 
 int gs_debug_tile_clock_rows(gs_ctx *c) {
     if (!c) return GS_ERR_INVALID;
-    if (lpt_schedule(c)) return lpt_order_entries(c) + gs_seg_units(lpt_front(c));
+    if (lpt_schedule(c)) return lpt_order_entries(c) + gs_seg_units(lpt_front(c)) + c->frame_useg;
     const int len = ((c->gx * c->gy + 7) / 8) * 8;
     const int units = std::max(c->frame_parts, 1) * (c->frame_seg_n ? 4 * c->frame_seg_n : 1);
     return units > 1 ? len * units : 0;
diff --git a/gaussiansplat_amd/csrc/gs_common.h b/gaussiansplat_amd/csrc/gs_common.h
--- a/gaussiansplat_amd/csrc/gs_common.h
+++ b/gaussiansplat_amd/csrc/gs_common.h
@@ -257,6 +257,10 @@
     uint32_t *bw_walked, *bw_work;
     const uint32_t *seg_hist;
     int seg_n;
+    float *snap_u;
+    const uint32_t *seg_len_u;
+    int useg;
+    const uint32_t *fwd_walked;
     int clock_by_block;
 };
 hipError_t gs_launch_sum_listed(const uint2 *ext, int n, unsigned long long *out, hipStream_t s);
@@ -264,6 +268,12 @@
 int gs_lpt_order_len(int gx, int gy);
 hipError_t gs_launch_clock_probe(unsigned long long *out, hipStream_t s);
 hipError_t gs_launch_sum_tiles(const uint32_t *a, const uint32_t *b, int n, unsigned long long *out, hipStream_t s);
+#ifndef GS_BWD_MINW
+#define GS_BWD_MINW 6
+#endif
+#ifndef GS_SEG_UNIFORM_FRAC
+#define GS_SEG_UNIFORM_FRAC 0.25f
+#endif
 #define GS_LPT_FRONT 2304
 #define GS_SEG_MAX 8
 #define GS_SEG_MIN_LEN 1024
@@ -273,6 +283,10 @@
 hipError_t gs_launch_tile_lpt_order(const uint32_t *work_or_ranges, int ranges_mode, int gx, int gy, uint32_t *order, hipStream_t s,
                                     unsigned long long *zero14 = nullptr, int buckets = 0, int front = 0, int split_div = 1,
                                     const uint32_t *walked = nullptr, uint32_t *zero_words = nullptr, uint32_t *host_nsplit = nullptr);
+__host__ __device__ inline uint32_t gs_seg_len_two(uint32_t w) {
+    const uint32_t sl = ((w * 5u + 7u) / 8u + 63u) & ~63u;
+    return w > sl ? sl : 0u;
+}
 #ifndef GS_SEG_ALL_NUM
 #define GS_SEG_ALL_NUM 5
 #define GS_SEG_ALL_DEN 8
diff --git a/gaussiansplat_amd/csrc/gs_composite.hip b/gaussiansplat_amd/csrc/gs_composite.hip
--- a/gaussiansplat_amd/csrc/gs_composite.hip
+++ b/gaussiansplat_amd/csrc/gs_composite.hip
@@ -2,9 +2,6 @@
 
 #pragma clang fp contract(off)
 
-#ifndef GS_BWD_MINW
-#define GS_BWD_MINW 6
-#endif
 #ifndef GS_FWD_MINW
 #define GS_FWD_MINW 5
 #endif
@@ -177,6 +174,13 @@
     return s1;
 }
 
+#define GS_SNAP_UNIFORM 0x40000000
+__device__ __forceinline__ int snaps_per_tile(const GsCompositeArgs &a, int snap_slot) {
+    return (snap_slot & GS_SNAP_UNIFORM) ? 1 : a.seg_hist ? a.seg_n - 1 : GS_SEG_MAX - 1;
+}
+__device__ __forceinline__ float *snap_of(const GsCompositeArgs &a, int snap_slot, int nsn) {
+    return (snap_slot & GS_SNAP_UNIFORM) ? a.snap_u + (size_t)(snap_slot & (GS_SNAP_UNIFORM - 1)) * (4 * 256) : a.snap + (size_t)snap_slot * (size_t)(nsn * 4 * 256);
+}
 template <bool EARLY, bool CULL, bool CLK, bool SLAB, bool SNAP = false>
 __device__ __forceinline__ void forward_tile(const GsCompositeArgs &a, const int tile, const int part, const int nparts, float4 *sp, float *syhi, const float nbig,
                                              const int snap_slot = -1, const uint32_t seg_len = 0) {
@@ -267,8 +271,8 @@
                     const float x = (!PACK || K == 4) ? fx : fy[2 + (p & 1)];
                     if (a.trans) a.trans[(uint32_t)((int)x - 1) + (uint32_t)a.W * (uint32_t)((int)fy[p] - 1)] = T[p];
                     if (SNAP && snap_slot >= 0) {
-                        const int nsn = a.seg_hist ? a.seg_n - 1 : GS_SEG_MAX - 1;
-                        float *st = a.snap + (size_t)snap_slot * (size_t)(nsn * 4 * 256) + 768 + ((int)fy[p] - ty0) * GS_TILE + ((int)x - (px - (lane & 15)));
+                        const int nsn = snaps_per_tile(a, snap_slot);
+                        float *st = snap_of(a, snap_slot, nsn) + 768 + ((int)fy[p] - ty0) * GS_TILE + ((int)x - (px - (lane & 15)));
                         for (int kk = (int)(next_snap / seg_len) - 1; kk < nsn; ++kk) st[kk * (4 * 256)] = __int_as_float(0x7FC00000);
                     }
                     dead[p] = true; T[p] = 0.0f; froze = true;
@@ -326,9 +330,9 @@
         }
         if (SNAP && EARLY && !SLAB && gp == next_snap) {
             const int ksnap = (int)(next_snap / seg_len) - 1;
-            const int nsn = a.seg_hist ? a.seg_n - 1 : GS_SEG_MAX - 1;
+            const int nsn = snaps_per_tile(a, snap_slot);
             if (ksnap < nsn) {
-                float *sn = a.snap + (size_t)snap_slot * (size_t)(nsn * 4 * 256) + ksnap * (4 * 256);
+                float *sn = snap_of(a, snap_slot, nsn) + ksnap * (4 * 256);
 #pragma unroll
                 for (int p = 0; p < 4; ++p) {
                     if (!dead[p]) {
@@ -456,7 +460,7 @@
         }
     }
     if (SNAP && snap_slot >= 0 && lane == 0) {
-        if (a.snap_walked) atomicMax(a.snap_walked + snap_slot, gp0 + walked);
+        if (a.snap_walked && !(snap_slot & GS_SNAP_UNIFORM)) atomicMax(a.snap_walked + snap_slot, gp0 + walked);
         if (part == 0) { if (a.bw_walked) a.bw_walked[tile] = 0u; if (a.bw_work) a.bw_work[tile] = 0u; }
     }
     if (lane == 0 && part == 0) {
@@ -517,6 +521,12 @@
         const int b = (int)blockIdx.x, slot = (b < a.front ? ((b >> 3) / 3) : ((b - a.front) >> 3)) * 8 + (b & 7);
         sl = a.seg_len[slot];
         if (sl) snap_slot = slot;
+    } else if (SNAP && EARLY && !SLAB && a.snap_u && nparts == 1 && a.parts <= 1) {
+        const int m = (int)blockIdx.x - a.front;
+        if (m >= 0 && m < a.useg) {
+            sl = a.seg_len_u[m];
+            if (sl) snap_slot = m | GS_SNAP_UNIFORM;
+        }
     }
     forward_tile<EARLY, CULL, CLK, SLAB, SNAP>(a, tile, part, nparts, sp, syhi, nbig, snap_slot, sl);
 }
@@ -814,6 +824,15 @@
             seg_start = (uint32_t)k * sl;
         }
         if (sl) { seg_end = k == a.seg_n - 1 ? 0xFFFFFFFFu : seg_start + sl; seg_tile = true; }
+    } else if (EARLY && a.snap_u && (int)blockIdx.x >= segunits + a.order_len) {
+        const int m = (int)blockIdx.x - segunits - a.order_len;
+        if (m >= a.useg) return;
+        const uint32_t sl = a.seg_len_u[m], t = a.tile_order[a.front + m];
+        if (sl == 0u || t == 0xFFFFFFFFu || (t >> 28)) return;
+        tile = (int)(t & GS_ORDER_TILE_MASK);
+        if (tile >= ntiles || a.fwd_walked[tile] <= sl) return;
+        snap_in = a.snap_u + (size_t)m * (4 * 256);
+        seg_start = sl; seg_tile = true;
     } else if ((int)blockIdx.x < segunits) {
         const int b = (int)blockIdx.x, x = b & 7, q = b >> 3, pos = q / (GS_SEG_MAX - 1), k = q - pos * (GS_SEG_MAX - 1) + 1, slot = 8 * pos + x;
         const uint32_t sl = a.seg_len[slot], t = a.tile_order[a.front + 8 * pos + x];
@@ -833,6 +852,12 @@
             if (sl) {
                 if (part) return;
                 nparts = 1; seg_end = sl; seg_tile = true;
+            }
+        } else if (a.snap_u && nparts == 1) {
+            const int m = (int)blockIdx.x - segunits - a.front;
+            if (m >= 0 && m < a.useg) {
+                const uint32_t sl = a.seg_len_u[m];
+                if (sl) { seg_end = sl; seg_tile = true; }
             }
         }
     }
@@ -873,6 +898,7 @@
     for (int i = tid; i < front; i += 1024) order[i] = GS_LPT_NONE;
     uint32_t *seg_len = order + front + 8 * per;
     if (front > 0) for (int i = tid; i < front / 3; i += 1024) { seg_len[i] = 0; if (zero_words) zero_words[i] = 0; }
+    uint32_t *seg_len_u = (front > 0 && walked) ? seg_len + front / 3 : nullptr;
     if (tid == 0) { wmax = 1; nsplit = 0; }
     if (zero14 && tid < 14) zero14[tid] = 0ull;
     __syncthreads();
@@ -959,7 +985,7 @@
     __syncthreads();
     uint32_t *main_order = order + front;
     for (int i = tid; i < 8 * per; i += 1024)
-        if ((uint32_t)(i >> 3) >= xcount[i & 7]) main_order[i] = GS_LPT_NONE;
+        if ((uint32_t)(i >> 3) >= xcount[i & 7]) { main_order[i] = GS_LPT_NONE; if (seg_len_u) seg_len_u[i] = 0u; }
     const uint32_t thr = front > 0 ? max(wtot / (uint32_t)max(split_div, 1), 256u) : 0xFFFFFFFFu, eligible = (uint32_t)front / 24u;
     for (int t = tid; t < ntiles; t += 1024) {
         int local;
@@ -967,6 +993,7 @@
         const int x = (int)(gi & 7u), r = x * nb + cls[t], i = (int)(gi >> 3) * GT + local;
         const uint32_t pos = rowstart[r] + pre[r * W + (i >> 5)] + (uint32_t)__popc(bm[r * W + (i >> 5)] & ((1u << (i & 31)) - 1u));
         uint32_t entry = (uint32_t)t;
+        if (seg_len_u) seg_len_u[8u * pos + (uint32_t)x] = gs_seg_len_two(walked[t]);
         if (pos < eligible) {
             const uint32_t w = ranges_mode ? src[2 * t + 1] - src[2 * t] : src[t];
             if (w >= thr) {
@@ -974,6 +1001,7 @@
                 for (uint32_t j = 0; j < extra; ++j) order[8u * (3u * pos + j) + (uint32_t)x] = (uint32_t)t | ((j + 1u) << 28) | (pc << 30);
                 entry |= pc << 30;
                 atomicAdd(&nsplit, 1u);
+                if (seg_len_u) seg_len_u[8u * pos + (uint32_t)x] = 0u;
                 if (walked) {
                     const uint32_t wk = walked[t], per_seg = (wk + GS_SEG_MAX - 1) / GS_SEG_MAX;
                     const uint32_t sl = max((per_seg + 63u) & ~63u, (uint32_t)GS_SEG_MIN_LEN);
@@ -1055,7 +1083,8 @@
 static dim3 composite_grid(const GsCompositeArgs &a, int ntiles, bool bwd = false) {
     const int len = (a.tile_order && a.order_len > 0) ? a.order_len : ((ntiles + 7) / 8) * 8;
     if (bwd && a.snap && a.seg_hist && a.t_min > 0.0f) return dim3((unsigned)(len * a.seg_n * (a.parts > 1 ? a.parts : 1)));
-    return dim3((unsigned)(len * (a.parts > 1 ? a.parts : 1) + ((bwd && a.snap && a.t_min > 0.0f) ? gs_seg_units(a.front) : 0)));
+    return dim3((unsigned)(len * (a.parts > 1 ? a.parts : 1) + ((bwd && a.snap && a.t_min > 0.0f) ? gs_seg_units(a.front) : 0) +
+                           ((bwd && a.snap_u && a.t_min > 0.0f) ? a.useg : 0)));
 }
 
 int gs_composite_grid_blocks(const GsCompositeArgs &a, int bwd) { return (int)composite_grid(a, a.gx * a.gy, bwd != 0).x; }
@@ -1076,6 +1105,7 @@
     if (a.split_ok && (!early || a.tile_ext || a.tile_pos || a.parts > 1)) return hipErrorInvalidValue;
     if (a.snap && !a.seg_hist && (!a.split_ok || !a.seg_len || !a.snap_walked || !a.tile_order || a.front <= 0)) return hipErrorInvalidValue;
     if (a.snap && a.seg_hist && (a.tile_order || a.seg_n < 2 || a.seg_n > GS_SEG_MAX || !early || a.tile_ext || a.tile_pos)) return hipErrorInvalidValue;
+    if (a.snap_u && (!a.split_ok || !a.seg_len_u || !a.tile_order || a.front <= 0 || a.useg <= 0 || a.useg > a.order_len - a.front || a.seg_hist)) return hipErrorInvalidValue;
     if (a.tile_ext && (gs_bin3_seg() != L2_SEG || !early || !a.cranges || !a.cids || !a.clr || !a.ids_w || a.tile_pos)) return hipErrorInvalidValue;
     if (a.tile_pos) {
         if (!early || a.tile_clock) return hipErrorInvalidValue;
@@ -1089,7 +1119,7 @@
         else hipLaunchKernelGGL((composite_fwd_kernel<false, GS_FWD_MINW, true, true>), grid, block, 0, s, a);
         return hipGetLastError();
     }
-    if (early && a.snap) {
+    if (early && (a.snap || a.snap_u)) {
         if (a.cull) hipLaunchKernelGGL((composite_fwd_kernel<true, GS_FWD_MINW, true, false, false, true>), grid, block, 0, s, a);
         else hipLaunchKernelGGL((composite_fwd_kernel<true, GS_FWD_MINW, false, false, false, true>), grid, block, 0, s, a);
     } else if (early) {
@@ -1110,6 +1140,7 @@
     const dim3 grid = composite_grid(a, ntiles, true), block(64);
     if (a.snap && !a.seg_hist && (!a.split_ok || !a.seg_len || !a.snap_walked || !a.tile_order || a.front <= 0)) return hipErrorInvalidValue;
     if (a.snap && a.seg_hist && (a.tile_order || a.seg_n < 2 || a.seg_n > GS_SEG_MAX || !early || a.tile_ext || a.nseg > 1)) return hipErrorInvalidValue;
+    if (a.snap_u && (!a.split_ok || !a.seg_len_u || !a.fwd_walked || !a.tile_order || a.front <= 0 || a.useg <= 0 || a.useg > a.order_len - a.front || a.seg_hist)) return hipErrorInvalidValue;
     if (a.parts > 1 && ((a.parts != 2 && a.parts != 4) || !early || a.tile_ext || a.nseg > 1 || (a.tile_clock && !a.clock_by_block))) return hipErrorInvalidValue;
     if (a.split_ok && (!early || a.tile_ext || a.nseg > 1 || a.parts > 1)) return hipErrorInvalidValue;
 #define GS_B2(E, D) do { if (a.cull) hipLaunchKernelGGL((composite_bwd_kernel<E, GS_BWD_MINW, D, true>), grid, block, 0, s, a); \
diff --git a/gaussiansplat_amd/csrc/gs_ctx.h b/gaussiansplat_amd/csrc/gs_ctx.h
--- a/gaussiansplat_amd/csrc/gs_ctx.h
+++ b/gaussiansplat_amd/csrc/gs_ctx.h
@@ -93,6 +93,10 @@
     const uint32_t *seg_hist = nullptr;
     uint32_t *pinned_split = nullptr;
     const uint32_t *frame_order_split = nullptr;
+    DevBuf snap_u;
+    const uint32_t *snap_order_u = nullptr;
+    int frame_useg = 0;
+    float seg_frac = -1.0f;
     int snap_parity = 0;
     hipStream_t side = nullptr;
     hipEvent_t ev_main = nullptr, ev_order = nullptr;
@@ -215,6 +219,15 @@
 inline const uint32_t *order_seg_len(const gs_ctx *c, const uint32_t *order) { return order + lpt_front(c) + gs_lpt_order_len(c->gx, c->gy); }
 inline int lpt_order_entries(const gs_ctx *c) { return lpt_front(c) + gs_lpt_order_len(c->gx, c->gy); }
 inline int lpt_split_div(const gs_ctx *c) { return c->wave_slots * 4 / 5; }
+inline const uint32_t *order_seg_len_u(const gs_ctx *c, const uint32_t *order) { return order_seg_len(c, order) + lpt_front(c) / 3; }
+inline size_t order_words(const gs_ctx *c) { return (size_t)lpt_order_entries(c) + lpt_front(c) / 3 + gs_lpt_order_len(c->gx, c->gy) + 16; }
+inline int uniform_seg_entries(const gs_ctx *c) {
+    if (lpt_front(c) <= 0 || c->cfg.deterministic) return 0;
+    const float f = c->seg_frac >= 0.0f ? c->seg_frac : GS_SEG_UNIFORM_FRAC;
+    const int per_xcd = (int)(((int64_t)c->gx * c->gy + 7) / 8), cap = gs_lpt_order_len(c->gx, c->gy) / 8;
+    const int pos = (int)std::ceil((double)f * per_xcd);
+    return 8 * std::min(std::max(pos, 0), cap);
+}
 inline bool use_side_stream(const gs_ctx *c) { return c->n >= 262144 || (c->cfg.debug_flags & GS_DEBUG_ALWAYS_ORDER); }
 inline int order_index(const gs_ctx *c) { return c->view_slot >= 0 ? c->view_slot : GS_MAX_VIEW_SLOTS; }
 
diff --git a/include/gsplat.h b/include/gsplat.h
--- a/include/gsplat.h
+++ b/include/gsplat.h
@@ -184,6 +184,8 @@
 
 int gs_debug_set_window(gs_ctx *ctx, int32_t start, int32_t len);
 
+int gs_debug_set_seg_fraction(gs_ctx *ctx, float f);
+
 int gs_rank_probe_result(const gs_ctx *ctx);
 
 #ifdef __cplusplus
```

Measured after the change: 833.0 Msplats/s, median of 6. +1.9%, better.
